# cvlab-kaist/SOLA

Measured on AMD Instinct MI355X. Metric: track-selection forward+loss samples/sec at (T=32,N=64,d=256), higher is better.
Workload: dtype f32 via split-f16 (hi+lo f16 operand pairs, 3 f16 MFMAs per product, f32 accumulate); 1 GPU; SOLA track selection forward+BCE+alignment loss+selection, T=32 N=64 d=256 L=16, mevis/default model (32.98M params, random init), 256 samples/step/GPU, conv weights re-standardised every step; batch_per_gpu=256, tracks=64, frames=32, text_len=16

## Files before the change

include/sola_hip.h:

```cpp
#ifndef SOLA_HIP_H
#define SOLA_HIP_H

#include <stddef.h>
#include <stdint.h>

#ifdef __cplusplus
extern "C" {
#endif

typedef enum SolaStatus {
    SOLA_OK = 0,
    SOLA_ERR_ARG = -1,
    SOLA_ERR_HIP = -2,
    SOLA_ERR_WEIGHT = -3,
    SOLA_ERR_WORKSPACE = -4,
    SOLA_ERR_STATE = -5
} SolaStatus;

typedef struct SolaConfig {
    int32_t object_token_dim;
    int32_t lang_token_dim;
    int32_t n_layers;
    int32_t max_temporal_length;
    int32_t n_negative;
    int32_t n_groups;
    int32_t n_groups_module;
    int32_t num_heads;
} SolaConfig;

typedef struct SolaCtx SolaCtx;

const char* sola_last_error(void);
const char* sola_version(void);

int sola_ctx_create(const SolaConfig* cfg, int device, SolaCtx** out);
int sola_ctx_destroy(SolaCtx* ctx);

int sola_num_weights(const SolaCtx* ctx);
int sola_weight_info(const SolaCtx* ctx, int index, const char** name, int64_t* numel);

int sola_set_weight(SolaCtx* ctx, const char* name, const void* dev_ptr, int64_t numel);

int sola_weights_changed(SolaCtx* ctx);
int sola_set_ws_policy(SolaCtx* ctx, int recompute_every_forward);

int sola_set_precision(SolaCtx* ctx, int precision);
int sola_set_split_guard(SolaCtx* ctx, int enable);

int sola_set_x16_arena(SolaCtx* ctx, void* dev_ptr, size_t bytes);
int sola_x16_arena_info(const SolaCtx* ctx, size_t* need_bytes, size_t* capacity_bytes, size_t* used_bytes);
int sola_split_fallback_count(const SolaCtx* ctx, int64_t* count, int32_t* last_guard);
int sola_cast_sp16(const float* dev_in, int ld_in, float* dev_out, int ld_out, int64_t rows, int K, float scale, void* stream);
int sola_cast_sp16_auto(const float* dev_in, int ld_in, float* dev_out, int ld_out, int64_t rows, int K, float* dev_scal, void* stream);
int sola_gemm_nt_split(const float* dev_a_sp, int lda, const float* dev_w_sp, const float* dev_bias, const float* dev_r,
                       int ldr, int r_is_split, float* dev_c, int ldc, int c_is_split, int M, int N, int K, float out_scale,
                       void* stream);
int sola_gemm_nt_split_scaled(const float* dev_a_sp, int lda, const float* dev_w_sp, const float* dev_bias, const float* dev_r,
                              int ldr, int r_is_split, float* dev_c, int ldc, int c_is_split, int M, int N, int K,
                              float out_scale, const float* dev_out_scale, void* stream);

int sola_cast_f16(const float* dev_in, int ld_in, void* dev_out, int ld_out, int64_t rows, int K, float scale, float* dev_scal, void* stream);
int sola_gemm_nt_f16(const void* dev_a_h, int lda, const void* dev_w_h, const float* dev_bias, const void* dev_r_h, int ldr,
                     void* dev_c, int ldc, int c_is_f16, int M, int N, int K, float out_scale, void* stream);
int sola_attention_f16(const void* dev_q, int ldq, const void* dev_k, int ldk, const void* dev_v, int ldv, void* dev_o, int ldo,
                       int G, int H, int head_dim, int Sq, int Sk, int inner, int64_t q_outer, int64_t q_inner, int64_t q_row_stride,
                       int64_t k_outer, int64_t k_inner, int64_t k_row_stride, float scale, void* stream);

int sola_gemm_nt_bf16(const void* dev_a, int lda, const void* dev_w, const float* dev_bias, const void* dev_r, int ldr, int r_is_bf16,
                      void* dev_c, int ldc, int c_is_bf16, int M, int N, int K, void* stream);
int sola_attention_bf16(const void* dev_q, int ldq, const void* dev_k, int ldk, const void* dev_v, int ldv, float* dev_o, void* dev_o_bf16, int ldo,
                        int G, int H, int head_dim, int Sq, int Sk, int inner, int64_t q_outer, int64_t q_inner, int64_t q_row_stride,
                        int64_t k_outer, int64_t k_inner, int64_t k_row_stride, float scale, float* dev_lse, void* stream);
int sola_attention_backward_bf16(const void* dev_q, int ldq, const void* dev_k, int ldk, const void* dev_v, int ldv, const void* dev_o, int o_is_bf16,
                                 const void* dev_dout, int dout_is_bf16, int ldo, const float* dev_lse, void* dev_dq_bf16, void* dev_dk_bf16, void* dev_dv_bf16,
                                 int ld_dq, int ld_dk, int ld_dv, float* dev_dq_scratch, float* dev_dvec, int G, int H, int head_dim, int Sq, int Sk,
                                 int inner, int64_t q_outer, int64_t q_inner, int64_t q_row_stride, int64_t k_outer, int64_t k_inner,
                                 int64_t k_row_stride, float scale, int64_t q_rows, float* dev_scratch, size_t scratch_floats, void* stream);

size_t sola_workspace_bytes(const SolaCtx* ctx, int B, int N, int T, int L);
int sola_forward(SolaCtx* ctx,
                 const float* dev_object_tokens,
                 const float* dev_lang_tokens,
                 int B, int N, int T, int L,
                 float* dev_score_map,
                 float* dev_score_tokens,
                 void* dev_workspace, size_t workspace_bytes, void* stream);

typedef struct SolaRaggedBatch {
    int32_t n_videos;
    const int32_t* video_tracks;
    const int32_t* video_frames;
    int32_t n_samples;
    const int32_t* sample_video;
    const int32_t* sample_text_len;
} SolaRaggedBatch;
size_t sola_ragged_workspace_bytes(const SolaCtx* ctx, const SolaRaggedBatch* batch);
int sola_forward_ragged(SolaCtx* ctx, const float* dev_object_tokens, const float* dev_lang_tokens, const SolaRaggedBatch* batch,
                        float* dev_score_map, float* dev_score_tokens, void* dev_workspace, size_t workspace_bytes, void* stream);
int sola_loss_ragged(const float* dev_score_map, const float* dev_score_tokens, const float* dev_labels,
                     const float* dev_pos_tokens, const float* dev_neg_tokens, int64_t neg_batch_stride, int n_samples,
                     const int32_t* dev_track_offsets, int max_tracks, int64_t total_tracks, int D, int n_neg,
                     float positive_weight, float temperature, float alignment_weight, float* dev_loss3,
                     int32_t* dev_neg_argmax, void* dev_scratch, size_t scratch_bytes, void* stream);

int sola_workspace_tap(const SolaCtx* ctx, const char* name, size_t* byte_offset, int64_t* rows, int64_t* cols);

int sola_loss(const float* dev_score_map, const float* dev_score_tokens,
              const float* dev_labels,
              const float* dev_pos_tokens,
              const float* dev_neg_tokens, int64_t neg_batch_stride,
              int B, int N, int D, int n_neg,
              float positive_weight, float temperature, float alignment_weight,
              float* dev_loss3, int32_t* dev_neg_argmax,
              void* dev_scratch, size_t scratch_bytes, void* stream);

int sola_select(const float* dev_score_map, int64_t n, float threshold, float* dev_prob, float* dev_pred, void* stream);

int sola_ws_standardize(const float* dev_w, int cout, int cin, int k, float* dev_out, void* stream);
int sola_gemm_nt(const float* dev_a, int lda, const float* dev_w, const float* dev_bias, const float* dev_r, int ldr,
                 float* dev_c, int ldc, int M, int N, int K, void* stream);
int sola_gemm_nn(const float* dev_a, int lda, const float* dev_w0, const float* dev_w1, const float* dev_w2, int w_rows, const float* dev_r,
                 int ldr, float* dev_c, int ldc, int M, int N, int K, void* stream);
int sola_conv1d_cl(const float* dev_x, const float* dev_wstd, const float* dev_bias, float* dev_y,
                   int R, int T_in, int cin, int cout, int k, int stride, int pad, void* stream);
int sola_group_norm(const float* dev_x, float* dev_y, float* dev_y2, const float* dev_pe,
                    const float* dev_gamma, const float* dev_beta,
                    int n_inst, int inner, int64_t outer_stride, int64_t inner_stride, int64_t tok_stride,
                    int ntok, int C, int groups, float eps, float leaky_slope, int apply_leaky, void* stream);
int sola_attention(const float* dev_q, int ldq, const float* dev_k, int ldk, const float* dev_v, int ldv,
                   float* dev_o, int ldo, int G, int H, int head_dim, int Sq, int Sk, int inner,
                   int64_t q_outer, int64_t q_inner, int64_t q_row_stride,
                   int64_t k_outer, int64_t k_inner, int64_t k_row_stride, float scale,
                   float* dev_lse , void* stream);
int sola_pos_encoding(const float* dev_gauss, int D, int t_len, int max_temporal_length, float* dev_pe, void* stream);

int sola_set_dropout(SolaCtx* ctx, float p_encoder, float p_attention, uint64_t seed);
int sola_set_stage_dropout(float p, uint64_t seed);
size_t sola_train_workspace_bytes(const SolaCtx* ctx, int B, int N, int T, int L);
size_t sola_backward_workspace_bytes(const SolaCtx* ctx, int B, int N, int T, int L);
int sola_set_grad(SolaCtx* ctx, const char* name, void* dev_ptr, int64_t numel);
int sola_forward_train(SolaCtx* ctx, const float* dev_object_tokens, const float* dev_lang_tokens,
                       int B, int N, int T, int L, float* dev_score_map, float* dev_score_tokens,
                       void* dev_workspace, size_t workspace_bytes, void* stream);
int sola_backward(SolaCtx* ctx, const float* dev_d_score_map, const float* dev_d_score_tokens,
                  const void* dev_forward_workspace, void* dev_scratch, size_t scratch_bytes, void* stream);
int sola_train_step_bind(SolaCtx* ctx, const char* const* names, const int32_t* group, int n, int n_groups);
size_t sola_train_step_workspace_bytes(const SolaCtx* ctx, int B, int N);
int sola_train_step(SolaCtx* ctx, const float* dev_object_tokens, const float* dev_lang_tokens, int B, int N, int T, int L,
                    const float* dev_labels, const float* dev_pos_tokens, float positive_weight, float temperature, float alignment_weight,
                    float max_grad_norm, float* dev_score_map, float* dev_score_tokens, float* dev_loss3, double* dev_grad_sq,
                    void* dev_train_workspace, size_t train_workspace_bytes, void* dev_backward_scratch, size_t backward_scratch_bytes,
                    void* dev_step_workspace, size_t step_workspace_bytes, void* stream);
int sola_adamw_bind(SolaCtx* ctx, const char* const* names, void* const* dev_exp_avg, void* const* dev_exp_avg_sq, void* const* dev_step, int n);
int sola_adamw_step(SolaCtx* ctx, double lr, double beta1, double beta2, double eps, double weight_decay, int64_t step, const double* dev_total_sq,
                    float max_grad_norm, int write_back_grads, void* stream);
size_t sola_train_ragged_workspace_bytes(const SolaCtx* ctx, const SolaRaggedBatch* batch);
size_t sola_backward_ragged_workspace_bytes(const SolaCtx* ctx, const SolaRaggedBatch* batch);
int sola_forward_train_ragged(SolaCtx* ctx, const float* dev_object_tokens, const float* dev_lang_tokens, const SolaRaggedBatch* batch,
                              float* dev_score_map, float* dev_score_tokens, void* dev_workspace, size_t workspace_bytes, void* stream);
int sola_backward_ragged(SolaCtx* ctx, const float* dev_d_score_map, const float* dev_d_score_tokens,
                         const void* dev_forward_workspace, void* dev_scratch, size_t scratch_bytes, void* stream);
int sola_loss_backward_ragged(const float* dev_score_map, const float* dev_score_tokens, const float* dev_labels,
                              const float* dev_pos_tokens, const float* dev_neg_tokens, int64_t neg_batch_stride, int n_samples,
                              const int32_t* dev_track_offsets, int max_tracks, int64_t total_tracks, int D, int n_neg,
                              float positive_weight, float temperature, float alignment_weight, const float* dev_g3,
                              float* dev_d_score_map, float* dev_d_score_tokens, float* dev_d_neg, void* dev_scratch,
                              size_t scratch_bytes, void* stream);
int sola_grad_bucket_count(const SolaCtx* ctx);
int sola_grad_bucket_of(const SolaCtx* ctx, const char* name);
int sola_backward_wait_bucket(SolaCtx* ctx, int bucket, void* stream);
int sola_loss_backward(const float* dev_score_map, const float* dev_score_tokens, const float* dev_labels,
                       const float* dev_pos_tokens, const float* dev_neg_tokens, int64_t neg_batch_stride,
                       int B, int N, int D, int n_neg, float positive_weight, float temperature, float alignment_weight,
                       const float* dev_g3, float* dev_d_score_map, float* dev_d_score_tokens, float* dev_d_neg,
                       void* dev_scratch, size_t scratch_bytes, void* stream);
size_t sola_grad_sqnorms_scratch_bytes(int n, const int64_t* numel);
int sola_grad_sqnorms(const float* const* dev_grads, const int64_t* numel, const int32_t* group, int n, int n_groups,
                      double* dev_out, void* dev_scratch, size_t scratch_bytes, void* stream);
int sola_grad_clip(float* const* dev_grads, const int64_t* numel, int n, const double* dev_total_sq, float max_norm,
                   void* stream);
int sola_ws_backward(const float* dev_w, const float* dev_dwstd, int cout, int cin, int k, float* dev_dw, void* stream);
int sola_attention_split(const float* dev_q_sp, int ldq, const float* dev_k_sp, int ldk, const float* dev_v_sp, int ldv,
                         float* dev_o, int ldo, int o_is_split, int G, int H, int head_dim, int Sq, int Sk, int inner,
                         int64_t q_outer, int64_t q_inner, int64_t q_row_stride,
                         int64_t k_outer, int64_t k_inner, int64_t k_row_stride, float scale, float* dev_lse, void* stream);
size_t sola_gemm_tn_scratch_bytes(int M, int N, int K);
int sola_gemm_tn(const float* dev_a, int lda, const float* dev_b, int ldb, float* dev_c, float* dev_bias_grad,
                 int M, int N, int K, void* dev_scratch, size_t scratch_bytes, void* stream);
size_t sola_gemm_tn_split_scratch_bytes(int M, int N, int K);
int sola_gemm_tn_split(const float* dev_a, int lda, const float* dev_b, int ldb, float* dev_c, int M, int N, int K,
                       void* dev_scratch, size_t scratch_bytes, void* stream);
int sola_gemm_tn_f16(const float* dev_a, int lda, const float* dev_b, int ldb, float* dev_c, int M, int N, int K, int fmt,
                     void* dev_scratch, size_t scratch_bytes, void* stream);
int sola_conv1d_cl_wgrad_f16(const float* dev_x, const float* dev_dy, float* dev_dwstd, int R, int T_in, int cin, int cout, int k,
                             int stride, int pad, int fmt, void* dev_scratch, size_t scratch_bytes, void* stream);
int sola_conv1d_cl_backward(const float* dev_x, const float* dev_wstd, const float* dev_dy, float* dev_dx,
                            float* dev_dwstd, float* dev_dbias, int R, int T_in, int cin, int cout, int k, int stride,
                            int pad, void* dev_scratch, size_t scratch_bytes, void* stream);
size_t sola_conv1d_cl_backward_split_scratch_bytes(int R, int T_in, int cin, int cout, int k, int stride, int pad);
int sola_conv1d_cl_backward_split(const float* dev_x, const float* dev_wstd, const float* dev_dy, float* dev_dx,
                                  float* dev_dwstd, float* dev_dbias, int R, int T_in, int cin, int cout, int k, int stride,
                                  int pad, void* dev_scratch, size_t scratch_bytes, void* stream);
int sola_group_norm_backward(const float* dev_x, const float* dev_dy, const float* dev_dy2, const float* dev_gamma,
                             const float* dev_beta, float* dev_dx, float* dev_dgamma, float* dev_dbeta,
                             int n_inst, int inner, int64_t outer_stride, int64_t inner_stride, int64_t tok_stride,
                             int ntok, int C, int groups, float eps, float leaky_slope, int apply_leaky,
                             void* dev_scratch, size_t scratch_bytes, void* stream);
int sola_attention_backward(const float* dev_q, int ldq, const float* dev_k, int ldk, const float* dev_v, int ldv,
                            const float* dev_o, const float* dev_dout, int ldo, const float* dev_lse,
                            float* dev_dq, float* dev_dk, float* dev_dv, float* dev_dvec ,
                            int G, int H, int head_dim, int Sq, int Sk, int inner,
                            int64_t q_outer, int64_t q_inner, int64_t q_row_stride,
                            int64_t k_outer, int64_t k_inner, int64_t k_row_stride, float scale, void* stream);
size_t sola_attention_backward_scratch_floats(int64_t q_rows, int G, int H, int Sk);
int sola_attention_backward_ws(const float* dev_q, int ldq, const float* dev_k, int ldk, const float* dev_v, int ldv,
                               const float* dev_o, const float* dev_dout, int ldo, const float* dev_lse,
                               float* dev_dq, float* dev_dk, float* dev_dv, float* dev_dvec, int G, int H, int head_dim, int Sq, int Sk,
                               int inner, int64_t q_outer, int64_t q_inner, int64_t q_row_stride, int64_t k_outer, int64_t k_inner,
                               int64_t k_row_stride, float scale, int64_t q_rows, float* dev_scratch, size_t scratch_floats, void* stream);

int64_t sola_mask_words(int H, int W);
int sola_mask_pack(const void* dev_masks, int elem_type, int n, int h, int w, int H, int W,
                   uint32_t* dev_bits, int64_t* dev_area, void* stream);
int sola_mask_pair_counts(const uint32_t* dev_a_bits, const int64_t* dev_a_area, int P, int T,
                          const uint32_t* dev_b_bits, const int64_t* dev_b_area, int R,
                          const int32_t* dev_a_frame, int64_t words,
                          int64_t* dev_inter, int64_t* dev_union, void* stream);
size_t sola_mask_iou_scratch_bytes(int P, int R, int H, int W);
int sola_mask_iou_matrix(const void* dev_a, const void* dev_b, int elem_type, int P, int R, int H, int W, int h, int w,
                         int64_t* dev_inter, int64_t* dev_union, void* dev_scratch, size_t scratch_bytes, void* stream);

int sola_mask_bilinear_pack(const void* dev_masks, int elem_type, int n, int h, int w, int H, int W,
                            uint32_t* dev_bits, int64_t* dev_area, void* stream);
int sola_mask_unpack(const uint32_t* dev_bits, int n, int H, int W, void* dev_out, int elem_type, void* stream);
int sola_rle_fill_or(const uint32_t* dev_cum, const int64_t* dev_off, int n_frames, int K, int h, int w,
                     uint8_t* dev_out, uint32_t* dev_bits, int64_t* dev_area, void* stream);

int64_t sola_rle_string_to_cum(const char* str, int64_t len, uint32_t* host_cum, int64_t cap, int64_t limit);

int64_t sola_jf_plane_words(int h, int w);
int sola_rle_pack_cm(const uint32_t* dev_cum, const int64_t* dev_off, int64_t n_planes, int h, int w, int64_t words_stride,
                     uint32_t* dev_bits, void* stream);
int sola_mask_select_counts(const uint32_t* dev_bits, int64_t words_stride, int n_masks, int T, const int32_t* dev_pred_off,
                            const int32_t* dev_pred_idx, const int32_t* dev_gt_off, const int32_t* dev_gt_idx, int E,
                            int64_t* dev_counts, void* stream);
int64_t sola_rle_strings_to_cum_batch(const char* chars, const int64_t* str_off, int64_t n, uint32_t* host_cum, int64_t cap,
                                      int64_t limit, int64_t* run_off);

int sola_mask_select_boundary_counts(const uint32_t* dev_bits, int64_t words_stride, int n_masks, int T, int h, int w, int radius,
                                     const int32_t* dev_pred_off, const int32_t* dev_pred_idx, const int32_t* dev_gt_off,
                                     const int32_t* dev_gt_idx, int E, int64_t* dev_counts, void* workspace, size_t workspace_bytes,
                                     void* stream);
size_t sola_boundary_counts_workspace_bytes(int h, int w, int radius, int E, int T);

size_t sola_rle_encode_scratch_bytes(int n, int h, int w);
int sola_rle_encode_runs(const void* dev_masks, int elem_type, int n, int h, int w, int64_t* dev_run_off,
                         void* dev_scratch, size_t scratch_bytes, void* stream);
int sola_rle_encode_cum(const void* dev_masks, int elem_type, int n, int h, int w, const int64_t* dev_run_off,
// ... 40 lines not shown
```

sola_amd/_lib.py:

```python
from __future__ import annotations

import contextlib
import ctypes as C
import os

_HERE = os.path.dirname(os.path.abspath(__file__))
LIB_PATH = os.environ.get("SOLA_HIP_LIB") or os.path.join(_HERE, "lib", "libsola_hip.so")


class SolaLibraryError(RuntimeError):
    pass


class SolaError(RuntimeError):
    """A libsola_hip call returned a negative status."""


class SolaConfig(C.Structure):
    _fields_ = [
        ("object_token_dim", C.c_int32),
        ("lang_token_dim", C.c_int32),
        ("n_layers", C.c_int32),
        ("max_temporal_length", C.c_int32),
        ("n_negative", C.c_int32),
        ("n_groups", C.c_int32),
        ("n_groups_module", C.c_int32),
        ("num_heads", C.c_int32),
    ]


class SolaRaggedBatch(C.Structure):
    _fields_ = [
        ("n_videos", C.c_int32),
        ("video_tracks", C.POINTER(C.c_int32)),
        ("video_frames", C.POINTER(C.c_int32)),
        ("n_samples", C.c_int32),
        ("sample_video", C.POINTER(C.c_int32)),
        ("sample_text_len", C.POINTER(C.c_int32)),
    ]


_vp, _i, _i64, _f, _sz = C.c_void_p, C.c_int, C.c_int64, C.c_float, C.c_size_t

SIGNATURES = {
    "sola_last_error": (C.c_char_p, []),
    "sola_version": (C.c_char_p, []),
    "sola_ctx_create": (_i, [C.POINTER(SolaConfig), _i, C.POINTER(_vp)]),
    "sola_ctx_destroy": (_i, [_vp]),
    "sola_num_weights": (_i, [_vp]),
    "sola_weight_info": (_i, [_vp, _i, C.POINTER(C.c_char_p), C.POINTER(_i64)]),
    "sola_set_weight": (_i, [_vp, C.c_char_p, _vp, _i64]),
    "sola_weights_changed": (_i, [_vp]),
    "sola_set_ws_policy": (_i, [_vp, _i]),
    "sola_set_precision": (_i, [_vp, _i]),
    "sola_set_split_guard": (_i, [_vp, _i]),
    "sola_split_fallback_count": (_i, [_vp, C.POINTER(_i64), C.POINTER(C.c_int32)]),
    "sola_cast_sp16": (_i, [_vp, _i, _vp, _i, _i64, _i, _f, _vp]),
    "sola_gemm_nt_split": (_i, [_vp, _i, _vp, _vp, _vp, _i, _i, _vp, _i, _i, _i, _i, _i, _f, _vp]),
    "sola_cast_sp16_auto": (_i, [_vp, _i, _vp, _i, _i64, _i, _vp, _vp]),
    "sola_gemm_nt_split_scaled": (_i, [_vp, _i, _vp, _vp, _vp, _i, _i, _vp, _i, _i, _i, _i, _i, _f, _vp, _vp]),
    "sola_cast_f16": (_i, [_vp, _i, _vp, _i, _i64, _i, _f, _vp, _vp]),
    "sola_gemm_nt_f16": (_i, [_vp, _i, _vp, _vp, _vp, _i, _vp, _i, _i, _i, _i, _i, _f, _vp]),
    "sola_gemm_nn": (_i, [_vp, _i, _vp, _vp, _vp, _i, _vp, _i, _vp, _i, _i, _i, _i, _vp]),
    "sola_gemm_nt_bf16": (_i, [_vp, _i, _vp, _vp, _vp, _i, _i, _vp, _i, _i, _i, _i, _i, _vp]),
    "sola_attention_bf16": (_i, [_vp, _i, _vp, _i, _vp, _i, _vp, _vp, _i, _i, _i, _i, _i, _i, _i, _i64, _i64, _i64, _i64, _i64, _i64, _f, _vp, _vp]),
    "sola_attention_backward_bf16": (_i, [_vp, _i, _vp, _i, _vp, _i, _vp, _i, _vp, _i, _i, _vp, _vp, _vp, _vp, _i, _i, _i, _vp, _vp, _i, _i, _i, _i, _i, _i,
                                          _i64, _i64, _i64, _i64, _i64, _i64, _f, _i64, _vp, _sz, _vp]),
    "sola_attention_f16": (_i, [_vp, _i, _vp, _i, _vp, _i, _vp, _i, _i, _i, _i, _i, _i, _i, _i64, _i64, _i64, _i64, _i64, _i64, _f, _vp]),
    "sola_workspace_bytes": (_sz, [_vp, _i, _i, _i, _i]),
    "sola_forward": (_i, [_vp, _vp, _vp, _i, _i, _i, _i, _vp, _vp, _vp, _sz, _vp]),
    "sola_ragged_workspace_bytes": (_sz, [_vp, C.POINTER(SolaRaggedBatch)]),
    "sola_forward_ragged": (_i, [_vp, _vp, _vp, C.POINTER(SolaRaggedBatch), _vp, _vp, _vp, _sz, _vp]),
    "sola_loss_ragged": (_i, [_vp, _vp, _vp, _vp, _vp, _i64, _i, _vp, _i, _i64, _i, _i, _f, _f, _f, _vp, _vp, _vp, _sz, _vp]),
    "sola_train_ragged_workspace_bytes": (_sz, [_vp, C.POINTER(SolaRaggedBatch)]),
    "sola_backward_ragged_workspace_bytes": (_sz, [_vp, C.POINTER(SolaRaggedBatch)]),
    "sola_forward_train_ragged": (_i, [_vp, _vp, _vp, C.POINTER(SolaRaggedBatch), _vp, _vp, _vp, _sz, _vp]),
    "sola_backward_ragged": (_i, [_vp, _vp, _vp, _vp, _vp, _sz, _vp]),
    "sola_loss_backward_ragged": (_i, [_vp, _vp, _vp, _vp, _vp, _i64, _i, _vp, _i, _i64, _i, _i, _f, _f, _f, _vp, _vp, _vp, _vp, _vp, _sz, _vp]),
    "sola_workspace_tap": (_i, [_vp, C.c_char_p, C.POINTER(_sz), C.POINTER(_i64), C.POINTER(_i64)]),
    "sola_loss": (_i, [_vp, _vp, _vp, _vp, _vp, _i64, _i, _i, _i, _i, _f, _f, _f, _vp, _vp, _vp, _sz, _vp]),
    "sola_select": (_i, [_vp, _i64, _f, _vp, _vp, _vp]),
    "sola_ws_standardize": (_i, [_vp, _i, _i, _i, _vp, _vp]),
    "sola_gemm_nt": (_i, [_vp, _i, _vp, _vp, _vp, _i, _vp, _i, _i, _i, _i, _vp]),
    "sola_conv1d_cl": (_i, [_vp, _vp, _vp, _vp, _i, _i, _i, _i, _i, _i, _i, _vp]),
    "sola_group_norm": (_i, [_vp, _vp, _vp, _vp, _vp, _vp, _i, _i, _i64, _i64, _i64, _i, _i, _i, _f, _f, _i, _vp]),
    "sola_attention": (_i, [_vp, _i, _vp, _i, _vp, _i, _vp, _i, _i, _i, _i, _i, _i, _i, _i64, _i64, _i64, _i64, _i64, _i64, _f, _vp, _vp]),
    "sola_attention_split": (_i, [_vp, _i, _vp, _i, _vp, _i, _vp, _i, _i, _i, _i, _i, _i, _i, _i, _i64, _i64, _i64, _i64, _i64, _i64, _f, _vp, _vp]),
    "sola_set_dropout": (_i, [_vp, _f, _f, C.c_uint64]),
    "sola_set_stage_dropout": (_i, [_f, C.c_uint64]),
    "sola_train_workspace_bytes": (_sz, [_vp, _i, _i, _i, _i]),
    "sola_backward_workspace_bytes": (_sz, [_vp, _i, _i, _i, _i]),
    "sola_set_grad": (_i, [_vp, C.c_char_p, _vp, _i64]),
    "sola_forward_train": (_i, [_vp, _vp, _vp, _i, _i, _i, _i, _vp, _vp, _vp, _sz, _vp]),
    "sola_backward": (_i, [_vp, _vp, _vp, _vp, _vp, _sz, _vp]),
    "sola_grad_bucket_count": (_i, [_vp]),
    "sola_grad_bucket_of": (_i, [_vp, C.c_char_p]),
    "sola_backward_wait_bucket": (_i, [_vp, _i, _vp]),
    "sola_loss_backward": (_i, [_vp, _vp, _vp, _vp, _vp, _i64, _i, _i, _i, _i, _f, _f, _f, _vp, _vp, _vp, _vp, _vp, _sz, _vp]),
    "sola_ws_backward": (_i, [_vp, _vp, _i, _i, _i, _vp, _vp]),
    "sola_gemm_tn_scratch_bytes": (_sz, [_i, _i, _i]),
    "sola_gemm_tn_split_scratch_bytes": (_sz, [_i, _i, _i]),
    "sola_gemm_tn_split": (_i, [_vp, _i, _vp, _i, _vp, _i, _i, _i, _vp, _sz, _vp]),
    "sola_gemm_tn_f16": (_i, [_vp, _i, _vp, _i, _vp, _i, _i, _i, _i, _vp, _sz, _vp]),
    "sola_conv1d_cl_wgrad_f16": (_i, [_vp, _vp, _vp, _i, _i, _i, _i, _i, _i, _i, _i, _vp, _sz, _vp]),
    "sola_gemm_tn": (_i, [_vp, _i, _vp, _i, _vp, _vp, _i, _i, _i, _vp, _sz, _vp]),
    "sola_conv1d_cl_backward": (_i, [_vp, _vp, _vp, _vp, _vp, _vp, _i, _i, _i, _i, _i, _i, _i, _vp, _sz, _vp]),
    "sola_conv1d_cl_backward_split_scratch_bytes": (_sz, [_i, _i, _i, _i, _i, _i, _i]),
    "sola_conv1d_cl_backward_split": (_i, [_vp, _vp, _vp, _vp, _vp, _vp, _i, _i, _i, _i, _i, _i, _i, _vp, _sz, _vp]),
    "sola_group_norm_backward": (_i, [_vp, _vp, _vp, _vp, _vp, _vp, _vp, _vp, _i, _i, _i64, _i64, _i64, _i, _i, _i, _f, _f, _i, _vp, _sz, _vp]),
    "sola_attention_backward": (_i, [_vp, _i, _vp, _i, _vp, _i, _vp, _vp, _i, _vp, _vp, _vp, _vp, _vp, _i, _i, _i, _i, _i, _i,
                                     _i64, _i64, _i64, _i64, _i64, _i64, _f, _vp]),
    "sola_attention_backward_scratch_floats": (_sz, [_i64, _i, _i, _i]),
    "sola_attention_backward_ws": (_i, [_vp, _i, _vp, _i, _vp, _i, _vp, _vp, _i, _vp, _vp, _vp, _vp, _vp, _i, _i, _i, _i, _i, _i,
                                        _i64, _i64, _i64, _i64, _i64, _i64, _f, _i64, _vp, _sz, _vp]),
    "sola_pos_encoding": (_i, [_vp, _i, _i, _i, _vp, _vp]),
    "sola_mask_words": (_i64, [_i, _i]),
    "sola_mask_pack": (_i, [_vp, _i, _i, _i, _i, _i, _i, _vp, _vp, _vp]),
    "sola_mask_pair_counts": (_i, [_vp, _vp, _i, _i, _vp, _vp, _i, _vp, _i64, _vp, _vp, _vp]),
    "sola_mask_bilinear_pack": (_i, [_vp, _i, _i, _i, _i, _i, _i, _vp, _vp, _vp]),
    "sola_mask_unpack": (_i, [_vp, _i, _i, _i, _vp, _i, _vp]),
    "sola_rle_fill_or": (_i, [_vp, _vp, _i, _i, _i, _i, _vp, _vp, _vp, _vp]),
    "sola_rle_string_to_cum": (_i64, [C.c_char_p, _i64, _vp, _i64, _i64]),
    "sola_jf_plane_words": (_i64, [_i, _i]),
    "sola_rle_pack_cm": (_i, [_vp, _vp, _i64, _i, _i, _i64, _vp, _vp]),
    "sola_mask_select_counts": (_i, [_vp, _i64, _i, _i, _vp, _vp, _vp, _vp, _i, _vp, _vp]),
    "sola_mask_select_boundary_counts": (_i, [_vp, _i64, _i, _i, _i, _i, _i, _vp, _vp, _vp, _vp, _i, _vp, _vp, _sz, _vp]),
    "sola_boundary_counts_workspace_bytes": (_sz, [_i, _i, _i, _i, _i]),
    "sola_rle_strings_to_cum_batch": (_i64, [_vp, _vp, _i64, _vp, _i64, _i64, _vp]),
    "sola_rle_encode_scratch_bytes": (_sz, [_i, _i, _i]),
    "sola_rle_encode_runs": (_i, [_vp, _i, _i, _i, _i, _vp, _vp, _sz, _vp]),
    "sola_rle_encode_cum": (_i, [_vp, _i, _i, _i, _i, _vp, _vp, _vp, _vp, _sz, _vp]),
    "sola_rle_encode_chars": (_i, [_vp, _vp, _vp, _i, _vp, _vp]),
    "sola_png_deflate_scratch_bytes": (_sz, [_i, _i, _i]),
    "sola_png_deflate_sizes": (_i, [_vp, _i, _i, _i, _i, _vp, _vp, _vp, _sz, _vp]),
    "sola_png_deflate_write": (_i, [_vp, _i, _i, _i, _i, _vp, _vp, _vp, _vp, _sz, _vp]),
    "sola_mask_iou_scratch_bytes": (_sz, [_i, _i, _i, _i]),
    "sola_mask_iou_matrix": (_i, [_vp, _vp, _i, _i, _i, _i, _i, _i, _i, _vp, _vp, _vp, _sz, _vp]),
    "sola_grad_sqnorms_scratch_bytes": (_sz, [_i, _vp]),
    "sola_grad_sqnorms": (_i, [_vp, _vp, _vp, _i, _i, _vp, _vp, _sz, _vp]),
    "sola_grad_clip": (_i, [_vp, _vp, _i, _vp, _f, _vp]),
    "sola_set_x16_arena": (_i, [_vp, _vp, _sz]),
    "sola_x16_arena_info": (_i, [_vp, C.POINTER(_sz), C.POINTER(_sz), C.POINTER(_sz)]),
    "sola_tune": (_i, [C.c_char_p, _i]),
    "sola_tune_query": (_i, [C.c_char_p, C.POINTER(_i), C.POINTER(_i)]),
    "sola_tune_key": (C.c_char_p, [_i]),
    "sola_has_experiments": (_i, []),
    "sola_selftest": (_i, [_vp]),
    "sola_adamw_bind": (_i, [_vp, C.POINTER(C.c_char_p), C.POINTER(_vp), C.POINTER(_vp), C.POINTER(_vp), _i]),
    "sola_adamw_step": (_i, [_vp, C.c_double, C.c_double, C.c_double, C.c_double, C.c_double, _i64, _vp, _f, _i, _vp]),
    "sola_train_step_bind": (_i, [_vp, C.POINTER(C.c_char_p), C.POINTER(C.c_int32), _i, _i]),
    "sola_train_step_workspace_bytes": (_sz, [_vp, _i, _i]),
    "sola_train_step": (_i, [_vp, _vp, _vp, _i, _i, _i, _i, _vp, _vp, _f, _f, _f, _f, _vp, _vp, _vp, _vp, _vp, _sz, _vp, _sz, _vp, _sz, _vp]),
    "sola_gemm_trace_read": (C.c_longlong, [_vp, C.c_longlong]),
    "sola_profile_enable": (_i, [_i]),
    "sola_profile_read": (_i, [C.POINTER(_i64), C.POINTER(C.c_double), C.POINTER(C.c_double), C.POINTER(C.c_double), _i]),
}

PROF_CATEGORIES = ["gemm128", "attn", "group_norm", "ws_standardize", "head_loss", "misc", "iou_pack", "iou_pair", "gemm64", "gemm_tn", "attn_bwd", "gemm_split",
                   "gemm_split256", "gemm_split256_gn"]

_lib = None


def lib():
    global _lib
    if _lib is not None:
        return _lib
    import torch

    if not os.path.exists(LIB_PATH):
        raise SolaLibraryError(
            f"{LIB_PATH} not found. Build it with `python -c 'import __graft_entry__ as g; g.build()'` "
            "(or `make -C sola_amd/csrc`). sola_amd has no CPU or PyTorch fallback.")
    try:
        h = C.CDLL(LIB_PATH)
    except OSError as e:
        raise SolaLibraryError(f"failed to load {LIB_PATH}: {e}") from e
    for name, (res, args) in SIGNATURES.items():
        try:
            fn = getattr(h, name)
        except AttributeError as e:
            raise SolaLibraryError(f"{LIB_PATH} does not export {name}") from e
        fn.restype = res
        fn.argtypes = args
    for kv in filter(None, os.environ.get("SOLA_TUNE", "").split(",")):
        k, v = kv.split("=")
        if h.sola_tune(k.strip().encode(), int(v)) != 0:
            raise SolaLibraryError(f"SOLA_TUNE: unknown key {k!r}")
    _lib = h
    return h


def has_experiments():
    return bool(lib().sola_has_experiments())


def tune_query(key):
    value, default = _i(), _i()
    check(lib().sola_tune_query(key.encode(), C.byref(value), C.byref(default)), f"sola_tune_query {key!r}")
    return value.value, default.value


def tune_default(key):
    return tune_query(key)[1]


@contextlib.contextmanager
def tuned(**keys):
    before = [(k, tune_query(k)[0]) for k in keys]
    try:
        for k, v in keys.items():
            check(lib().sola_tune(k.encode(), int(v)), f"sola_tune {k!r}")
        yield
    finally:
        for k, old in reversed(before):
            check(lib().sola_tune(k.encode(), old), f"sola_tune {k!r}")


def check(status, what=""):
    if status != 0:
        msg = lib().sola_last_error()
        raise SolaError(f"{what} failed with status {status}: {msg.decode() if msg else ''}")


def ptr(t):
    return None if t is None else C.c_void_p(t.data_ptr())


def current_stream(device=None):
    import torch

    return C.c_void_p(torch.cuda.current_stream(device).cuda_stream)
# ... 25 lines not shown
```

sola_amd/csrc/api.hip:

```cpp
#include <math.h>
#include <stdarg.h>
#include <string.h>

#include <algorithm>
#include <exception>
#include <mutex>

#include "ragged.h"
#include "tune.h"

static thread_local char g_err[1024] = "";
void sola_set_error(const char* fmt, ...) {
    va_list ap;
    va_start(ap, fmt);
    vsnprintf(g_err, sizeof(g_err), fmt, ap);
    va_end(ap);
}
extern "C" const char* sola_last_error(void) { return g_err; }
extern "C" const char* sola_version(void) { return "sola_hip 0.6 (gfx950; f32, range-guarded split-f16 and f16-operand MFMA forward and backward, ragged batches, mask IoU + masklet rows)"; }

namespace {
struct ProfRec {
    int cat;
    hipEvent_t e0, e1;
// ... 203 lines not shown
    if (w->grad != static_cast<float*>(dev_ptr)) c->adam_n = 0;
    w->grad = static_cast<float*>(dev_ptr);
    return SOLA_OK;
}

extern "C" int sola_weights_changed(SolaCtx* c) {
    SOLA_ARG(c, "weights_changed: null ctx");
    c->ws_dirty = true;
    c->lin16_dirty = true;
    return SOLA_OK;
}

extern "C" int sola_set_dropout(SolaCtx* c, float p_encoder, float p_attention, uint64_t seed) {
    SOLA_ARG(c && p_encoder >= 0.f && p_encoder < 1.f && p_attention >= 0.f && p_attention < 1.f, "set_dropout: bad argument");
    c->p_drop_encoder = p_encoder;
    c->p_drop_attention = p_attention;
    c->drop_seed = seed;
    return SOLA_OK;
}

static thread_local DropoutCfg g_stage_drop = {0u, 0u, 0xFFFFFFFFu, 1.f, 0};
extern "C" int sola_set_stage_dropout(float p, uint64_t seed) {
    SOLA_ARG(p >= 0.f && p < 1.f, "set_stage_dropout: p=%f", (double)p);
    g_stage_drop = make_dropout(p, seed, 0);
    return SOLA_OK;
}

__global__ void selftest_wave_kernel(const float* __restrict__ in, int* __restrict__ bad) {
    const int i = blockIdx.x * blockDim.x + threadIdx.x;
    const float x = in[i];
    float v = x, m = x;
    int wrong = 0;
    float w = x;
#pragma unroll
    for (int o = 32, s = 0; o > 0; o >>= 1, ++s) {
        v += __shfl_xor(v, o, 64);
        m = fmaxf(m, __shfl_xor(m, o, 64));
        w = s == 0 ? sum_xor32(w) : s == 1 ? sum_xor16(w) : s == 2 ? sum_xor8(w) : s == 3 ? sum_xor4(w) : s == 4 ? sum_xor2(w) : sum_xor1(w);
        wrong |= __float_as_uint(w) != __float_as_uint(v) ? 1 << s : 0;
    }
    wrong |= __float_as_uint(wave_sum(x)) != __float_as_uint(v) ? 64 : 0;
    wrong |= __float_as_uint(wave_max(x)) != __float_as_uint(m) ? 128 : 0;
    if (wrong) atomicOr(bad, wrong);
}
extern "C" int sola_selftest(void* stream_) {
    hipStream_t s = as_stream(stream_);
    constexpr int n = 64 * 1024;
    std::vector<float> h(n);
    unsigned r = 12345u;
    for (int i = 0; i < n; ++i) {
        r = r * 1664525u + 1013904223u;
        h[i] = ((int)(r >> 8) % 20001 - 10000) / 37.0f * ((i % 7) ? 1.f : 1e-3f);
    }
    float* d_in = nullptr;
    int* d_bad = nullptr;
    SOLA_HIP(hipMalloc(&d_in, n * sizeof(float)));
    if (hipMalloc(&d_bad, sizeof(int)) != hipSuccess) { (void)hipFree(d_in); sola_set_error("selftest: hipMalloc"); return SOLA_ERR_HIP; }
    int bad = 0, rc = SOLA_OK;
    if (hipMemcpyAsync(d_in, h.data(), n * sizeof(float), hipMemcpyHostToDevice, s) != hipSuccess || hipMemsetAsync(d_bad, 0, sizeof(int), s) != hipSuccess) rc = SOLA_ERR_HIP;
    if (rc == SOLA_OK) {
        hipLaunchKernelGGL(selftest_wave_kernel, dim3(n / 256), dim3(256), 0, s, d_in, d_bad);
        if (hipGetLastError() != hipSuccess || hipMemcpyAsync(&bad, d_bad, sizeof(int), hipMemcpyDeviceToHost, s) != hipSuccess || hipStreamSynchronize(s) != hipSuccess) rc = SOLA_ERR_HIP;
    }
    (void)hipFree(d_in);
    (void)hipFree(d_bad);
    if (rc != SOLA_OK) { sola_set_error("selftest: HIP error"); return rc; }
    if (bad) {
        sola_set_error("selftest: the vector-ALU wave reductions differ from the __shfl_xor butterfly (mask 0x%x: bits 0-5 = steps 32..1, 64 = wave_sum, 128 = wave_max)", bad);
        return SOLA_ERR_STATE;
    }
    return SOLA_OK;
}

extern "C" int sola_has_experiments(void) {
#ifdef SOLA_EXPERIMENTS
    return 1;
#else
    return 0;
#endif
}

static int g_stage_split_math = 0;
static void sola_set_stage_split_math(int v) { g_stage_split_math = v != 0; }
#define TUNE_EXTERN(key) extern int g_##key;
#define TUNE_NONE(key, setter, report)
SOLA_TUNE_KEYS(TUNE_EXTERN, TUNE_NONE)
#ifdef SOLA_EXPERIMENTS
SOLA_TUNE_EXPERIMENT_KEYS(TUNE_EXTERN, TUNE_NONE)
#endif
namespace {
struct TuneKey {
    const char* key;
    void (*set)(int);
    int (*report)();
    int initial;
};
#define TUNE_PLAIN(key) {#key, [](int v) { g_##key = v; }, []() -> int { return g_##key; }, g_##key},
#define TUNE_SPECIAL(key, setter, report) {#key, setter, []() -> int { return report; }, report},
const TuneKey g_tune_keys[] = {
    SOLA_TUNE_KEYS(TUNE_PLAIN, TUNE_SPECIAL)
#ifdef SOLA_EXPERIMENTS
    SOLA_TUNE_EXPERIMENT_KEYS(TUNE_PLAIN, TUNE_SPECIAL)
#endif
};
constexpr int kTuneKeys = sizeof(g_tune_keys) / sizeof(g_tune_keys[0]);

const TuneKey* tune_find(const char* key) {
    for (const TuneKey& k : g_tune_keys)
        if (!strcmp(key, k.key)) return &k;
    sola_set_error("tune: unknown key '%s'%s", key, sola_has_experiments() ? "" : " (experiment keys exist in EXPERIMENTS=1 builds only)");
    return nullptr;
}
}

extern "C" int sola_tune(const char* key, int value) {
    SOLA_ARG(key, "tune: null key");
    const TuneKey* k = tune_find(key);
    if (!k) return SOLA_ERR_ARG;
    k->set(value);
    return SOLA_OK;
}

extern "C" int sola_tune_query(const char* key, int* value, int* default_value) {
    SOLA_ARG(key, "tune: null key");
    const TuneKey* k = tune_find(key);
    if (!k) return SOLA_ERR_ARG;
    if (value) *value = k->report();
    if (default_value) *default_value = k->initial;
    return SOLA_OK;
}

extern "C" const char* sola_tune_key(int index) { return index >= 0 && index < kTuneKeys ? g_tune_keys[index].key : nullptr; }

extern "C" int sola_set_ws_policy(SolaCtx* c, int every) {
    SOLA_ARG(c, "set_ws_policy: null ctx");
    c->ws_every_forward = every != 0;
    return SOLA_OK;
}

extern "C" size_t sola_workspace_bytes(const SolaCtx* c, int B, int N, int T, int L) {
    if (!c || B <= 0 || N <= 0 || T <= 0 || L < 0) return 0;
    return make_plan(c, B, N, T, L, false).total;
}

extern "C" size_t sola_train_workspace_bytes(const SolaCtx* c, int B, int N, int T, int L) {
    if (!c || B <= 0 || N <= 0 || T <= 0 || L < 0) return 0;
    return make_plan(c, B, N, T, L, true).total;
}

extern "C" int sola_workspace_tap(const SolaCtx* c, const char* name, size_t* off, int64_t* rows, int64_t* cols) {
    SOLA_ARG(c && name, "workspace_tap: null argument");
    auto it = c->last.bufs.find(name);
    SOLA_ARG(it != c->last.bufs.end(), "workspace_tap: no buffer named '%s' (run sola_forward first)", name);
    if (off) *off = it->second.off;
    if (rows) *rows = it->second.rows;
    if (cols) *cols = it->second.cols;
    return SOLA_OK;
}

extern "C" int sola_set_precision(SolaCtx* c, int precision) {
    SOLA_ARG(c && precision >= 0 && precision <= 3, "set_precision: 0 (f32), 1 (split-f16), 2 (f16 storage / f16 GEMM operands) or 3 (bf16 GEMM operands, training)");
    if (precision >= 1 && !c->lin16_buf) {
        const size_t D = c->cfg.lang_token_dim;
        size_t ws_total = 0;
        for (int i = 0; i < 6; ++i) ws_total += (size_t)c->conv[i].cout * c->conv[i].cin * c->conv[i].k;
        SOLA_HIP(hipSetDevice(c->device));
        SOLA_HIP(hipMalloc(&c->ws16_buf, ws_total * sizeof(float)));
        SOLA_HIP(hipMalloc(&c->lin16_buf, (size_t)c->cfg.n_layers * 12 * D * D * sizeof(float)));
        const size_t n_pairs = 2 + (size_t)c->cfg.n_layers * 12;
        SOLA_HIP(hipMalloc(&c->scal_buf, (2 * n_pairs + 2 + 4) * sizeof(float)));
        SOLA_HIP(hipMemset(c->scal_buf, 0, (2 * n_pairs + 2 + 4) * sizeof(float)));
        c->guard = reinterpret_cast<int*>(c->scal_buf + 2 * n_pairs);
        SOLA_HIP(hipHostMalloc(reinterpret_cast<void**>(&c->guard_host), 2 * sizeof(int), hipHostMallocDefault));
        c->guard_host[0] = c->guard_host[1] = 0;
    }
    c->precision = precision;
    c->ws_dirty = true;
    c->lin16_dirty = true;
    return SOLA_OK;
}

extern "C" int sola_cast_sp16(const float* in, int ld_in, float* out, int ld_out, int64_t rows, int K, float scale, void* stream_) {
    return launch_cast_sp16(in, ld_in, out, ld_out, rows, K, scale, as_stream(stream_));
}

extern "C" int sola_gemm_nt_split(const float* a_sp, int lda, const float* w_sp, const float* bias, const float* r, int ldr,
                                  int r_sp16, float* cmat, int ldc, int c_sp16, int M, int N, int K, float out_scale, void* stream_) {
    SOLA_ARG(a_sp && w_sp && cmat, "gemm_nt_split: null argument");
    GemmDesc gd{};
    gd.nprob = 1;
    gd.p[0] = GemmProblem{a_sp, w_sp, bias, r, cmat};
    gd.M = M; gd.N = N; gd.K = K; gd.lda = lda; gd.ldr = ldr; gd.ldc = ldc;
    gd.arith = 1; gd.out_scale = out_scale; gd.r_sp16 = r_sp16; gd.c_sp16 = c_sp16;
    return launch_gemm(gd, as_stream(stream_));
}

int launch_attention_f16(const AttnDesc& d, hipStream_t s);
extern "C" int sola_cast_f16(const float* in, int ld_in, void* out, int ld_out, int64_t rows, int K, float scale, float* dev_scal, void* stream_) {
    return launch_cast_f16(in, ld_in, out, ld_out, rows, K, scale, dev_scal, as_stream(stream_));
}
extern "C" int sola_gemm_nt_f16(const void* a_h, int lda, const void* w_h, const float* bias, const void* r_h, int ldr, void* cmat, int ldc,
                                int c_is_f16, int M, int N, int K, float out_scale, void* stream_) {
    SOLA_ARG(a_h && w_h && cmat, "gemm_nt_f16: null argument");
    GemmDesc gd{};
    gd.nprob = 1;
    gd.p[0] = GemmProblem{static_cast<const float*>(a_h), static_cast<const float*>(w_h), bias, static_cast<const float*>(r_h), static_cast<float*>(cmat)};
    gd.M = M; gd.N = N; gd.K = K; gd.lda = lda; gd.ldr = ldr; gd.ldc = ldc;
    gd.arith = 2; gd.out_scale = out_scale; gd.r_f16 = r_h ? 1 : 0; gd.c_f16 = c_is_f16;
    return launch_gemm(gd, as_stream(stream_));
}
extern "C" int sola_attention_f16(const void* q, int ldq, const void* k, int ldk, const void* v, int ldv, void* o, int ldo, int G, int H,
                                  int head_dim, int Sq, int Sk, int inner, int64_t q_outer, int64_t q_inner, int64_t q_rs,
                                  int64_t k_outer, int64_t k_inner, int64_t k_rs, float scale, void* stream_) {
    SOLA_ARG(q && k && v && o, "attention_f16: null argument");
    AttnDesc d{static_cast<const float*>(q), static_cast<const float*>(k), static_cast<const float*>(v), static_cast<float*>(o), ldq, ldk, ldv, ldo,
               G, H, head_dim, Sq, Sk, inner, q_outer, q_inner, q_rs, k_outer, k_inner, k_rs, scale, nullptr};
    return launch_attention_f16(d, as_stream(stream_));
}

extern "C" int sola_gemm_nt_bf16(const void* a_b, int lda, const void* w_b, const float* bias, const void* r, int ldr, int r_is_bf16, void* cmat, int ldc,
                                 int c_is_bf16, int M, int N, int K, void* stream_) {
    SOLA_ARG(a_b && w_b && cmat, "gemm_nt_bf16: null argument");
    GemmDesc gd{};
    gd.nprob = 1;
    gd.p[0] = GemmProblem{static_cast<const float*>(a_b), static_cast<const float*>(w_b), bias, static_cast<const float*>(r), static_cast<float*>(cmat)};
    gd.M = M; gd.N = N; gd.K = K; gd.lda = lda; gd.ldr = ldr; gd.ldc = ldc;
    gd.arith = 2; gd.bf16 = 1; gd.out_scale = 1.f; gd.r_f16 = (r && r_is_bf16) ? 1 : 0; gd.c_f16 = c_is_bf16;
    return launch_gemm(gd, as_stream(stream_));
}
extern "C" int sola_attention_bf16(const void* q, int ldq, const void* k, int ldk, const void* v, int ldv, float* o, void* o_bf16, int ldo, int G, int H,
                                   int head_dim, int Sq, int Sk, int inner, int64_t q_outer, int64_t q_inner, int64_t q_rs,
                                   int64_t k_outer, int64_t k_inner, int64_t k_rs, float scale, float* lse, void* stream_) {
    SOLA_ARG(q && k && v && (o || o_bf16), "attention_bf16: null argument");
    AttnDesc d{static_cast<const float*>(q), static_cast<const float*>(k), static_cast<const float*>(v), o, ldq, ldk, ldv, ldo,
               G, H, head_dim, Sq, Sk, inner, q_outer, q_inner, q_rs, k_outer, k_inner, k_rs, scale, lse};
    d.drop = g_stage_drop;
    d.in_bf16 = 1;
    bool done = false;
    if (o_bf16) { d.o_cast = o_bf16; d.o_cast_fmt = 3; d.o_cast_done = &done; }
    SOLA_TRY(launch_attention(d, as_stream(stream_)));
    SOLA_ARG(!o_bf16 || done, "attention_bf16: this shape does not write the bf16 output");
    return SOLA_OK;
}
extern "C" int sola_attention_backward_bf16(const void* q, int ldq, const void* k, int ldk, const void* v, int ldv, const void* o, int o_bf16, const void* dout, int dout_bf16, int ldo,
                                            const float* lse, void* dq16, void* dk16, void* dv16, int ld_dq, int ld_dk, int ld_dv, float* dq_scratch,
                                            float* dvec, int G, int H, int head_dim, int Sq, int Sk, int inner, int64_t q_outer, int64_t q_inner,
                                            int64_t q_rs, int64_t k_outer, int64_t k_inner, int64_t k_rs, float scale, int64_t q_rows, float* scratch,
                                            size_t scratch_floats, void* stream_) {
    SOLA_ARG(q && k && v && o && dout && lse && dq16 && dk16 && dv16 && dq_scratch && dvec, "attention_backward_bf16: null argument");
    AttnBwdDesc d{static_cast<const float*>(q), static_cast<const float*>(k), static_cast<const float*>(v), static_cast<const float*>(o), static_cast<const float*>(dout), lse, dq_scratch, nullptr, nullptr, dvec,
                  ldq, ldk, ldv, ldo, ld_dq, ld_dk, ld_dv, G, H, head_dim, Sq, Sk, inner, q_outer, q_inner, q_rs, k_outer, k_inner, k_rs, scale};
    d.drop = g_stage_drop;
    d.part = scratch; d.part_floats = scratch_floats; d.part_rows = q_rows;
    d.io_bf16 = 1; d.dq16 = dq16; d.dk16 = dk16; d.dv16 = dv16;
    d.dout_bf16 = dout_bf16 ? 1 : 0;
    d.o_bf16 = o_bf16 ? 1 : 0;
    return launch_attention_bwd(d, as_stream(stream_));
}

extern "C" int sola_cast_sp16_auto(const float* in, int ld_in, float* out, int ld_out, int64_t rows, int K, float* scal, void* stream_) {
    return launch_cast_sp16_auto(in, ld_in, out, ld_out, rows, K, scal, as_stream(stream_));
}

extern "C" int sola_gemm_nt_split_scaled(const float* a_sp, int lda, const float* w_sp, const float* bias, const float* r, int ldr,
                                         int r_sp16, float* cmat, int ldc, int c_sp16, int M, int N, int K, float out_scale,
                                         const float* out_scale_dev, void* stream_) {
    SOLA_ARG(a_sp && w_sp && cmat, "gemm_nt_split_scaled: null argument");
    GemmDesc gd{};
    gd.nprob = 1;
    gd.p[0] = GemmProblem{a_sp, w_sp, bias, r, cmat};
    gd.M = M; gd.N = N; gd.K = K; gd.lda = lda; gd.ldr = ldr; gd.ldc = ldc;
    gd.arith = 1; gd.out_scale = out_scale; gd.out_scale_dev = out_scale_dev; gd.r_sp16 = r_sp16; gd.c_sp16 = c_sp16;
    return launch_gemm(gd, as_stream(stream_));
}

int sola_split_guard_tripped(SolaCtx* c, hipStream_t s, bool* tripped) {
    *tripped = false;
    if (!c->split_guard || !c->guard) return SOLA_OK;
    hipStreamCaptureStatus cap = hipStreamCaptureStatusNone;
    if (hipStreamIsCapturing(s, &cap) == hipSuccess && cap != hipStreamCaptureStatusNone) return SOLA_OK;
    SOLA_HIP(hipMemcpyAsync(c->guard_host, c->guard, 2 * sizeof(int), hipMemcpyDeviceToHost, s));
    SOLA_HIP(hipStreamSynchronize(s));
    *tripped = (c->guard_host[0] | c->guard_host[1]) != 0;
    if (!c->guard_host[1]) c->weight_range_bad = false;
    if (c->guard_host[1] && !c->weight_range_bad) {
        c->weight_range_bad = true;
        fprintf(stderr, "sola_hip: GroupNorm weights outside the range of the split-f16 activations (rms of (gamma, beta) not in "
                        "[2^-6, 2^9]): precision 1 calls run on the exact-f32 kernels until the weights change\n");
    }
    return SOLA_OK;
}
static bool split_known_out_of_range(const SolaCtx* c) { return c->precision == 1 && c->split_guard && c->weight_range_bad && !c->lin16_dirty; }

int g_infer_f32_rows = 4096;
struct PrecScope {
    SolaCtx* c;
    int saved;
    PrecScope(SolaCtx* ctx, int p) : c(ctx), saved(ctx->precision) { c->precision = p; }
    ~PrecScope() { c->precision = saved; }
    PrecScope(const PrecScope&) = delete;
    PrecScope& operator=(const PrecScope&) = delete;
};
static bool few_rows_f32(const SolaCtx* c, long long rows0) { return c->precision == 1 && g_infer_f32_rows > 0 && rows0 <= g_infer_f32_rows; }

extern "C" int sola_forward(SolaCtx* c, const float* obj, const float* lang, int B, int N, int T, int L, float* score_map,
                            float* score_tokens, void* workspace, size_t ws_bytes, void* stream_) {
    hipStream_t s = as_stream(stream_);
    SOLA_ARG(!c || c->precision != 3, "forward: precision 3 (bf16 GEMM operands) is a TRAINING mode; inference runs precision 0, 1 or 2");
    if (c && B > 0 && N > 0 && T > 0 && few_rows_f32(c, (long long)B * N * T)) {
        PrecScope f32(c, 0);
// ... 666 lines not shown
```

sola_amd/csrc/ctx.h:

```cpp
#pragma once
#include <string>
#include <unordered_map>
#include <vector>

#include "kernels.h"

struct ConvGeom {
    int cin, cout, k, stride, pad;
};
struct Weight {
    std::string name;
    int64_t numel;
    const float* ptr;
    float* grad;
};
struct Buf {
    size_t off;
    int64_t rows, cols;
};
struct Plan {
    int B = 0, N = 0, T = 0, L = 0, W = 0, Tp = 0, M = 0;
    int Tl[6] = {0};
    bool train = false;
    bool rag = false;
    std::unordered_map<std::string, Buf> bufs;
    size_t total = 0;
    size_t add(const std::string& name, int64_t rows, int64_t cols) {
        const size_t off = total;
        bufs[name] = Buf{off, rows, cols};
        total += (((size_t)rows * (size_t)cols * sizeof(float)) + 255) & ~(size_t)255;
        return off;
    }
};

struct RagTables {
    const int4* u_lvl[7] = {nullptr};
    const int2* rowmap[5] = {nullptr};
    const int4* imap[5] = {nullptr};
    const int4* u_vt = nullptr;
    const int4* u_st = nullptr;
    const int4* u_strk = nullptr;
    const int4* u_smp = nullptr;
    const int4* u_lang = nullptr;
    const int4* u_langk = nullptr;
    const int4* u_gather = nullptr;
    const int32_t* trk_off = nullptr;
    int V = 0, S = 0, NT = 0, sumNS = 0, sumTpV = 0, sumTpS = 0;
    int maxN = 0, maxT[7] = {0}, maxW = 0, maxRowsSample = 0;
    long long rows[7] = {0}, Mv = 0, Ms = 0, LW = 0, Lin = 0;
    bool identity = false;
};

struct SolaRagStage;
void sola_rag_stage_free(SolaRagStage* st);

struct SolaCtx {
    SolaConfig cfg;
    int device;
    ConvGeom conv[6];
    std::vector<Weight> weights;
    std::unordered_map<std::string, int> index;
    float* ws_buf = nullptr;
    size_t ws_off[6];
    bool ws_dirty = true;
    int ws16_fmt = 0;
    bool ws_every_forward = true;
    Plan last;
    const float* last_obj = nullptr;
    RagTables last_rag;
    const void* last_ws = nullptr;
    std::vector<char> qkv16;
    std::vector<char> res16;
    std::vector<char> attn_o16;
    std::vector<char> gn2_stats;
    int precision = 0;
    bool lin16_dirty = true;
    float* ws16_buf = nullptr;
    float* lin16_buf = nullptr;
    struct X16Entry { const float* src; const void* p16; int cols; int fmt; };
    std::vector<X16Entry> x16;
    char* x16_arena = nullptr;
    size_t x16_cap = 0, x16_used = 0, x16_need = 0;
    void* x16_alloc(size_t bytes) {
        bytes = (bytes + 255) & ~(size_t)255;
        x16_need += bytes;
        if (x16_used + bytes > x16_cap) return nullptr;
        void* r = x16_arena + x16_used;
        x16_used += bytes;
        return r;
    }
    const void* x16_find(const float* src, int cols, int fmt) const {
        for (const X16Entry& e : x16)
            if (e.src == src && e.cols == cols && e.fmt == fmt) return e.p16;
        return nullptr;
    }
    float* scal_buf = nullptr;
    int* guard = nullptr;
    int* guard_host = nullptr;
    bool split_guard = true;
    long long split_fallbacks = 0;
    bool weight_range_bad = false;
    SolaRagStage* rag_stage = nullptr;
    std::vector<hipEvent_t> bucket_ev;
    hipStream_t side_stream = nullptr;
    hipEvent_t ev_fork = nullptr, ev_side[4] = {nullptr, nullptr, nullptr, nullptr};
    bool bucket_recorded = false;
    int n_buckets() const { return cfg.n_layers + 1; }
    float* scal_pair(int i) const { return scal_buf + 2 * i; }
    float* scal_extra(int i) const { return scal_buf + 2 * (2 + (size_t)cfg.n_layers * 12) + 2 + i; }
    const float* lin_inv_scale(int layer, int attn, int proj) const { return scal_buf + 2 * (2 + (layer * 3 + attn) * 4 + proj) + 1; }
    struct StepBinding {
        std::vector<int> widx;
        std::vector<int32_t> group;
        std::vector<long long> numel;
        int n_groups = 0;
        size_t sq_scratch = 0;
    } step;
    void* adam_tab = nullptr;
    int adam_n = 0, adam_cap = 0, adam_blocks = 0;
    bool adam_has_steps = false;
    int* adam_ticket = nullptr;
    double adam_bytes = 0.0;
    float p_drop_encoder = 0.f, p_drop_attention = 0.f;
    unsigned long long drop_seed = 0;
    DropoutCfg enc_drop(int conv_idx) const { return make_dropout(p_drop_encoder, drop_seed, 1u + (unsigned)conv_idx); }
    DropoutCfg attn_drop(int layer, int a) const { return make_dropout(p_drop_attention, drop_seed, 100u + 3u * (unsigned)layer + (unsigned)a); }
};

static const int kConvIdx[6] = {0, 4, 8, 12, 16, 20};
static const int kNormIdx[5] = {1, 5, 9, 13, 17};
static const char* const kAttnShort[3] = {"obj", "mot", "o2l"};
static const char* const kAttnLong[3] = {"obj_attn", "motion_attn", "object2lang_attn"};
constexpr float kLinScale = 64.f;
int sola_refresh_lin16(SolaCtx* c, hipStream_t s);
int sola_refresh_conv_weights(SolaCtx* c, int fmt, bool force, hipStream_t s);
int sola_check_forward_args(const SolaCtx* c, const char* who, size_t need, const void* workspace, size_t ws_bytes);

inline const float* ctx_weight(const SolaCtx* c, const std::string& name) {
    auto it = c->index.find(name);
    return it == c->index.end() ? nullptr : c->weights[it->second].ptr;
}
inline float* ctx_grad(const SolaCtx* c, const std::string& name) {
    auto it = c->index.find(name);
    return it == c->index.end() ? nullptr : c->weights[it->second].grad;
}

inline std::string abuf(bool train, int layer, const char* attn, const char* what) {
    if (!train) return what;
    return "l" + std::to_string(layer) + "_" + attn + "_" + what;
}

struct RagShape;
Plan make_plan(const SolaCtx* c, int B, int N, int T, int L, bool train);
Plan make_plan_ragged(const SolaCtx* c, const RagShape& r, bool train);
int sola_forward_train_impl(SolaCtx* c, const float* obj, const float* lang, int B, int N, int T, int L, float* score_map,
                            float* score_tokens, void* workspace, size_t ws_bytes, hipStream_t s, const RagShape* rs = nullptr);
int sola_forward_infer_impl(SolaCtx* c, const float* obj, const float* lang, int B, int N, int T, int L, float* score_map,
                            float* score_tokens, void* workspace, size_t ws_bytes, hipStream_t s);
size_t sola_backward_scratch_bytes(const SolaCtx* c, const Plan& p);
size_t sola_ragged_workspace_bytes_impl(const SolaCtx* c, const SolaRaggedBatch* b, int precision);
int sola_forward_ragged_impl(SolaCtx* c, const float* obj, const float* lang, const SolaRaggedBatch* batch, float* score_map,
                             float* score_tokens, void* workspace, size_t ws_bytes, hipStream_t s);
```

sola_amd/csrc/forward.hip:

```cpp
#include <math.h>
#include <string.h>

#include <algorithm>

#include "ragged.h"

int g_train_gn_cast = 1;
extern int g_train_dw_f16;
int g_train_attn_cast = 1;
int g_train_bf16_store = 3;
int g_train_gn_stats = 1;
int g_train_x16_keep = 1;
int g_train_split_min_rows = 1024;

namespace {
struct PlanSizes {
    int64_t rows0;
    int64_t rows[6];
    int64_t M, BW;
    int64_t S;
    int64_t gn_slots;
    size_t tables;
};
void plan_fill(Plan& p, const SolaCtx* c, const PlanSizes& z, bool train) {
    const int D = c->cfg.lang_token_dim, H = c->cfg.num_heads;
    if (z.tables) p.add("tables", (int64_t)((z.tables + 3) / 4), 1);
    for (int i = 0; i < 6; ++i) {
        p.add("conv" + std::to_string(i), z.rows[i], c->conv[i].cout);
        if (i < 5) p.add("act" + std::to_string(i), z.rows[i], c->conv[i].cout);
    }
    if (z.M <= 8192) p.add("splitk", 8192, 4096);
    p.add("pe", p.Tp, D);
    p.add("gn_slots", z.gn_slots, 1);
    p.add("lang", z.BW, D);
    p.add("lbar", z.S, D);
    if (!train && c->precision >= 1) {
        p.add("obj_sp", z.rows0, c->cfg.object_token_dim);
        p.add("conv5_sp", z.M, D);
        p.add("lang_sp", z.BW, D);
    }
    if (train && c->precision >= 1 && z.M >= g_train_split_min_rows) {
        int64_t amax = std::max<int64_t>(z.rows0 * c->cfg.object_token_dim, std::max<int64_t>(z.M * D, z.BW * D));
        for (int i = 0; i < 5; ++i) amax = std::max<int64_t>(amax, z.rows[i] * c->conv[i].cout);
        p.add("sp_a", amax, 1);
        p.add("sp_b", z.M, D);
    }
    const int n_sets = train ? c->cfg.n_layers : 1;
    for (int l = 0; l < n_sets; ++l)
        for (int a = 0; a < (train ? 3 : 1); ++a) {
            p.add(abuf(train, l, kAttnShort[a], "q"), z.M, D);
            if (!train || a < 2) {
                p.add(abuf(train, l, kAttnShort[a], "k"), z.M, D);
                p.add(abuf(train, l, kAttnShort[a], "v"), z.M, D);
            }
            p.add(abuf(train, l, kAttnShort[a], "attn"), z.M, D);
            p.add(abuf(train, l, kAttnShort[a], "res"), z.M, D);
            if (train) p.add(abuf(train, l, kAttnShort[a], "lse"), z.M, H);
            if (!train || a == 2) {
                p.add(abuf(train, l, kAttnShort[a], "lk"), z.BW, D);
                p.add(abuf(train, l, kAttnShort[a], "lv"), z.BW, D);
            }
        }
    for (int l = 0; l < c->cfg.n_layers; ++l) {
        if (train) p.add("l" + std::to_string(l) + "_gn2st", z.S * c->cfg.n_groups_module, 2);
        p.add("l" + std::to_string(l) + "_obj", z.M, D);
        p.add("l" + std::to_string(l) + "_xpe", z.M, D);
        p.add("l" + std::to_string(l) + "_motion", z.M, D);
        p.add("l" + std::to_string(l) + "_o2l", z.M, D);
    }
}
}

Plan make_plan(const SolaCtx* c, int B, int N, int T, int L, bool train) {
    Plan p;
    p.B = B; p.N = N; p.T = T; p.L = L; p.train = train;
    p.W = L + c->cfg.n_negative;
    int t = T;
    for (int i = 0; i < 6; ++i) {
        t = (t + 2 * c->conv[i].pad - c->conv[i].k) / c->conv[i].stride + 1;
        p.Tl[i] = t;
    }
    p.Tp = p.Tl[5];
    p.M = B * N * p.Tp;
    const int64_t R = (int64_t)B * N;
    PlanSizes z{};
    z.rows0 = R * T;
    for (int i = 0; i < 6; ++i) z.rows[i] = R * p.Tl[i];
    z.M = p.M; z.BW = (int64_t)B * p.W; z.S = B;
    z.gn_slots = std::max<int64_t>(R * T, (int64_t)p.M) / 4 + 1024;
    plan_fill(p, c, z, train);
    return p;
}

Plan make_plan_ragged(const SolaCtx* c, const RagShape& r, bool train) {
    Plan p;
    p.rag = true;
    p.B = r.S; p.N = r.maxN; p.T = r.maxT[0]; p.L = r.maxW - c->cfg.n_negative; p.train = train;
    p.W = r.maxW;
    for (int i = 0; i < 6; ++i) p.Tl[i] = r.maxT[i + 1];
    p.Tp = r.maxT[6];
    p.M = (int)r.Ms;
    PlanSizes z{};
    z.rows0 = r.rows[0];
    for (int i = 0; i < 6; ++i) z.rows[i] = r.rows[i + 1];
    z.M = r.Ms; z.BW = r.LW; z.S = r.S;
    z.gn_slots = (int64_t)(rag_gn_slots_bytes(r) / 4 + 64);
    z.tables = rag_tables_bytes(r, train);
    plan_fill(p, c, z, train);
    return p;
}

int sola_forward_train_impl(SolaCtx* c, const float* obj, const float* lang, int B, int N, int T, int L, float* score_map,
                            float* score_tokens, void* workspace, size_t ws_bytes, hipStream_t s, const RagShape* rs) {
    SOLA_ARG(c && obj && lang && score_map && score_tokens && workspace, "forward: null argument");
    if (rs) SOLA_ARG(rs->identity, "forward: a ragged training batch has one sample per video (sample_video[i] == i)");
    else SOLA_ARG(B > 0 && N > 0 && T > 0 && L >= 1, "forward: bad sizes B=%d N=%d T=%d L=%d", B, N, T, L);
    Plan p = rs ? make_plan_ragged(c, *rs, true) : make_plan(c, B, N, T, L, true);
    SOLA_TRY(sola_check_forward_args(c, "forward", p.total, workspace, ws_bytes));
    char* base = static_cast<char*>(workspace);
    auto buf = [&](const std::string& name) { return reinterpret_cast<float*>(base + p.bufs.at(name).off); };
    float* const splitk_ws = p.bufs.count("splitk") ? buf("splitk") : nullptr;
    const size_t splitk_bytes = splitk_ws ? (size_t)p.bufs.at("splitk").rows * p.bufs.at("splitk").cols * sizeof(float) : 0;
    auto W = [&](const std::string& name) { return ctx_weight(c, name); };
    const int D = c->cfg.lang_token_dim, H = c->cfg.num_heads, DH = D / H;
    const int Tp = p.Tp, M = p.M, Wn = p.W;
    if (rs) { B = rs->S; N = rs->maxN; T = rs->maxT[0]; }
    const int R = rs ? rs->NT : B * N;
    RagTables rt;
    if (rs) SOLA_TRY(rag_build_tables(c, *rs, base + p.bufs.at("tables").off, true, &rt, s));
    auto level_rows = [&](int lvl) -> long long { return rs ? rs->rows[lvl] : (long long)R * (lvl == 0 ? T : p.Tl[lvl - 1]); };
    const long long text_rows = rs ? rs->LW : (long long)B * Wn;
    const bool pure = c->precision >= 2;
    const int bf = c->precision == 3 ? 1 : 0;
    const bool split = c->precision >= 1 && D % (pure ? 64 : 32) == 0 && c->cfg.object_token_dim % (pure ? 64 : 32) == 0 && p.M >= g_train_split_min_rows;
    const int lowp_arith = pure ? 2 : 1;
    auto cast_auto = [&](const float* in, int ld, float* out, long long rows, int K, float* scal) -> int {
        return pure ? launch_cast_f16(in, ld, out, K, rows, K, 0.f, scal, s, 13, nullptr, bf) : launch_cast_sp16_auto(in, ld, out, K, rows, K, scal, s);
    };
    auto cast_fixed = [&](const float* in, int ld, float* out, long long rows, int K, float scale, void* side16 = nullptr) -> int {
        return pure ? launch_cast_f16(in, ld, out, K, rows, K, scale, nullptr, s, 13, nullptr, bf) : launch_cast_sp16(in, ld, out, K, rows, K, scale, s, side16);
    };

    SOLA_TRY(sola_refresh_conv_weights(c, split ? (pure ? 2 + bf : 1) : 0, true, s));
    auto lin_idx = [&](const std::string& attn, int proj) -> int {
        const int l = attn[attn.find('.') + 1] - '0';
        int a3 = 0;
        for (int a = 0; a < 3; ++a)
            if (attn.size() >= strlen(kAttnLong[a]) && attn.compare(attn.size() - strlen(kAttnLong[a]), std::string::npos, kAttnLong[a]) == 0) a3 = a;
        return (l * 3 + a3) * 4 + proj;
    };
    auto lin16 = [&](const std::string& attn, int proj) -> const float* {
        return pure ? reinterpret_cast<const float*>(reinterpret_cast<const _Float16*>(c->lin16_buf) + (size_t)lin_idx(attn, proj) * D * D)
                    : c->lin16_buf + (size_t)lin_idx(attn, proj) * D * D;
    };
    auto lin_inv = [&](const std::string& attn, int proj) -> const float* { return c->scal_buf + 2 * (2 + lin_idx(attn, proj)) + 1; };
    if (split) SOLA_TRY(sola_refresh_lin16(c, s));
    float* const sp_a = split ? buf("sp_a") : nullptr;
    float* const sp_b = split ? buf("sp_b") : nullptr;
    const bool keep16 = split && pure && g_train_x16_keep != 0;
    const bool side16_on = split && !pure && g_train_x16_keep != 0 && g_train_dw_f16 != 0;
    c->x16.clear();
    c->x16_used = 0;
    c->x16_need = 0;
    auto side16 = [&](const float* src, long long rows, int cols) -> void* {
        if (!side16_on) return nullptr;
        void* q = c->x16_alloc((size_t)rows * cols * 2);
        if (q) c->x16.push_back(SolaCtx::X16Entry{src, q, cols, 1});
        return q;
    };
    auto slot16 = [&](int which, const float* src, long long rows, int cols) -> float* {
        if (keep16)
            if (void* q = c->x16_alloc((size_t)rows * cols * 2)) {
                c->x16.push_back(SolaCtx::X16Entry{src, q, cols, 1 + bf});
                return static_cast<float*>(q);
            }
        return which ? sp_b : sp_a;
    };

    const int gn_fmt = (split && pure && g_train_gn_cast) ? 2 + bf : 0;
    const float* pc_src[2] = {nullptr, nullptr};
    float* pc_dst[2] = {nullptr, nullptr};
    const float* x = obj;
    int t_in = T;
    for (int i = 0; i < 6; ++i) {
        const ConvGeom& g = c->conv[i];
        const std::string cp = "short_motion_encoder." + std::to_string(kConvIdx[i]);
        GemmDesc gd{};
        gd.nprob = 1;
        gd.p[0] = GemmProblem{x, c->ws_buf + c->ws_off[i], W(cp + ".bias"), nullptr, buf("conv" + std::to_string(i))};
        gd.M = (int)level_rows(i + 1); gd.N = g.cout; gd.K = g.k * g.cin;
        gd.lda = g.cin; gd.ldr = 0; gd.ldc = g.cout;
        gd.conv = g.k > 1 ? 1 : 0;
// ... 112 lines not shown
    void* ac_side = nullptr;
    bool ac_done = false;
    int o16_site = -1;
    c->attn_o16.assign((size_t)c->cfg.n_layers * 3, 0);
    auto attention = [&](AttnDesc& ad) -> int {
        ac_src = nullptr; ac_done = false;
        if (split && (pure ? g_train_attn_cast != 0 : g_train_attn_cast == 2) && ad.ldo == D) {
            ac_src = ad.o;
            ac_dst = slot16(0, ad.o, M, D);
            ac_side = side16(ad.o, M, D);
            ad.o_cast = ac_dst; ad.o_side = ac_side; ad.o_cast_fmt = pure ? 2 + bf : 1; ad.o_cast_done = &ac_done;
            if (o16_site >= 0 && ad.in_bf16 && g_train_bf16_store >= 3 && ac_dst != sp_a && ac_dst != sp_b && ad.o_cast_fmt == 3 &&
                attention_bf16_mfma_supported(ad) && attention_bwd_dout_bf16_enabled()) {
                ad.o = nullptr;
                c->attn_o16[(size_t)o16_site] = 1;
            }
        }
        o16_site = -1;
        return launch_attention(ad, s);
    };
    auto out_proj = [&](const std::string& attn, const float* ao, const float* resid, float* res, const void* r16 = nullptr) -> int {
        GemmDesc gd{};
        gd.nprob = 1;
        gd.p[0] = GemmProblem{ao, W(attn + ".out_proj.weight"), W(attn + ".out_proj.bias"), resid, res};
        gd.M = M; gd.N = D; gd.K = D; gd.lda = D; gd.ldr = D; gd.ldc = D;
        gd.splitk_ws = splitk_ws; gd.splitk_bytes = splitk_bytes;
        if (split && r16) { gd.p[0].R = static_cast<const float*>(r16); gd.r_f16 = 1; gd.c_f16 = 1; }
        if (split) {
            float* dst;
            if (ac_src == ao) {
                dst = ac_dst;
                if (!ac_done) SOLA_TRY(cast_fixed(ao, D, dst, M, D, 1.f, ac_side));
            } else {
                dst = slot16(0, ao, M, D);
                SOLA_TRY(cast_fixed(ao, D, dst, M, D, 1.f, side16(ao, M, D)));
            }
            ac_src = nullptr;
            gd.p[0].A = dst; gd.p[0].W = lin16(attn, 3); gd.p[0].scale_dev = lin_inv(attn, 3);
            gd.arith = lowp_arith; gd.out_scale = 1.f; gd.bf16 = bf;
        }
        return launch_gemm(gd, s);
    };
    int gn_layer = 0;
    auto gn = [&](const std::string& lp, int idx, const float* res, float* y, float* y2, int n_inst, int inner,
                  long long outer, long long inner_stride, long long tok_stride, int ntok, const int4* units = nullptr,
                  const float* next_src0 = nullptr, const float* next_src1 = nullptr, bool res_bf16 = false) -> int {
        GroupNormDesc nd{};
        nd.in_f16 = res_bf16 ? 2 : 0;
        if (gn_fmt) {
            const float* nxt[2] = {next_src0, next_src1};
            const long long y_rows = std::max<long long>(M, text_rows);
            for (int e = 0; e < 2; ++e) {
                if (!nxt[e]) continue;
                if (nxt[e] == y) { float* dst = slot16(e, y, y_rows, D); nd.y_cast = dst; pc_src[e] = y; pc_dst[e] = dst; }
                else if (nxt[e] == y2) { float* dst = slot16(e, y2, y_rows, D); nd.y2_cast = dst; pc_src[e] = y2; pc_dst[e] = dst; }
            }
            nd.cast_fmt = gn_fmt;
        }
            nd.slice_ws = buf("gn_slots"); nd.slice_ws_bytes = (size_t)p.bufs.at("gn_slots").rows * p.bufs.at("gn_slots").cols * sizeof(float);
        nd.x = res; nd.y = y; nd.y2 = y2; nd.pe = y2 ? buf("pe") : nullptr;
        nd.gamma = W(lp + "norm." + std::to_string(idx) + ".weight");
        nd.beta = W(lp + "norm." + std::to_string(idx) + ".bias");
        nd.n_inst = n_inst; nd.inner = inner; nd.outer_stride = outer; nd.inner_stride = inner_stride;
        nd.tok_stride = tok_stride; nd.ntok = ntok; nd.C = D; nd.groups = c->cfg.n_groups_module;
        nd.eps = 1e-5f; nd.slope = 0.f; nd.leaky = 0;
        nd.units = units;
        if (idx == 2 && g_train_gn_stats) {
            const int l = gn_layer;
            int wrote = 0;
            nd.stats_out = buf("l" + std::to_string(l) + "_gn2st");
            nd.stats_written = &wrote;
            SOLA_TRY(launch_group_norm(nd, s));
            if ((size_t)l < c->gn2_stats.size()) c->gn2_stats[l] = (char)wrote;
            return SOLA_OK;
        }
        return launch_group_norm(nd, s);
    };
    c->gn2_stats.assign((size_t)c->cfg.n_layers, 0);
    c->res16.assign((size_t)c->cfg.n_layers * 3, 0);
    auto resid16 = [&](const float* resid) -> const void* {
        if (!(split && pure && bf && g_train_bf16_store >= 2 && keep16 && D % 8 == 0)) return nullptr;
        return c->x16_find(resid, D, 1 + bf);
    };
    const float* xin = buf("conv5");
    for (int l = 0; l < c->cfg.n_layers; ++l) {
        const std::string lp = "object_lang_align_layers." + std::to_string(l) + ".";
        gn_layer = l;
        const std::string ls = "l" + std::to_string(l);
        auto ab = [&](int a, const char* what) { return buf(abuf(true, l, kAttnShort[a], what)); };
        float* x_obj = buf(ls + "_obj");
        float* x_pe = buf(ls + "_xpe");
        float* x_mot = buf(ls + "_motion");
        float* x_o2l = buf(ls + "_o2l");
        {
            AttnDesc ad{ab(0, "q"), ab(0, "k"), ab(0, "v"), ab(0, "attn"), D, D, D, D, B * Tp, H, DH, N, N, Tp,
                        (long long)N * Tp, 1, Tp, (long long)N * Tp, 1, Tp, scale, ab(0, "lse")};
            if (rs) { ad.G = rt.sumTpS; ad.inner = 1; ad.q_units = rt.u_st; }
            ad.drop = c->attn_drop(l, 0);
            const bool s16 = site16(ad, false);
            SOLA_TRY(linear3(xin, xin, xin, lp + "obj_attn", 3, M, ab(0, "q"), ab(0, "k"), ab(0, "v"), 0, nullptr, s16));
            ad.in_bf16 = s16 ? 1 : 0;
            c->qkv16[(size_t)l * 3 + 0] = s16;
            o16_site = l * 3 + 0;
            SOLA_TRY(attention(ad));
        }
        const void* r16_0 = resid16(xin);
        c->res16[(size_t)l * 3 + 0] = r16_0 != nullptr;
        SOLA_TRY(out_proj(lp + "obj_attn", ab(0, "attn"), xin, ab(0, "res"), r16_0));
        if (rs) SOLA_TRY(gn(lp, 0, ab(0, "res"), x_obj, x_pe, rt.sumTpS, 1, 0, 0, 1, N, rt.u_st, x_pe, x_obj, r16_0 != nullptr));
        else SOLA_TRY(gn(lp, 0, ab(0, "res"), x_obj, x_pe, B * Tp, Tp, (long long)N * Tp, 1, Tp, N, nullptr, x_pe, x_obj, r16_0 != nullptr));
        {
            AttnDesc ad{ab(1, "q"), ab(1, "k"), ab(1, "v"), ab(1, "attn"), D, D, D, D, B * N, H, DH, Tp, Tp, 1,
                        (long long)Tp, 0, 1, (long long)Tp, 0, 1, scale, ab(1, "lse")};
            if (rs) { ad.G = rt.sumNS; ad.q_units = rt.u_strk; }
            ad.drop = c->attn_drop(l, 1);
            const bool s16 = site16(ad, false);
            SOLA_TRY(linear3(x_pe, x_pe, x_obj, lp + "motion_attn", 3, M, ab(1, "q"), ab(1, "k"), ab(1, "v"), 0, nullptr, s16));
            ad.in_bf16 = s16 ? 1 : 0;
            c->qkv16[(size_t)l * 3 + 1] = s16;
            o16_site = l * 3 + 1;
            SOLA_TRY(attention(ad));
        }
        const void* r16_1 = resid16(x_obj);
        c->res16[(size_t)l * 3 + 1] = r16_1 != nullptr;
        SOLA_TRY(out_proj(lp + "motion_attn", ab(1, "attn"), x_obj, ab(1, "res"), r16_1));
        if (rs) SOLA_TRY(gn(lp, 1, ab(1, "res"), x_mot, nullptr, rt.sumNS, 1, 0, 0, 1, Tp, rt.u_strk, x_mot, nullptr, r16_1 != nullptr));
        else SOLA_TRY(gn(lp, 1, ab(1, "res"), x_mot, nullptr, B * N, 1, Tp, 0, 1, Tp, nullptr, x_mot, nullptr, r16_1 != nullptr));
        {
            AttnDesc ad{ab(2, "q"), ab(2, "lk"), ab(2, "lv"), ab(2, "attn"), D, D, D, D, B, H, DH, N * Tp, Wn, 1,
                        (long long)N * Tp, 0, 1, (long long)Wn, 0, 1, scale, ab(2, "lse")};
            if (rs) { ad.Sq = rt.maxRowsSample; ad.q_units = rt.u_smp; ad.k_units = rt.u_langk; }
            ad.drop = c->attn_drop(l, 2);
            const bool s16 = site16(ad, true);
            SOLA_TRY(linear3(x_mot, nullptr, nullptr, lp + "object2lang_attn", 1, M, ab(2, "q"), nullptr, nullptr, 0, nullptr, s16));
            SOLA_TRY(linear3(buf("lang"), buf("lang"), nullptr, lp + "object2lang_attn", 2, (int)text_rows, ab(2, "lk"), ab(2, "lv"), nullptr, 1,
                             split ? c->scal_pair(1) : nullptr, s16));
            ad.in_bf16 = s16 ? 1 : 0;
            c->qkv16[(size_t)l * 3 + 2] = s16;
            o16_site = l * 3 + 2;
            SOLA_TRY(attention(ad));
        }
        const void* r16_2 = resid16(x_mot);
        c->res16[(size_t)l * 3 + 2] = r16_2 != nullptr;
        SOLA_TRY(out_proj(lp + "object2lang_attn", ab(2, "attn"), x_mot, ab(2, "res"), r16_2));
        const float* nxt_in = l + 1 < c->cfg.n_layers ? x_o2l : nullptr;
        if (rs) SOLA_TRY(gn(lp, 2, ab(2, "res"), x_o2l, nullptr, B, 1, 0, 0, 1, rt.maxRowsSample, rt.u_smp, nxt_in, nullptr, r16_2 != nullptr));
        else SOLA_TRY(gn(lp, 2, ab(2, "res"), x_o2l, nullptr, B, 1, (long long)N * Tp, 0, 1, N * Tp, nullptr, nxt_in, nullptr, r16_2 != nullptr));
        xin = x_o2l;
    }

    HeadDesc hd{xin, buf("lbar"), score_map, score_tokens, B, N, Tp, D};
    if (rs) { hd.B = 1; hd.N = rt.sumNS; hd.units = rt.u_strk; }
    SOLA_TRY(launch_score_head(hd, s));
    c->last = p;
    c->last_rag = rt;
    c->last_ws = workspace;
    c->last_obj = obj;
    return SOLA_OK;
}
```

sola_amd/csrc/forward_infer.hip:

```cpp
#include <math.h>

#include <algorithm>

#include "ctx.h"

int sola_refresh_lin16(SolaCtx* c, hipStream_t s) {
    if (!c->lin16_dirty) return SOLA_OK;
    SOLA_ARG(c->lin16_buf && c->scal_buf, "split-f16 weights requested before sola_set_precision(ctx, 1)");
    static const char* pn[4] = {"q_proj", "k_proj", "v_proj", "out_proj"};
    const int D = c->cfg.lang_token_dim;
    std::vector<const float*> in;
    std::vector<float*> out;
    for (int l = 0; l < c->cfg.n_layers; ++l)
        for (int a = 0; a < 3; ++a)
            for (int j = 0; j < 4; ++j) {
                const std::string nm = "object_lang_align_layers." + std::to_string(l) + "." + kAttnLong[a] + "." + pn[j] + ".weight";
                const float* w = ctx_weight(c, nm);
                if (!w) {
                    sola_set_error("forward: weight '%s' has not been set", nm.c_str());
                    return SOLA_ERR_WEIGHT;
                }
                in.push_back(w);
                out.push_back(c->lin16_buf + ((size_t)(l * 3 + a) * 4 + j) * D * D);
            }
    if (c->precision >= 2) {
        std::vector<void*> outh;
        for (size_t i = 0; i < out.size(); ++i) outh.push_back(reinterpret_cast<_Float16*>(c->lin16_buf) + i * (size_t)D * D);
        SOLA_TRY(launch_cast_f16_auto_multi(in.data(), outh.data(), (int)in.size(), D, D, c->scal_pair(2), s, c->precision == 3 ? 1 : 0));
    } else {
        SOLA_TRY(launch_cast_sp16_auto_multi(in.data(), out.data(), (int)in.size(), D, D, c->scal_pair(2), s));
    }
    std::vector<NormPair> norms;
    for (int i = 0; i < 5; ++i) {
        const std::string np = "short_motion_encoder." + std::to_string(kNormIdx[i]);
        norms.push_back(NormPair{ctx_weight(c, np + ".weight"), ctx_weight(c, np + ".bias"), c->conv[i].cout});
    }
    for (int l = 0; l < c->cfg.n_layers; ++l)
        for (int j = 0; j < 3; ++j) {
            const std::string np = "object_lang_align_layers." + std::to_string(l) + ".norm." + std::to_string(j);
            norms.push_back(NormPair{ctx_weight(c, np + ".weight"), ctx_weight(c, np + ".bias"), D});
        }
    for (const NormPair& n : norms)
        if (!n.gamma || !n.beta) {
            sola_set_error("forward: a GroupNorm weight has not been set");
            return SOLA_ERR_WEIGHT;
        }
    SOLA_HIP(hipMemsetAsync(c->guard + 1, 0, sizeof(int), s));
    for (size_t i0 = 0; i0 < norms.size(); i0 += 32)
        SOLA_TRY(launch_norm_range_check(norms.data() + i0, (int)std::min<size_t>(32, norms.size() - i0), c->guard + 1, s));
    c->lin16_dirty = false;
    return SOLA_OK;
}

int sola_refresh_conv_weights(SolaCtx* c, int fmt, bool force, hipStream_t s) {
    if (!force && !c->ws_dirty && !c->ws_every_forward && (fmt == 0 || c->ws16_fmt == fmt)) return SOLA_OK;
    WsLayer layers[6];
    for (int i = 0; i < 6; ++i) {
        const std::string nm = "short_motion_encoder." + std::to_string(kConvIdx[i]) + ".weight";
        layers[i] = WsLayer{ctx_weight(c, nm), c->ws_buf + c->ws_off[i], c->conv[i].cout, c->conv[i].cin, c->conv[i].k};
    }
    SOLA_TRY(launch_ws_standardize(layers, 6, s));
    c->ws16_fmt = 0;
    for (int i = 0; i < 6 && fmt != 0; ++i) {
        const int kc = c->conv[i].k * c->conv[i].cin;
        const float* w = c->ws_buf + c->ws_off[i];
        if (fmt == 1) SOLA_TRY(launch_cast_sp16(w, kc, c->ws16_buf + c->ws_off[i], kc, c->conv[i].cout, kc, 1.f, s));
        else SOLA_TRY(launch_cast_f16(w, kc, reinterpret_cast<_Float16*>(c->ws16_buf) + c->ws_off[i], kc, c->conv[i].cout, kc, 1.f, nullptr, s, 13,
                                      nullptr, fmt == 3 ? 1 : 0));
    }
    c->ws_dirty = false;
    c->ws16_fmt = fmt;
    return SOLA_OK;
}

int sola_check_forward_args(const SolaCtx* c, const char* who, size_t need, const void* workspace, size_t ws_bytes) {
    for (const Weight& w : c->weights)
        if (!w.ptr) {
            sola_set_error("%s: weight '%s' has not been set", who, w.name.c_str());
            return SOLA_ERR_WEIGHT;
        }
    if (ws_bytes < need) {
        sola_set_error("%s: workspace %zu bytes < required %zu", who, ws_bytes, need);
        return SOLA_ERR_WORKSPACE;
    }
    SOLA_ARG((reinterpret_cast<uintptr_t>(workspace) & 255) == 0, "%s: workspace must be 256-byte aligned", who);
    return SOLA_OK;
}

int g_attn_split_min_keys = 96;

int g_lang_shared_neg = 1;

int launch_attention_f16(const AttnDesc& d, hipStream_t s);

int sola_forward_infer_impl(SolaCtx* c, const float* obj, const float* lang, int B, int N, int T, int L, float* score_map,
                            float* score_tokens, void* workspace, size_t ws_bytes, hipStream_t s) {
    SOLA_ARG(c && obj && lang && score_map && score_tokens && workspace, "forward: null argument");
    SOLA_ARG(B > 0 && N > 0 && T > 0 && L >= 1, "forward: bad sizes B=%d N=%d T=%d L=%d", B, N, T, L);
    const bool sp = c->precision == 1;
    const bool h16 = c->precision == 2;
    if (sp)
        SOLA_ARG(c->cfg.object_token_dim % 8 == 0 && (c->cfg.lang_token_dim / c->cfg.n_groups_module) % 8 == 0 &&
                     (2 * c->cfg.object_token_dim / c->cfg.n_groups) % 8 == 0 && (c->cfg.lang_token_dim / c->cfg.n_groups) % 8 == 0,
                 "split-f16 mode needs channel counts per GroupNorm group that are multiples of 8");
    if (h16)
        SOLA_ARG(c->cfg.object_token_dim % 64 == 0 && c->cfg.lang_token_dim % 64 == 0,
                 "16-bit storage mode needs object_token_dim and lang_token_dim to be multiples of 64");
    Plan p = make_plan(c, B, N, T, L, false);
    SOLA_TRY(sola_check_forward_args(c, "forward", p.total, workspace, ws_bytes));
    char* base = static_cast<char*>(workspace);
    auto buf = [&](const std::string& name) { return reinterpret_cast<float*>(base + p.bufs.at(name).off); };
    float* const splitk_ws = (!h16 && p.bufs.count("splitk")) ? buf("splitk") : nullptr;
    const size_t splitk_bytes = splitk_ws ? (size_t)p.bufs.at("splitk").rows * p.bufs.at("splitk").cols * sizeof(float) : 0;
    auto W = [&](const std::string& name) { return ctx_weight(c, name); };
    const int D = c->cfg.lang_token_dim, H = c->cfg.num_heads, DH = D / H, d_in = c->cfg.object_token_dim;
    const int Tp = p.Tp, M = p.M, Wn = p.W;
    const int R = B * N;
    int* const guard = (sp || h16) ? c->guard : nullptr;
    auto ws_w = [&](int i) -> const float* {
        if (h16) return reinterpret_cast<const float*>(reinterpret_cast<const _Float16*>(c->ws16_buf) + c->ws_off[i]);
        return sp ? c->ws16_buf + c->ws_off[i] : c->ws_buf + c->ws_off[i];
    };
    auto lin_w = [&](const std::string& an, const char* proj_name, int layer, int attn, int proj) -> const float* {
        const size_t idx = (size_t)(layer * 3 + attn) * 4 + proj;
        if (sp) return c->lin16_buf + idx * D * D;
        if (h16) return reinterpret_cast<const float*>(reinterpret_cast<const _Float16*>(c->lin16_buf) + idx * D * D);
        return W(an + "." + proj_name + ".weight");
    };
    auto lin_inv = [&](int layer, int attn, int proj) -> const float* { return (sp || h16) ? c->lin_inv_scale(layer, attn, proj) : nullptr; };

    SOLA_TRY(sola_refresh_conv_weights(c, sp ? 1 : (h16 ? 2 : 0), false, s));
    if (sp || h16) {
        SOLA_TRY(sola_refresh_lin16(c, s));
        SOLA_HIP(hipMemsetAsync(c->guard, 0, sizeof(int), s));
    } else {
        c->x16.clear();
        c->x16_used = 0;
        c->x16_need = 0;
    }

    const float* x = obj;
    if (sp) SOLA_TRY(launch_cast_sp16_auto(obj, d_in, buf("obj_sp"), d_in, (long long)R * T, d_in, c->scal_pair(0), s));
    if (h16) SOLA_TRY(launch_cast_f16(obj, d_in, buf("obj_sp"), d_in, (long long)R * T, d_in, 256.f, c->scal_pair(0), s, 6, c->scal_extra(0)));
    if (sp || h16) x = buf("obj_sp");
    const bool conv5_16 = h16 || (sp && c->conv[5].cout % 8 == 0);
    int t_in = T;
    for (int i = 0; i < 6; ++i) {
        const ConvGeom& g = c->conv[i];
        const std::string cp = "short_motion_encoder." + std::to_string(kConvIdx[i]);
        const bool to16 = i == 5 && conv5_16;
        GemmDesc gd{};
        gd.nprob = 1;
        gd.p[0] = GemmProblem{x, ws_w(i), W(cp + ".bias"), nullptr, to16 ? buf("conv5_sp") : buf("conv" + std::to_string(i))};
        gd.M = R * p.Tl[i]; gd.N = g.cout; gd.K = g.k * g.cin;
        gd.lda = g.cin; gd.ldr = 0; gd.ldc = g.cout;
        gd.conv = g.k > 1 ? 1 : 0;
        gd.T_in = t_in; gd.T_out = p.Tl[i]; gd.stride = g.stride; gd.pad = g.pad; gd.Cin = g.cin;
        if (sp) {
            gd.arith = 1; gd.out_scale = 1.f; gd.c_sp16 = to16 ? 1 : 0; gd.guard = guard;
            if (i == 0) gd.out_scale_dev = c->scal_pair(0) + 1;
        }
        if (h16) {
            gd.arith = 2; gd.out_scale = 1.f; gd.c_f16 = 1; gd.guard = guard;
            if (i == 0) gd.bias_scale_dev = c->scal_extra(0);
        }
        gd.splitk_ws = splitk_ws; gd.splitk_bytes = splitk_bytes;
        bool fused_norm = false;
        if (sp && i < 5) {
            GemmDesc probe = gd;
            probe.c_sp16 = 1;
            if (gemm_gn_fusable(probe, g.cout / c->cfg.n_groups, p.Tl[i])) {
                const std::string np = "short_motion_encoder." + std::to_string(kNormIdx[i]);
                gd.c_sp16 = 1;
                gd.p[0].C = buf("act" + std::to_string(i));
                gd.gn_gamma = W(np + ".weight"); gd.gn_beta = W(np + ".bias");
                gd.gn_tokens = p.Tl[i]; gd.gn_eps = 1e-5f; gd.gn_slope = 0.01f;
                fused_norm = true;
            }
        }
        SOLA_TRY(launch_gemm(gd, s));
        if (i < 5 && !fused_norm) {
            const std::string np = "short_motion_encoder." + std::to_string(kNormIdx[i]);
            GroupNormDesc nd{};
            nd.slice_ws = buf("gn_slots"); nd.slice_ws_bytes = (size_t)p.bufs.at("gn_slots").rows * p.bufs.at("gn_slots").cols * sizeof(float);
            nd.x = buf("conv" + std::to_string(i)); nd.y = buf("act" + std::to_string(i));
            nd.gamma = W(np + ".weight"); nd.beta = W(np + ".bias");
            nd.n_inst = R; nd.inner = 1; nd.outer_stride = p.Tl[i]; nd.inner_stride = 0; nd.tok_stride = 1;
            nd.ntok = p.Tl[i]; nd.C = g.cout; nd.groups = c->cfg.n_groups; nd.eps = 1e-5f; nd.slope = 0.01f; nd.leaky = 1;
            nd.out_sp16 = sp ? 1 : 0; nd.guard = guard;
            if (h16) {
                nd.in_f16 = 1; nd.out_f16 = 1;
                if (i == 0) nd.in_scale_dev = c->scal_pair(0) + 1;
            }
            SOLA_TRY(launch_group_norm(nd, s));
        }
        if (i < 5) x = buf("act" + std::to_string(i));
        t_in = p.Tl[i];
    }
    if (sp && !conv5_16) SOLA_TRY(launch_cast_sp16(buf("conv5"), D, buf("conv5_sp"), D, M, D, 1.f, s));

    SOLA_TRY(launch_pos_encoding(W("positional_encoding_gaussian_matrix"), D, Tp, c->cfg.max_temporal_length, buf("pe"), s));
    bool shared_neg = false;
    if (sp && g_lang_shared_neg && c->cfg.n_negative > 0 && Wn <= g_attn_split_min_keys && (long long)B * L + c->cfg.n_negative >= 1024) {
        AttnDesc probe{};
        probe.G = B; probe.H = H; probe.DH = DH; probe.Sq = N * Tp; probe.Sk = Wn; probe.inner = 1; probe.k_private = L;
        shared_neg = attention_shared_keys_supported(probe);
    }
    const long long lang_rows = shared_neg ? (long long)B * L + c->cfg.n_negative : (long long)B * Wn;
    if (shared_neg) SOLA_TRY(launch_lang_concat_shared(lang, W("negative_token.weight"), buf("lang"), buf("lbar"), B, L, c->cfg.n_negative, D, s));
    else SOLA_TRY(launch_lang_concat(lang, W("negative_token.weight"), buf("lang"), buf("lbar"), B, L, c->cfg.n_negative, D, s));
    if (sp) SOLA_TRY(launch_cast_sp16_auto(buf("lang"), D, buf("lang_sp"), D, lang_rows, D, c->scal_pair(1), s));
    if (h16) SOLA_TRY(launch_cast_f16(buf("lang"), D, buf("lang_sp"), D, lang_rows, D, 1.f, c->scal_pair(1), s, 6));
    const float* const lang_in = (sp || h16) ? buf("lang_sp") : buf("lang");

    const float scale = 1.0f / sqrtf((float)DH);
    auto linear3 = [&](const float* a0, const float* a1, const float* a2, int layer, int attn, int nprob, int rows, float* o0,
                       float* o1, float* o2, int first_proj, int out_sp16, const float* a_inv_scale = nullptr) -> int {
        static const char* pn[3] = {"q_proj", "k_proj", "v_proj"};
        const std::string an = "object_lang_align_layers." + std::to_string(layer) + "." + kAttnLong[attn];
        const float* as[3] = {a0, a1, a2};
        float* os[3] = {o0, o1, o2};
        GemmDesc gd{};
        gd.nprob = nprob;
        for (int j = 0; j < nprob; ++j)
            gd.p[j] = GemmProblem{as[j], lin_w(an, pn[first_proj + j], layer, attn, first_proj + j), W(an + "." + pn[first_proj + j] + ".bias"),
                                  nullptr, os[j], lin_inv(layer, attn, first_proj + j)};
        gd.M = rows; gd.N = D; gd.K = D; gd.lda = D; gd.ldr = 0; gd.ldc = D;
        if (sp) { gd.arith = 1; gd.out_scale = 1.f; gd.out_scale_dev = a_inv_scale; gd.c_sp16 = out_sp16; gd.guard = guard; }
        if (h16) { gd.arith = 2; gd.out_scale = 1.f; gd.out_scale_dev = a_inv_scale; gd.c_f16 = 1; gd.guard = guard; }
        gd.splitk_ws = splitk_ws; gd.splitk_bytes = splitk_bytes;
        return launch_gemm(gd, s);
    };
    auto out_proj = [&](int layer, int attn, const float* resid, int resid_sp16) -> int {
        const std::string an = "object_lang_align_layers." + std::to_string(layer) + "." + kAttnLong[attn];
        GemmDesc gd{};
        gd.nprob = 1;
        gd.p[0] = GemmProblem{buf("attn"), lin_w(an, "out_proj", layer, attn, 3), W(an + ".out_proj.bias"), resid, buf("res"), lin_inv(layer, attn, 3)};
        gd.M = M; gd.N = D; gd.K = D; gd.lda = D; gd.ldr = D; gd.ldc = D;
        if (sp) { gd.arith = 1; gd.out_scale = 1.f; gd.r_sp16 = resid_sp16; }
        if (h16) { gd.arith = 2; gd.out_scale = 1.f; gd.r_f16 = 1; gd.c_f16 = 1; gd.guard = guard; }
        gd.splitk_ws = splitk_ws; gd.splitk_bytes = splitk_bytes;
        return launch_gemm(gd, s);
    };
    auto gn = [&](const std::string& lp, int idx, float* y, float* y2, int out16, int n_inst, int inner, long long outer,
                  long long inner_stride, long long tok_stride, int ntok) -> int {
        GroupNormDesc nd{};
        nd.slice_ws = buf("gn_slots"); nd.slice_ws_bytes = (size_t)p.bufs.at("gn_slots").rows * p.bufs.at("gn_slots").cols * sizeof(float);
        nd.x = buf("res"); nd.y = y; nd.y2 = y2; nd.pe = y2 ? buf("pe") : nullptr;
        nd.gamma = W(lp + "norm." + std::to_string(idx) + ".weight");
        nd.beta = W(lp + "norm." + std::to_string(idx) + ".bias");
        nd.n_inst = n_inst; nd.inner = inner; nd.outer_stride = outer; nd.inner_stride = inner_stride;
        nd.tok_stride = tok_stride; nd.ntok = ntok; nd.C = D; nd.groups = c->cfg.n_groups_module;
        nd.eps = 1e-5f; nd.slope = 0.f; nd.leaky = 0; nd.guard = guard;
        if (sp) nd.out_sp16 = out16;
        if (h16) { nd.in_f16 = 1; nd.out_f16 = out16; }
        return launch_group_norm(nd, s);
    };
    auto attention = [&](const float* q, const float* k, const float* v, int G, int Sq, int Sk, int inner, long long qo,
                         long long qi, long long qr, long long ko, long long ki, long long kr, int in_sp16, int k_private = 0,
                         long long k_shared_row = 0) -> int {
        AttnDesc ad{q, k, v, buf("attn"), D, D, D, D, G, H, DH, Sq, Sk, inner, qo, qi, qr, ko, ki, kr, scale, nullptr};
        ad.k_private = k_private;
        ad.k_shared_row = k_shared_row;
        ad.o_sp16 = sp ? 1 : 0;
        ad.in_sp16 = in_sp16;
        ad.guard = guard;
        ad.split_math = sp ? 1 : 0;
        return h16 ? launch_attention_f16(ad, s) : launch_attention(ad, s);
    };
    const int obj_sp = (sp && N > g_attn_split_min_keys && N > 16 && DH % 16 == 0) ? 1 : 0;
    const int mot_sp = (sp && Tp > g_attn_split_min_keys && Tp > 16 && DH % 16 == 0) ? 1 : 0;
    const int o2l_sp = (sp && Wn > g_attn_split_min_keys && DH % 16 == 0) ? 1 : 0;

    const float* xin = (sp || h16) ? buf("conv5_sp") : buf("conv5");
    const float* xres = conv5_16 ? buf("conv5_sp") : buf("conv5");
    int xres_sp = conv5_16 ? 1 : 0;
    for (int l = 0; l < c->cfg.n_layers; ++l) {
        const std::string lp = "object_lang_align_layers." + std::to_string(l) + ".";
        const std::string ls = "l" + std::to_string(l);
        const bool last = l + 1 == c->cfg.n_layers;
        float *q = buf("q"), *k = buf("k"), *v = buf("v");
        float* x_obj = buf(ls + "_obj");
        float* x_pe = buf(ls + "_xpe");
        float* x_mot = buf(ls + "_motion");
        float* x_o2l = buf(ls + "_o2l");
        SOLA_TRY(linear3(xin, xin, xin, l, 0, 3, M, q, k, v, 0, obj_sp));
        SOLA_TRY(attention(q, k, v, B * Tp, N, N, Tp, (long long)N * Tp, 1, Tp, (long long)N * Tp, 1, Tp, obj_sp));
        SOLA_TRY(out_proj(l, 0, xres, xres_sp));
        SOLA_TRY(gn(lp, 0, x_obj, x_pe, 1, B * Tp, Tp, (long long)N * Tp, 1, Tp, N));
        SOLA_TRY(linear3(x_pe, x_pe, x_obj, l, 1, 3, M, q, k, v, 0, mot_sp));
        SOLA_TRY(attention(q, k, v, B * N, Tp, Tp, 1, (long long)Tp, 0, 1, (long long)Tp, 0, 1, mot_sp));
        SOLA_TRY(out_proj(l, 1, x_obj, 1));
        SOLA_TRY(gn(lp, 1, x_mot, nullptr, 1, B * N, 1, Tp, 0, 1, Tp));
        SOLA_TRY(linear3(x_mot, nullptr, nullptr, l, 2, 1, M, q, nullptr, nullptr, 0, o2l_sp));
        SOLA_TRY(linear3(lang_in, lang_in, nullptr, l, 2, 2, (int)lang_rows, buf("lk"), buf("lv"), nullptr, 1, o2l_sp, c->scal_pair(1) + 1));
        if (shared_neg) SOLA_TRY(attention(q, buf("lk"), buf("lv"), B, N * Tp, Wn, 1, (long long)N * Tp, 0, 1, (long long)L, 0, 1, o2l_sp, L, (long long)B * L));
        else SOLA_TRY(attention(q, buf("lk"), buf("lv"), B, N * Tp, Wn, 1, (long long)N * Tp, 0, 1, (long long)Wn, 0, 1, o2l_sp));
        SOLA_TRY(out_proj(l, 2, x_mot, 1));
        SOLA_TRY(gn(lp, 2, x_o2l, nullptr, last ? 0 : 1, B, 1, (long long)N * Tp, 0, 1, N * Tp));
        xin = x_o2l;
        xres = x_o2l;
        xres_sp = 1;
    }

    HeadDesc hd{xin, buf("lbar"), score_map, score_tokens, B, N, Tp, D};
    SOLA_TRY(launch_score_head(hd, s));
    c->last = p;
    c->last_obj = nullptr;
    return SOLA_OK;
}
```

sola_amd/csrc/head.hip:

```cpp
#include "kernels.h"

namespace {

struct HeadArgs {
    const float* x;
    const float* lbar;
    float* score_map;
    float* score_tokens;
    int N, Tp, D;
    const int4* units;
};

__global__ __launch_bounds__(256) void score_head_kernel(const HeadArgs a) {
    extern __shared__ float sh[];
    float* logits = sh;
    float* red = sh + ((a.Tp + 3) & ~3);
    const int bn = blockIdx.x;
    int b = bn / a.N, Tp = a.Tp;
    long long row0 = (long long)bn * a.Tp;
    if (a.units) {
        const int4 u = a.units[bn];
        row0 = u.x; Tp = u.z; b = u.w;
    }
    const int d4n = a.D >> 2;
    const float4* xb = reinterpret_cast<const float4*>(a.x + row0 * a.D);
    const float4* lb = reinterpret_cast<const float4*>(a.lbar + (long long)b * a.D);
    const int lane = threadIdx.x & 63, wave = threadIdx.x >> 6;
    for (int t = wave; t < Tp; t += 4) {
        float s = 0.f;
        for (int i = lane; i < d4n; i += 64) {
            const float4 xv = xb[(long long)t * d4n + i], lv = lb[i];
            s += (xv.x * lv.x + xv.y * lv.y) + (xv.z * lv.z + xv.w * lv.w);
        }
        s = wave_sum(s);
        if (lane == 0) logits[t] = s;
    }
    __syncthreads();
    float mx = -INFINITY;
    for (int t = 0; t < Tp; ++t) mx = fmaxf(mx, logits[t]);
    float den = 0.f;
    for (int t = 0; t < Tp; ++t) den += expf(logits[t] - mx);
    __syncthreads();
    for (int t = threadIdx.x; t < Tp; t += 256) logits[t] = expf(logits[t] - mx) / den;
    __syncthreads();
    float part = 0.f;
    float4* out = reinterpret_cast<float4*>(a.score_tokens + (long long)bn * a.D);
    for (int i = threadIdx.x; i < d4n; i += 256) {
        float4 acc = make_float4(0.f, 0.f, 0.f, 0.f);
        for (int t = 0; t < Tp; ++t) {
            const float w = logits[t];
            const float4 xv = xb[(long long)t * d4n + i];
            acc.x += xv.x * w; acc.y += xv.y * w; acc.z += xv.z * w; acc.w += xv.w * w;
        }
        out[i] = acc;
        const float4 lv = lb[i];
        part += (acc.x * lv.x + acc.y * lv.y) + (acc.z * lv.z + acc.w * lv.w);
    }
    const float score = block_sum_256(part, red);
    if (threadIdx.x == 0) a.score_map[bn] = score;
}

struct LossArgs {
    const float *score_map, *score_tokens, *labels, *pos, *neg;
    long long neg_batch_stride;
    int N, D, n_neg;
    float pos_w, temp_scale;
    float* terms;
    int32_t* neg_argmax;
    const int32_t* trk_off;
};
__device__ __forceinline__ void sample_tracks(const LossArgs& a, int b, long long& first, int& count) {
    if (a.trk_off) { first = a.trk_off[b]; count = a.trk_off[b + 1] - a.trk_off[b]; }
    else { first = (long long)b * a.N; count = a.N; }
}

__device__ __forceinline__ float bce_logits(float x, float y) {
    return fmaxf(x, 0.f) - x * y + log1pf(expf(-fabsf(x)));
}

__global__ __launch_bounds__(256) void loss_terms_kernel(const LossArgs a) {
    extern __shared__ float sh[];
    float* negl = sh;
    float* red = sh + ((a.n_neg + 3) & ~3);
    const int bn = blockIdx.x;
    const int b = bn / a.N;
    const int d4n = a.D >> 2;
    const float4* tok = reinterpret_cast<const float4*>(a.score_tokens + (long long)bn * a.D);
    const float4* pos = reinterpret_cast<const float4*>(a.pos + (long long)b * a.D);
    const float* negb = a.neg + (long long)b * a.neg_batch_stride;
    const int lane = threadIdx.x & 63, wave = threadIdx.x >> 6;
    float p = 0.f;
    for (int i = threadIdx.x; i < d4n; i += 256) {
        const float4 tv = tok[i], pv = pos[i];
        p += (tv.x * pv.x + tv.y * pv.y) + (tv.z * pv.z + tv.w * pv.w);
    }
    const float pos_logit = block_sum_256(p, red) * a.temp_scale;
    for (int m = wave; m < a.n_neg; m += 4) {
        const float4* nv = reinterpret_cast<const float4*>(negb + (long long)m * a.D);
        float s = 0.f;
        for (int i = lane; i < d4n; i += 64) {
            const float4 tv = tok[i], v = nv[i];
            s += (tv.x * v.x + tv.y * v.y) + (tv.z * v.z + tv.w * v.w);
        }
        s = wave_sum(s);
        if (lane == 0) negl[m] = s * a.temp_scale;
    }
    __syncthreads();
    if (threadIdx.x == 0) {
        const float y = a.labels[bn];
        const float x = a.score_map[bn];
        const float w = y > 0.f ? a.pos_w : 1.f;
        int arg = 0;
        float best = negl[0];
        for (int m = 1; m < a.n_neg; ++m)
            if (negl[m] > best) { best = negl[m]; arg = m; }
        float neg_sum = 0.f;
        for (int m = 0; m < a.n_neg; ++m) neg_sum += bce_logits(negl[m], m == arg ? (1.f - y) : 0.f);
        a.terms[(long long)bn * 3 + 0] = w * bce_logits(x, y);
        a.terms[(long long)bn * 3 + 1] = bce_logits(pos_logit, y);
        a.terms[(long long)bn * 3 + 2] = neg_sum;
        if (a.neg_argmax) a.neg_argmax[bn] = arg;
    }
}

constexpr int LOSS_RPB = 8;
__global__ __launch_bounds__(256) void loss_terms_rows_kernel(const LossArgs a) {
    extern __shared__ float sh[];
    const int d4n = a.D >> 2;
    float4* tok = reinterpret_cast<float4*>(sh);
    float* logit = sh + (size_t)LOSS_RPB * a.D;
    const int b = blockIdx.y, n0 = blockIdx.x * LOSS_RPB;
    long long first;
    int count;
    sample_tracks(a, b, first, count);
    if (n0 >= count) return;
    const int rows = min(LOSS_RPB, count - n0);
    const int lane = threadIdx.x & 63, wave = threadIdx.x >> 6;
    for (int i = threadIdx.x; i < LOSS_RPB * d4n; i += 256) {
        const int r = i / d4n, c = i - r * d4n;
        tok[i] = r < rows ? reinterpret_cast<const float4*>(a.score_tokens + (first + n0 + r) * a.D)[c]
                          : make_float4(0.f, 0.f, 0.f, 0.f);
    }
    __syncthreads();
    const float* negb = a.neg + (long long)b * a.neg_batch_stride;
    const int stride = a.n_neg + 1;
    for (int m = wave; m <= a.n_neg; m += 4) {
        const float4* vec = reinterpret_cast<const float4*>(m < a.n_neg ? negb + (long long)m * a.D : a.pos + (long long)b * a.D);
        float s[LOSS_RPB];
#pragma unroll
        for (int r = 0; r < LOSS_RPB; ++r) s[r] = 0.f;
        for (int i = lane; i < d4n; i += 64) {
            const float4 v = vec[i];
#pragma unroll
            for (int r = 0; r < LOSS_RPB; ++r) {
                const float4 tv = tok[r * d4n + i];
                s[r] += (tv.x * v.x + tv.y * v.y) + (tv.z * v.z + tv.w * v.w);
            }
        }
#pragma unroll
        for (int r = 0; r < LOSS_RPB; ++r) {
            const float t = wave_sum(s[r]);
            if (lane == 0) logit[r * stride + m] = t * a.temp_scale;
        }
    }
    __syncthreads();
    if (threadIdx.x < rows) {
        const int r = threadIdx.x;
        const long long bn = first + n0 + r;
        const float* negl = logit + r * stride;
        const float y = a.labels[bn];
        const float x = a.score_map[bn];
        const float w = y > 0.f ? a.pos_w : 1.f;
        int arg = 0;
        float best = negl[0];
        for (int m = 1; m < a.n_neg; ++m)
            if (negl[m] > best) { best = negl[m]; arg = m; }
        float neg_sum = 0.f;
        for (int m = 0; m < a.n_neg; ++m) neg_sum += bce_logits(negl[m], m == arg ? (1.f - y) : 0.f);
        a.terms[bn * 3 + 0] = w * bce_logits(x, y);
        a.terms[bn * 3 + 1] = bce_logits(negl[a.n_neg], y);
        a.terms[bn * 3 + 2] = neg_sum;
        if (a.neg_argmax) a.neg_argmax[bn] = arg;
    }
}

template <int NI>
__global__ __launch_bounds__(256) void loss_terms_regs_kernel(const LossArgs a) {
    extern __shared__ float sh[];
    float* logit = sh;
    const int d4n = a.D >> 2;
    const int b = blockIdx.y, n0 = blockIdx.x * LOSS_RPB;
    long long first;
    int count;
    sample_tracks(a, b, first, count);
    if (n0 >= count) return;
    const int rows = min(LOSS_RPB, count - n0);
    const int lane = threadIdx.x & 63, wave = threadIdx.x >> 6;
    float4 tk[LOSS_RPB][NI];
#pragma unroll
    for (int r = 0; r < LOSS_RPB; ++r)
#pragma unroll
        for (int i = 0; i < NI; ++i)
            tk[r][i] = r < rows ? reinterpret_cast<const float4*>(a.score_tokens + (first + n0 + r) * a.D)[lane + 64 * i]
                                : make_float4(0.f, 0.f, 0.f, 0.f);
    const float* negb = a.neg + (long long)b * a.neg_batch_stride;
    const int stride = a.n_neg + 1;
    auto vec_of = [&](int m) { return reinterpret_cast<const float4*>(m < a.n_neg ? negb + (long long)m * a.D : a.pos + (long long)b * a.D); };
    float4 vcur[NI], vnext[NI];
    if (wave <= a.n_neg) {
#pragma unroll
        for (int i = 0; i < NI; ++i) vcur[i] = vec_of(wave)[lane + 64 * i];
    }
    for (int m = wave; m <= a.n_neg; m += 4) {
        if (m + 4 <= a.n_neg) {
#pragma unroll
            for (int i = 0; i < NI; ++i) vnext[i] = vec_of(m + 4)[lane + 64 * i];
        }
        float s[LOSS_RPB];
#pragma unroll
        for (int r = 0; r < LOSS_RPB; ++r) s[r] = 0.f;
#pragma unroll
        for (int i = 0; i < NI; ++i) {
            const float4 v = vcur[i];
#pragma unroll
            for (int r = 0; r < LOSS_RPB; ++r) {
                const float4 tv = tk[r][i];
                s[r] += (tv.x * v.x + tv.y * v.y) + (tv.z * v.z + tv.w * v.w);
            }
        }
#pragma unroll
        for (int i = 0; i < NI; ++i) vcur[i] = vnext[i];
#pragma unroll
        for (int r = 0; r < LOSS_RPB; ++r) {
            const float t = wave_sum(s[r]);
            if (lane == 0) logit[r * stride + m] = t * a.temp_scale;
        }
    }
    (void)d4n;
    __syncthreads();
    if (threadIdx.x < rows) {
        const int r = threadIdx.x;
        const long long bn = first + n0 + r;
        const float* negl = logit + r * stride;
        const float y = a.labels[bn];
        const float x = a.score_map[bn];
        const float w = y > 0.f ? a.pos_w : 1.f;
        int arg = 0;
        float best = negl[0];
        for (int m = 1; m < a.n_neg; ++m)
            if (negl[m] > best) { best = negl[m]; arg = m; }
        float neg_sum = 0.f;
        for (int m = 0; m < a.n_neg; ++m) neg_sum += bce_logits(negl[m], m == arg ? (1.f - y) : 0.f);
        a.terms[bn * 3 + 0] = w * bce_logits(x, y);
        a.terms[bn * 3 + 1] = bce_logits(negl[a.n_neg], y);
        a.terms[bn * 3 + 2] = neg_sum;
        if (a.neg_argmax) a.neg_argmax[bn] = arg;
    }
}

__global__ __launch_bounds__(256) void loss_reduce_kernel(const float* terms, int n, int n_neg, float pos_w,
                                                          float align_w, float* loss3) {
    __shared__ float red[4];
    float s0 = 0.f, s1 = 0.f, s2 = 0.f;
    for (int i = threadIdx.x; i < n; i += 256) {
        s0 += terms[(long long)i * 3 + 0];
        s1 += terms[(long long)i * 3 + 1];
        s2 += terms[(long long)i * 3 + 2];
    }
    s0 = block_sum_256(s0, red);
    s1 = block_sum_256(s1, red);
    s2 = block_sum_256(s2, red);
    if (threadIdx.x == 0) {
        const float bce = s0 / (float)n;
        const float align = pos_w * (s1 / (float)n) + s2 / ((float)n * (float)n_neg);
        loss3[0] = bce + align_w * align;
        loss3[1] = bce;
        loss3[2] = align;
    }
}

__global__ __launch_bounds__(256) void loss_reduce_ragged_kernel(const float* terms, const int32_t* trk_off, int n_neg, float pos_w,
                                                                 float align_w, float* loss3) {
    __shared__ float red[4];
    const int b = blockIdx.x;
    const int first = trk_off[b], n = trk_off[b + 1] - first;
    float s0 = 0.f, s1 = 0.f, s2 = 0.f;
    for (int i = threadIdx.x; i < n; i += 256) {
        s0 += terms[(long long)(first + i) * 3 + 0];
        s1 += terms[(long long)(first + i) * 3 + 1];
        s2 += terms[(long long)(first + i) * 3 + 2];
    }
    s0 = block_sum_256(s0, red);
    s1 = block_sum_256(s1, red);
    s2 = block_sum_256(s2, red);
    if (threadIdx.x == 0) {
        const float bce = s0 / (float)n;
        const float align = pos_w * (s1 / (float)n) + s2 / ((float)n * (float)n_neg);
        loss3[b * 3 + 0] = bce + align_w * align;
        loss3[b * 3 + 1] = bce;
        loss3[b * 3 + 2] = align;
    }
}

__global__ void select_kernel(const float* score, long long n, float thr, float* prob, float* pred) {
    const long long i = (long long)blockIdx.x * blockDim.x + threadIdx.x;
    if (i >= n) return;
    const float p = 1.f / (1.f + expf(-score[i]));
    if (prob) prob[i] = p;
    if (pred) pred[i] = p > thr ? 1.f : 0.f;
}

}

int launch_score_head(const HeadDesc& d, hipStream_t s) {
    SOLA_ARG(d.D % 4 == 0 && d.B > 0 && d.N > 0 && d.Tp > 0, "score_head: bad sizes");
    HeadArgs a{d.x, d.lbar, d.score_map, d.score_tokens, d.N, d.Tp, d.D, d.units};
    const size_t lds = (((size_t)d.Tp + 3) & ~(size_t)3) * 4 + 16;
    SOLA_ARG(lds <= 60000, "score_head: T'=%d too long", d.Tp);
    const double elems = (double)d.B * d.N * d.Tp * d.D;
    SolaProfScope prof(SOLA_PROF_HEAD, s, 4.0 * elems, 4.0 * elems + 4.0 * d.B * d.N * d.D);
    hipLaunchKernelGGL(score_head_kernel, dim3(d.B * d.N), dim3(256), lds, s, a);
    SOLA_LAUNCH_CHECK();
    return SOLA_OK;
}

int launch_loss(const LossDesc& d, hipStream_t s) {
    SOLA_ARG(d.D % 4 == 0 && d.B > 0 && d.N > 0 && d.n_neg > 0 && d.n_neg < 8192, "loss: bad sizes");
    LossArgs a{d.score_map, d.score_tokens, d.labels, d.pos, d.neg, d.neg_batch_stride, d.N, d.D, d.n_neg,
               d.pos_w, d.temp_scale, d.terms, d.neg_argmax, d.trk_off};
    const size_t lds = (((size_t)d.n_neg + 3) & ~(size_t)3) * 4 + 16;
    {
        SolaProfScope prof(SOLA_PROF_HEAD, s, 2.0 * d.B * d.N * (double)d.D * (d.n_neg + 1),
                           4.0 * d.B * d.N * (double)d.D);
        const size_t lds_rows = ((size_t)LOSS_RPB * d.D + (size_t)LOSS_RPB * (d.n_neg + 1)) * 4;
        const size_t lds_logits = (size_t)LOSS_RPB * (d.n_neg + 1) * 4;
        if (d.D == 1024 && lds_logits <= 64 * 1024)
            hipLaunchKernelGGL(loss_terms_regs_kernel<4>, dim3((d.N + LOSS_RPB - 1) / LOSS_RPB, d.B), dim3(256), lds_logits, s, a);
        else if (d.D == 512 && lds_logits <= 64 * 1024)
            hipLaunchKernelGGL(loss_terms_regs_kernel<2>, dim3((d.N + LOSS_RPB - 1) / LOSS_RPB, d.B), dim3(256), lds_logits, s, a);
        else if (lds_rows <= 64 * 1024)
            hipLaunchKernelGGL(loss_terms_rows_kernel, dim3((d.N + LOSS_RPB - 1) / LOSS_RPB, d.B), dim3(256), lds_rows, s, a);
        else {
            SOLA_ARG(!d.trk_off, "loss: ragged batches need D and n_neg that fit the row kernels' LDS");
            hipLaunchKernelGGL(loss_terms_kernel, dim3(d.B * d.N), dim3(256), lds, s, a);
        }
        SOLA_LAUNCH_CHECK();
    }
    {
        SolaProfScope prof(SOLA_PROF_HEAD, s, 0, 12.0 * d.B * d.N);
        if (d.trk_off)
            hipLaunchKernelGGL(loss_reduce_ragged_kernel, dim3(d.B), dim3(256), 0, s, d.terms, d.trk_off, d.n_neg, d.pos_w, d.align_w, d.loss3);
        else
            hipLaunchKernelGGL(loss_reduce_kernel, dim3(1), dim3(256), 0, s, d.terms, d.B * d.N, d.n_neg, d.pos_w, d.align_w, d.loss3);
        SOLA_LAUNCH_CHECK();
    }
    return SOLA_OK;
}

int launch_select(const float* score, long long n, float thr, float* prob, float* pred, hipStream_t s) {
    SOLA_ARG(n > 0, "select: n=%lld", n);
    SolaProfScope prof(SOLA_PROF_HEAD, s, 0, 12.0 * n);
    hipLaunchKernelGGL(select_kernel, dim3((unsigned)((n + 255) / 256)), dim3(256), 0, s, score, n, thr, prob, pred);
    SOLA_LAUNCH_CHECK();
    return SOLA_OK;
}
```

sola_amd/csrc/kernels.h:

```cpp
#pragma once
#include "common.h"

struct GemmProblem {
    const float* A;
    const float* W;
    const float* bias;
    const float* R;
    float* C;
    const float* scale_dev;
};
struct GemmDesc {
    GemmProblem p[3];
    int nprob;
    int M, N, K;
    int lda, ldr, ldc;
    int conv;
    int T_in, T_out, stride, pad, Cin;
    const int2* rowmap;
    int arith;
    float out_scale;
    int ksplit;
    const float* out_scale_dev;
    int r_sp16;
    int c_sp16;
// ... 82 lines not shown
int launch_splitk_reduce_bf16(const void* part, int ksplit, int nprob, float* const* C, int M, int N, int ldc, const float* out_scale_dev,
                              const float* scale_dev, hipStream_t s);
bool gemm_tn_tr_supported(int M, int N, int K, long long lda, long long ldb);
void gemm_tn_tr_geometry(int M, int N, int K, int nprob, int max_ranges, int& ksplit, int& kper);
int launch_gemm_tn_tr(const GemmTnTrDesc& d, hipStream_t s);
int launch_splitk_reduce(const float* part, int ksplit, int nprob, float* const* C, int M, int N, int ldc, const float* out_scale_dev,
                         const float* scale_dev, hipStream_t s);

int launch_transpose(const float* in, float* out, int rows, int cols, int ldi, int ldo, int col_off, hipStream_t s);
int launch_transpose_cast(const float* in, void* out, int rows, int cols, int ldi, int ldo, int col_off, float scale, int fmt, hipStream_t s);
size_t colsum_scratch_bytes(int segments, int seg_rows, int cols);
int launch_colsum(const float* in, float* out, int segments, int seg_rows, int cols, int ld, float scale, int accumulate,
                  float* scratch, size_t scratch_bytes, hipStream_t s);
int launch_colsum_pair(const float* in0, const float* in1, float* out0, float* out1, int seg_rows, int cols, int ld, float* scratch,
                       size_t scratch_bytes, hipStream_t s);
struct ColsumPairGroupDesc {
    const float* in0[16];
    const float* in1[16];
    float* out0[16];
    float* out1[16];
    int rows[16], cols[16];
    int n;
};
int launch_colsum_pair_group(const ColsumPairGroupDesc& d, hipStream_t s);
struct ColsumJobsDesc {
    const float* in[48];
    float* out[48];
    int rows[48], cols[48], ld[48];
    int n;
};
int launch_colsum_jobs(const ColsumJobsDesc& d, hipStream_t s);

struct AttnDesc {
    const float *q, *k, *v;
    float* o;
    int ldq, ldk, ldv, ldo;
    int G, H, DH, Sq, Sk, inner;
    long long q_outer, q_inner, q_rs;
    long long k_outer, k_inner, k_rs;
    float scale;
    float* lse;
    DropoutCfg drop;
    int o_sp16;
    int in_sp16;
    int in_bf16 = 0;
    int* guard;
    const int4 *q_units, *k_units;
    int split_math;
    int k_private = 0;
    long long k_shared_row = 0;
    void* o_cast = nullptr;
    void* o_side = nullptr;
    int o_cast_fmt = 0;
    bool* o_cast_done = nullptr;
};
int launch_attention(const AttnDesc& d, hipStream_t s);
bool attention_in_bf16_supported(const AttnDesc& d);
bool attention_bf16_mfma_supported(const AttnDesc& d);
bool attention_shared_keys_supported(const AttnDesc& d);

struct AttnBwdDesc {
    const float *q, *k, *v, *o, *dout, *lse;
    float *dq, *dk, *dv, *dvec;
    int ldq, ldk, ldv, ldo;
    int ld_dq, ld_dk, ld_dv;
    int G, H, DH, Sq, Sk, inner;
    long long q_outer, q_inner, q_rs;
    long long k_outer, k_inner, k_rs;
    float scale;
    DropoutCfg drop;
    const int4 *q_units, *k_units;
    float* part = nullptr;
    size_t part_floats = 0;
    long long part_rows = 0;
    int io_bf16 = 0;
    void *dq16 = nullptr, *dk16 = nullptr, *dv16 = nullptr;
    int dout_bf16 = 0;
    int o_bf16 = 0;
};
bool attention_bwd_dout_bf16_enabled();
int launch_attention_bwd(const AttnBwdDesc& d, hipStream_t s);
bool attention_bwd_bf16_supported(const AttnBwdDesc& d);
size_t attention_bwd_part_floats(long long q_rows, int G, int H, int Sk);

struct GroupNormBwdDesc {
    const float* x;
    const float* dy;
    const float* dy2;
    const float *gamma, *beta;
    float* dx;
    float* dgamma_part;
    float* dbeta_part;
    int n_inst, inner;
    long long outer_stride, inner_stride, tok_stride;
    int ntok, C, groups;
    float eps, slope;
    int leaky;
    DropoutCfg drop;
    const int4* units;
    void* dx16 = nullptr;
    int x_bf16 = 0;
    const void* stats_in = nullptr;
    int dy2_bf16 = 0;
};
int launch_group_norm_bwd(const GroupNormBwdDesc& d, hipStream_t s);
bool group_norm_bwd_dy2_bf16_supported(int ntok, int C, int groups);
struct WsBwdLayer {
    const float* w;
    const float* dwstd;
    float* dw;
    int cout, cin, k;
};
int launch_ws_backward(const WsBwdLayer* layers, int n_layers, hipStream_t s);
struct HeadBwdDesc {
    const float *x, *lbar, *d_score, *d_tok;
    float* dx;
    float* dlbar_part;
    int B, N, Tp, D;
    const int4* units;
};
int launch_score_head_bwd(const HeadBwdDesc& d, hipStream_t s);
struct LossBwdDesc {
    const float *score_map, *score_tokens, *labels, *pos, *neg;
    long long neg_batch_stride;
    int B, N, D, n_neg;
    float pos_w, temp_scale, align_w;
    const float* g3;
    float* d_score;
    float* d_tok;
    float* coef;
    float* d_neg;
    const int32_t* trk_off;
    long long total_tracks;
};
int launch_loss_bwd(const LossBwdDesc& d, hipStream_t s);
int launch_neg_token_grad(const float* d_lang, const float* dlbar, const float* d_neg_align, float* d_negw, int B, int L,
                          int n_neg, int D, hipStream_t s, const int4* units = nullptr);
int launch_segsum_rows(const float* in, float* out, const int32_t* off, int segments, int cols, hipStream_t s);

size_t mt_sqnorm_scratch_bytes(int n, const long long* numel);
int launch_mt_sqnorm(const float* const* ptrs, const long long* numel, const int* group, int n, int n_groups, double* out,
                     void* scratch, size_t scratch_bytes, hipStream_t s);
int launch_mt_clip(float* const* ptrs, const long long* numel, int n, const double* total_sq, float max_norm, hipStream_t s);
size_t mt_adam_entry_bytes();
void mt_adam_entry_fill(void* host_entry, float* p, float* g, float* m, float* v, float* step, long long numel, int first_block);
int mt_adam_blocks(long long numel);
int launch_mt_clip_adamw(const void* tab_dev, int n, int blocks, double bytes, const double* total_sq, float max_norm, double lr, double beta1, double beta2,
                         double eps, double weight_decay, float step, int write_back, int* ticket, hipStream_t s);

struct WsLayer {
    const float* w;
    float* out;
    int cout, cin, k;
};
int launch_ws_standardize(const WsLayer* layers, int n_layers, hipStream_t s);

struct GroupNormDesc {
    const float* x;
    float* y;
    float* y2;
    const float* pe;
    const float *gamma, *beta;
    int n_inst, inner;
    long long outer_stride, inner_stride, tok_stride;
    int ntok, C, groups;
    float eps, slope;
    int leaky;
    DropoutCfg drop;
    int out_sp16;
    int* guard;
    const int4* units;
    int in_f16, out_f16;
    const float* in_scale_dev;
    void* slice_ws;
    size_t slice_ws_bytes;
    void* y_cast = nullptr;
    void* y2_cast = nullptr;
    int cast_fmt = 0;
    void* stats_out = nullptr;
    int* stats_written = nullptr;
};
int launch_group_norm(const GroupNormDesc& d, hipStream_t s);
int launch_cast_sp16(const float* in, int ld_in, float* out, int ld_out, long long rows, int K, float scale, hipStream_t s, void* side16 = nullptr);
int launch_amax_accumulate(const float* in, int ld_in, long long rows, int K, float* scal, hipStream_t s);
int launch_amax_colsum(const float* in, int ld_in, long long rows, int K, float* scal, float* part, hipStream_t s);
int launch_cast_bf16_colsum(const float* in, int ld_in, void* out, int ld_out, long long rows, int K, float* scal, float* part, hipStream_t s);
int launch_colsum_slabs_bf16(const void* in, int ld_in, long long rows, int K, float* scal, float* part, hipStream_t s);
int launch_cast_sp16_scaled(const float* in, int ld_in, float* out, int ld_out, long long rows, int K, float* scal, hipStream_t s);
int launch_cast_sp16_auto(const float* in, int ld_in, float* out, int ld_out, long long rows, int K, float* scal, hipStream_t s);
int launch_cast_sp16_auto_multi(const float* const* in, float* const* out, int n, int rows, int K, float* scal, hipStream_t s);
int launch_cast_f16(const float* in, int ld_in, void* out, int ld_out, long long rows, int K, float scale, float* scal, hipStream_t s,
                    int target_exp = 13, float* scale_out = nullptr, int bf16 = 0);
int launch_cast_f16_auto_multi(const float* const* in, void* const* out, int n, int rows, int K, float* scal, hipStream_t s, int bf16 = 0);
int launch_cast_f16_scaled(const float* in, int ld_in, void* out, int ld_out, long long rows, int K, float* scal, hipStream_t s, int bf16 = 0);
int launch_cast_f16_t(const float* in, int ld_in, void* out, long long ld_out, int rows, int cols, float* scal, hipStream_t s, int bf16 = 0);
struct NormPair { const float *gamma, *beta; int C; };
int launch_norm_range_check(const NormPair* norms, int n, int* guard, hipStream_t s);
int launch_pos_encoding(const float* gauss, int D, int t_len, int max_len, float* pe, hipStream_t s);
int launch_lang_concat(const float* lang, const float* neg, float* out, float* lbar, int B, int L, int n_neg, int D,
                       hipStream_t s);
int launch_lang_concat_shared(const float* lang, const float* neg, float* out, float* lbar, int B, int L, int n_neg, int D, hipStream_t s);
int launch_lang_concat_ragged(const float* lang, const float* neg, float* out, float* lbar, int B, const int4* units, int n_neg,
                              int D, hipStream_t s);
int launch_gather_rows(const float* src, float* dst, const int4* list, int n, int row_floats, long long total_rows, hipStream_t s);

struct HeadDesc {
    const float* x;
    const float* lbar;
    float* score_map;
    float* score_tokens;
    int B, N, Tp, D;
    const int4* units;
};
int launch_score_head(const HeadDesc& d, hipStream_t s);
struct LossDesc {
    const float *score_map, *score_tokens, *labels, *pos, *neg;
    long long neg_batch_stride;
    int B, N, D, n_neg;
    float pos_w, temp_scale, align_w;
    float* terms;
    float* loss3;
    int32_t* neg_argmax;
    const int32_t* trk_off;
};
int launch_loss(const LossDesc& d, hipStream_t s);
int launch_select(const float* score, long long n, float thr, float* prob, float* pred, hipStream_t s);

bool launch_mask_pack_pair(const void* a_masks, int P, uint32_t* a_bits, long long* a_area, const void* b_masks, int R, uint32_t* b_bits,
                           long long* b_area, size_t area_span_bytes, int H, int W, hipStream_t s, int* status);
int launch_mask_pack(const void* masks, int elem_type, int n, int h, int w, int H, int W, uint32_t* bits,
                     long long* area, hipStream_t s);
int launch_mask_pair(const uint32_t* a_bits, const long long* a_area, int P, int T, const uint32_t* b_bits,
                     const long long* b_area, int R, const int32_t* a_frame, long long words, long long* inter,
                     long long* uni, hipStream_t s);

int launch_mask_bilinear_pack(const void* masks, int elem_type, int n, int h, int w, int H, int W, uint32_t* bits,
                              long long* area, hipStream_t s);
int launch_mask_unpack(const uint32_t* bits, int n, int H, int W, void* out, int elem_type, hipStream_t s);
int launch_rle_fill_or(const uint32_t* cum, const long long* off, int n_frames, int K, int h, int w, uint8_t* out,
                       uint32_t* bits, long long* area, hipStream_t s);

size_t rle_encode_scratch_bytes(int n, int h, int w);
int launch_rle_encode_runs(const void* masks, int elem_type, int n, int h, int w, long long* run_off, void* scratch,
                           size_t scratch_bytes, hipStream_t s);
int launch_rle_encode_cum(const void* masks, int elem_type, int n, int h, int w, const long long* run_off, uint32_t* cum,
                          long long* char_off, void* scratch, size_t scratch_bytes, hipStream_t s);
int launch_rle_encode_chars(const uint32_t* cum, const long long* run_off, const long long* char_off, int n, char* chars,
                            hipStream_t s);

size_t png_deflate_scratch_bytes(int n, int h, int w);
int launch_png_deflate_sizes(const void* masks, int elem_type, int n, int h, int w, long long* byte_off, uint32_t* adler,
                             void* scratch, size_t scratch_bytes, hipStream_t s);
int launch_png_deflate_write(const void* masks, int elem_type, int n, int h, int w, const long long* byte_off,
                             const uint32_t* adler, uint8_t* bytes, void* scratch, size_t scratch_bytes, hipStream_t s);
```

sola_amd/csrc/norm.hip:

```cpp
#include <algorithm>

#include <map>
#include <mutex>
#include <utility>

#include "kernels.h"

namespace {

constexpr int WS_MAX_LAYERS = 8;
constexpr int WS_MAX_PER_THREAD = 16;
struct WsArgs {
    WsLayer layer[WS_MAX_LAYERS];
    int first_block[WS_MAX_LAYERS + 1];
    int n_layers;
};

__global__ __launch_bounds__(256) void ws_standardize_kernel(const WsArgs a) {
    __shared__ float red[4];
    int li = 0;
    while (li + 1 < a.n_layers && (int)blockIdx.x >= a.first_block[li + 1]) ++li;
    const WsLayer L = a.layer[li];
    const int co = blockIdx.x - a.first_block[li];
    const int n = L.cin * L.k;
    const float* w = L.w + (long long)co * n;
    float v[WS_MAX_PER_THREAD];
    float s = 0.f;
#pragma unroll
    for (int i = 0; i < WS_MAX_PER_THREAD; ++i) {
        const int idx = threadIdx.x + 256 * i;
        v[i] = idx < n ? w[idx] : 0.f;
        s += v[i];
    }
    const float mean = block_sum_256(s, red) / (float)n;
    float q = 0.f;
#pragma unroll
    for (int i = 0; i < WS_MAX_PER_THREAD; ++i) {
        const int idx = threadIdx.x + 256 * i;
        const float c = idx < n ? v[i] - mean : 0.f;
        v[i] = c;
        q += c * c;
    }
    const float var = block_sum_256(q, red) / (float)(n - 1);
    const float denom = sqrtf(var) + 1e-5f;
    float* out = L.out + (long long)co * n;
#pragma unroll
    for (int i = 0; i < WS_MAX_PER_THREAD; ++i) {
        const int idx = threadIdx.x + 256 * i;
        if (idx < n) {
            const int ci = idx / L.k, kk = idx - ci * L.k;
            out[kk * L.cin + ci] = v[i] / denom;
        }
    }
}

struct GnArgs {
    const float* x;
    float* y;
    float* y2;
    const float* pe;
    const float *gamma, *beta;
    int inner;
    long long outer_stride, inner_stride, tok_stride;
    int ntok, C, cg, groups;
    float eps, slope;
    int leaky;
    DropoutCfg drop;
    int out_sp16;
    int* guard;
    const int4* units;
    int in_f16, out_f16;
    const float* in_scale_dev;
    void *y_cast, *y2_cast;
    int cast_fmt;
    float2* stats_out;
};

typedef _Float16 half4n __attribute__((ext_vector_type(4)));
__device__ __forceinline__ float4 gn_load(const GnArgs& a, long long off) {
    float4 v;
    if (a.in_f16 == 2) {
        const uint2 w = *reinterpret_cast<const uint2*>(reinterpret_cast<const unsigned short*>(a.x) + off);
        v = make_float4(__builtin_bit_cast(float, w.x << 16), __builtin_bit_cast(float, w.x & 0xffff0000u),
                        __builtin_bit_cast(float, w.y << 16), __builtin_bit_cast(float, w.y & 0xffff0000u));
    } else if (a.in_f16) {
        const half4n h = *reinterpret_cast<const half4n*>(reinterpret_cast<const _Float16*>(a.x) + off);
        v = make_float4((float)h[0], (float)h[1], (float)h[2], (float)h[3]);
    } else {
        v = *reinterpret_cast<const float4*>(a.x + off);
    }
    if (a.in_scale_dev) {
        const float sc = *a.in_scale_dev;
        v.x *= sc; v.y *= sc; v.z *= sc; v.w *= sc;
    }
    return v;
}

template <int R>
__device__ __forceinline__ void gn_load_slots(const GnArgs& a, float4 (&v)[R], long long row0, long long tok_stride, int ntok, int t_first, int tpp, int ch) {
    const float sc = a.in_scale_dev ? *a.in_scale_dev : 1.f;
    if (a.in_f16 == 2) {
        const unsigned short* x = reinterpret_cast<const unsigned short*>(a.x);
        uint2 h[R];
#pragma unroll
        for (int r = 0; r < R; ++r) {
            const int t = t_first + r * tpp;
            h[r] = *reinterpret_cast<const uint2*>(x + (row0 + (long long)(t < ntok ? t : 0) * tok_stride) * a.C + ch);
        }
#pragma unroll
        for (int r = 0; r < R; ++r) {
            const bool ok = t_first + r * tpp < ntok;
            v[r] = make_float4(ok ? __builtin_bit_cast(float, h[r].x << 16) * sc : 0.f, ok ? __builtin_bit_cast(float, h[r].x & 0xffff0000u) * sc : 0.f,
                               ok ? __builtin_bit_cast(float, h[r].y << 16) * sc : 0.f, ok ? __builtin_bit_cast(float, h[r].y & 0xffff0000u) * sc : 0.f);
        }
    } else if (a.in_f16) {
        const _Float16* x = reinterpret_cast<const _Float16*>(a.x);
        half4n h[R];
#pragma unroll
        for (int r = 0; r < R; ++r) {
            const int t = t_first + r * tpp;
            h[r] = *reinterpret_cast<const half4n*>(x + (row0 + (long long)(t < ntok ? t : 0) * tok_stride) * a.C + ch);
        }
#pragma unroll
        for (int r = 0; r < R; ++r) {
            const bool ok = t_first + r * tpp < ntok;
            v[r] = make_float4(ok ? (float)h[r][0] * sc : 0.f, ok ? (float)h[r][1] * sc : 0.f, ok ? (float)h[r][2] * sc : 0.f, ok ? (float)h[r][3] * sc : 0.f);
        }
    } else {
#pragma unroll
        for (int r = 0; r < R; ++r) {
            const int t = t_first + r * tpp;
            v[r] = *reinterpret_cast<const float4*>(a.x + (row0 + (long long)(t < ntok ? t : 0) * tok_stride) * a.C + ch);
        }
#pragma unroll
        for (int r = 0; r < R; ++r) {
            const bool ok = t_first + r * tpp < ntok;
            v[r] = make_float4(ok ? v[r].x * sc : 0.f, ok ? v[r].y * sc : 0.f, ok ? v[r].z * sc : 0.f, ok ? v[r].w * sc : 0.f);
        }
    }
}

struct GnUnit { long long row0, tok_stride; int ntok, pe_row; };
__device__ __forceinline__ GnUnit gn_unit(const GnArgs& a, int inst) {
    GnUnit u;
    if (a.units) {
        const int4 d = a.units[inst];
        u.row0 = d.x; u.tok_stride = d.y; u.ntok = d.z; u.pe_row = d.w;
    } else {
        u.row0 = (long long)(inst / a.inner) * a.outer_stride + (long long)(inst % a.inner) * a.inner_stride;
        u.tok_stride = a.tok_stride; u.ntok = a.ntok; u.pe_row = inst % a.inner;
    }
    return u;
}

typedef _Float16 half8 __attribute__((ext_vector_type(8)));

__device__ __forceinline__ void gn_apply_store(const GnArgs& a, long long off, const float4 v, float mean, float rstd, const float4 ga,
                                               const float4 be, const float4 pe, int c4) {
    float4 o;
    o.x = (v.x - mean) * rstd * ga.x + be.x;
    o.y = (v.y - mean) * rstd * ga.y + be.y;
    o.z = (v.z - mean) * rstd * ga.z + be.z;
    o.w = (v.w - mean) * rstd * ga.w + be.w;
    if (a.leaky) {
        o.x = o.x >= 0.f ? o.x : o.x * a.slope;
        o.y = o.y >= 0.f ? o.y : o.y * a.slope;
        o.z = o.z >= 0.f ? o.z : o.z * a.slope;
        o.w = o.w >= 0.f ? o.w : o.w * a.slope;
    }
    if (a.drop.enabled) {
        o.x = dropout_keep(a.drop, (unsigned long long)off) ? o.x * a.drop.scale : 0.f;
        o.y = dropout_keep(a.drop, (unsigned long long)off + 1) ? o.y * a.drop.scale : 0.f;
        o.z = dropout_keep(a.drop, (unsigned long long)off + 2) ? o.z * a.drop.scale : 0.f;
        o.w = dropout_keep(a.drop, (unsigned long long)off + 3) ? o.w * a.drop.scale : 0.f;
    }
    if (a.out_f16) {
        if (off < 0) return;
        half4n h;
        h[0] = (_Float16)o.x; h[1] = (_Float16)o.y; h[2] = (_Float16)o.z; h[3] = (_Float16)o.w;
        *reinterpret_cast<half4n*>(reinterpret_cast<_Float16*>(a.y) + off) = h;
        if (a.y2) {
            h[0] = (_Float16)(o.x + pe.x); h[1] = (_Float16)(o.y + pe.y); h[2] = (_Float16)(o.z + pe.z); h[3] = (_Float16)(o.w + pe.w);
            *reinterpret_cast<half4n*>(reinterpret_cast<_Float16*>(a.y2) + off) = h;
        }
        if (a.guard && !(fmaxf(fmaxf(fabsf(o.x), fabsf(o.y)), fmaxf(fabsf(o.z), fabsf(o.w))) < 65000.f)) atomicOr(a.guard, 1);
        return;
    }
    if (a.out_sp16) {
        const float4 o2 = make_float4(o.x + pe.x, o.y + pe.y, o.z + pe.z, o.w + pe.w);
        const float4 n = make_float4(__shfl_xor(o.x, 1, 64), __shfl_xor(o.y, 1, 64), __shfl_xor(o.z, 1, 64), __shfl_xor(o.w, 1, 64));
        const float4 n2 = make_float4(__shfl_xor(o2.x, 1, 64), __shfl_xor(o2.y, 1, 64), __shfl_xor(o2.z, 1, 64), __shfl_xor(o2.w, 1, 64));
        if ((c4 & 1) == 0 && off >= 0) {
            const float v8[8] = {o.x, o.y, o.z, o.w, n.x, n.y, n.z, n.w};
            half8 hi, lo;
#pragma unroll
            for (int j = 0; j < 8; ++j) { _Float16 h1, l1; split_f16(v8[j], h1, l1); hi[j] = h1; lo[j] = l1; }
            half8* dst = reinterpret_cast<half8*>(a.y + off);
            dst[0] = hi; dst[1] = lo;
            if (a.guard) {
                float m = 0.f;
#pragma unroll
                for (int j = 0; j < 8; ++j) m = fmaxf(m, fabsf(v8[j]));
                if (!(m < 65000.f)) atomicOr(a.guard, 1);
            }
            if (a.y2) {
                const float w8[8] = {o2.x, o2.y, o2.z, o2.w, n2.x, n2.y, n2.z, n2.w};
#pragma unroll
                for (int j = 0; j < 8; ++j) { _Float16 h1, l1; split_f16(w8[j], h1, l1); hi[j] = h1; lo[j] = l1; }
                half8* dst2 = reinterpret_cast<half8*>(a.y2 + off);
                dst2[0] = hi; dst2[1] = lo;
            }
        }
        return;
    }
    if (a.cast_fmt >= 2 && off >= 0) {
        const bool bf = a.cast_fmt == 3;
        auto cv = [&](float x) -> _Float16 { return bf ? __builtin_bit_cast(_Float16, (__bf16)x) : (_Float16)x; };
        half4n h;
        if (a.y_cast) {
            h[0] = cv(o.x); h[1] = cv(o.y); h[2] = cv(o.z); h[3] = cv(o.w);
            *reinterpret_cast<half4n*>(static_cast<_Float16*>(a.y_cast) + off) = h;
        }
        if (a.y2_cast) {
            h[0] = cv(o.x + pe.x); h[1] = cv(o.y + pe.y); h[2] = cv(o.z + pe.z); h[3] = cv(o.w + pe.w);
            *reinterpret_cast<half4n*>(static_cast<_Float16*>(a.y2_cast) + off) = h;
        }
    }
    if (off < 0) return;
    *reinterpret_cast<float4*>(a.y + off) = o;
    if (a.y2) *reinterpret_cast<float4*>(a.y2 + off) = make_float4(o.x + pe.x, o.y + pe.y, o.z + pe.z, o.w + pe.w);
}

__global__ __launch_bounds__(256) void group_norm_kernel(const GnArgs a) {
    __shared__ float red[4];
    const int inst = (int)(blockIdx.x / a.groups), g = (int)(blockIdx.x % a.groups);
    const int f4 = a.cg >> 2;
    const int lpt = f4;
    const int tpp = 256 / lpt;
    const int tl = threadIdx.x / lpt;
    const int c4 = threadIdx.x - tl * lpt;
    const GnUnit un = gn_unit(a, inst);
    const long long row0 = un.row0, tok_stride = un.tok_stride;
    const int ntok = un.ntok;
    const int ch = g * a.cg + c4 * 4;
    const bool active = tl < tpp;
    const float cnt = (float)ntok * (float)a.cg;

    float s = 0.f;
    if (active)
        for (int t = tl; t < ntok; t += tpp) {
            const float4 v = gn_load(a, (row0 + (long long)t * tok_stride) * a.C + ch);
            s += (v.x + v.y) + (v.z + v.w);
        }
    const float mean = block_sum_256(s, red) / cnt;
    float q = 0.f;
    if (active)
        for (int t = tl; t < ntok; t += tpp) {
            const float4 v = gn_load(a, (row0 + (long long)t * tok_stride) * a.C + ch);
            const float d0 = v.x - mean, d1 = v.y - mean, d2 = v.z - mean, d3 = v.w - mean;
            q += (d0 * d0 + d1 * d1) + (d2 * d2 + d3 * d3);
        }
    const float var = block_sum_256(q, red) / cnt;
    const float rstd = 1.0f / sqrtf(var + a.eps);
    if (!active) return;
    const float4 ga = *reinterpret_cast<const float4*>(a.gamma + ch);
    const float4 be = *reinterpret_cast<const float4*>(a.beta + ch);
    float4 pe = make_float4(0.f, 0.f, 0.f, 0.f);
    if (a.y2) pe = *reinterpret_cast<const float4*>(a.pe + (long long)un.pe_row * a.C + ch);
    for (int t = tl; t < ntok; t += tpp) {
        const long long off = (row0 + (long long)t * tok_stride) * a.C + ch;
        gn_apply_store(a, off, gn_load(a, off), mean, rstd, ga, be, pe, c4);
    }
}

template <int NTHR>
__device__ __forceinline__ float block_sum_n(float v, float* red) {
    if (NTHR == 256) return block_sum_256(v, red);
    v = wave_sum(v);
    __syncthreads();
    if ((threadIdx.x & 63) == 0) red[threadIdx.x >> 6] = v;
    __syncthreads();
    float t = 0.f;
#pragma unroll
    for (int i = 0; i < NTHR / 64; ++i) t += red[i];
    return t;
}

template <int R, bool WAVE, int NTHR = 256>
__global__ __launch_bounds__(NTHR) void group_norm_reg_kernel(const GnArgs a, long long n_units) {
    __shared__ float red[NTHR / 64];
    const int f4 = a.cg >> 2;
    const int nthr = WAVE ? 64 : NTHR;
    const int tid = WAVE ? (threadIdx.x & 63) : threadIdx.x;
    const long long unit = WAVE ? (long long)blockIdx.x * 4 + (threadIdx.x >> 6) : (long long)blockIdx.x;
    if (WAVE && unit >= n_units) return;
    const int inst = (int)(unit / a.groups), g = (int)(unit - (long long)inst * a.groups);
    const int tpp = nthr / f4;
    const int tl = tid / f4, c4 = tid - tl * f4;
    const GnUnit un = gn_unit(a, inst);
    const long long row0 = un.row0, tok_stride = un.tok_stride;
    const int ntok = un.ntok;
    const int ch = g * a.cg + c4 * 4;
    const float cnt = (float)ntok * (float)a.cg;
    const float4 ga = *reinterpret_cast<const float4*>(a.gamma + ch);
    const float4 be = *reinterpret_cast<const float4*>(a.beta + ch);
    float4 pe = make_float4(0.f, 0.f, 0.f, 0.f);
    if (a.y2) pe = *reinterpret_cast<const float4*>(a.pe + (long long)un.pe_row * a.C + ch);
    float4 v[R];
    gn_load_slots<R>(a, v, row0, tok_stride, ntok, tl, tpp, ch);
    float s = 0.f;
#pragma unroll
    for (int r = 0; r < R; ++r) s += (v[r].x + v[r].y) + (v[r].z + v[r].w);
    const float mean = (WAVE ? wave_sum(s) : block_sum_n<NTHR>(s, red)) / cnt;
    float q = 0.f;
#pragma unroll
    for (int r = 0; r < R; ++r) {
        if (tl + r * tpp < ntok) {
            const float d0 = v[r].x - mean, d1 = v[r].y - mean, d2 = v[r].z - mean, d3 = v[r].w - mean;
            q += (d0 * d0 + d1 * d1) + (d2 * d2 + d3 * d3);
        }
    }
    const float var = (WAVE ? wave_sum(q) : block_sum_n<NTHR>(q, red)) / cnt;
    const float rstd = 1.0f / sqrtf(var + a.eps);
#pragma unroll
    for (int r = 0; r < R; ++r) {
        const int t = tl + r * tpp;
        const long long off = t < ntok ? (row0 + (long long)t * tok_stride) * a.C + ch : -1;
        gn_apply_store(a, off, v[r], mean, rstd, ga, be, pe, c4);
    }
}

template <int R, bool WAVE, int NTHR = 256>
__global__ __launch_bounds__(NTHR) void group_norm_reg_h8_kernel(const GnArgs a, long long n_units) {
    __shared__ float red[NTHR / 64];
    const int f8 = a.cg >> 3;
    const int nthr = WAVE ? 64 : NTHR;
    const int tid = WAVE ? (threadIdx.x & 63) : threadIdx.x;
    const long long unit = WAVE ? (long long)blockIdx.x * 4 + (threadIdx.x >> 6) : (long long)blockIdx.x;
    if (WAVE && unit >= n_units) return;
    const int inst = (int)(unit / a.groups), g = (int)(unit - (long long)inst * a.groups);
    const int tpp = nthr / f8;
    const int tl = tid / f8, c8 = tid - tl * f8;
    const GnUnit un = gn_unit(a, inst);
    const long long row0 = un.row0, tok_stride = un.tok_stride;
    const int ntok = un.ntok;
    const int ch = g * a.cg + c8 * 8;
    const float cnt = (float)ntok * (float)a.cg;
    const float sc_in = a.in_scale_dev ? *a.in_scale_dev : 1.f;
    const _Float16* x16 = reinterpret_cast<const _Float16*>(a.x);
    float v[R][8];
    float s = 0.f;
#pragma unroll
    for (int r = 0; r < R; ++r) {
        const int t = tl + r * tpp;
        const bool ok = t < ntok;
        const half8 h = *reinterpret_cast<const half8*>(x16 + (row0 + (long long)(ok ? t : 0) * tok_stride) * a.C + ch);
#pragma unroll
        for (int e = 0; e < 8; ++e) v[r][e] = ok ? (float)h[e] * sc_in : 0.f;
        s += ((v[r][0] + v[r][1]) + (v[r][2] + v[r][3])) + ((v[r][4] + v[r][5]) + (v[r][6] + v[r][7]));
    }
    const float mean = (WAVE ? wave_sum(s) : block_sum_n<NTHR>(s, red)) / cnt;
    float q = 0.f;
#pragma unroll
    for (int r = 0; r < R; ++r)
        if (tl + r * tpp < ntok) {
#pragma unroll
            for (int e = 0; e < 8; ++e) {
                const float d = v[r][e] - mean;
                q += d * d;
            }
        }
    const float var = (WAVE ? wave_sum(q) : block_sum_n<NTHR>(q, red)) / cnt;
    const float rstd = 1.0f / sqrtf(var + a.eps);
    float ga[8], be[8], pe[8];
    {
        const float4 g0 = *reinterpret_cast<const float4*>(a.gamma + ch), g1 = *reinterpret_cast<const float4*>(a.gamma + ch + 4);
        const float4 b0 = *reinterpret_cast<const float4*>(a.beta + ch), b1 = *reinterpret_cast<const float4*>(a.beta + ch + 4);
        ga[0] = g0.x; ga[1] = g0.y; ga[2] = g0.z; ga[3] = g0.w; ga[4] = g1.x; ga[5] = g1.y; ga[6] = g1.z; ga[7] = g1.w;
        be[0] = b0.x; be[1] = b0.y; be[2] = b0.z; be[3] = b0.w; be[4] = b1.x; be[5] = b1.y; be[6] = b1.z; be[7] = b1.w;
#pragma unroll
        for (int e = 0; e < 8; ++e) pe[e] = 0.f;
        if (a.y2) {
            const float4 p0 = *reinterpret_cast<const float4*>(a.pe + (long long)un.pe_row * a.C + ch);
            const float4 p1 = *reinterpret_cast<const float4*>(a.pe + (long long)un.pe_row * a.C + ch + 4);
            pe[0] = p0.x; pe[1] = p0.y; pe[2] = p0.z; pe[3] = p0.w; pe[4] = p1.x; pe[5] = p1.y; pe[6] = p1.z; pe[7] = p1.w;
        }
    }
    float m = 0.f;
    _Float16* y16 = reinterpret_cast<_Float16*>(a.y);
    _Float16* y216 = reinterpret_cast<_Float16*>(a.y2);
#pragma unroll
    for (int r = 0; r < R; ++r) {
        const int t = tl + r * tpp;
        if (t < ntok) {
            const long long off = (row0 + (long long)t * tok_stride) * a.C + ch;
            half8 h, h2;
#pragma unroll
            for (int e = 0; e < 8; ++e) {
                float o = (v[r][e] - mean) * rstd * ga[e] + be[e];
                if (a.leaky) o = o >= 0.f ? o : o * a.slope;
                h[e] = (_Float16)o;
                h2[e] = (_Float16)(o + pe[e]);
                m = fmaxf(m, fabsf(o));
            }
            *reinterpret_cast<half8*>(y16 + off) = h;
            if (a.y2) *reinterpret_cast<half8*>(y216 + off) = h2;
        }
    }
    if (a.guard && !(m < 65000.f)) atomicOr(a.guard, 1);
}

constexpr int GNC_R = 32;
struct GncGeo { long long row0, tok_stride, unit; int ntok, pe_row, g, inst, t0, tl, c4, tpp, nslice, sl; };
__device__ __forceinline__ GncGeo gnc_geo(const GnArgs& a, int S) {
    GncGeo q;
    const long long rest = blockIdx.x / a.groups;
    q.g = (int)(blockIdx.x - rest * a.groups);
    q.inst = (int)(rest / S);
    const int sl = (int)(rest - (long long)q.inst * S);
    q.sl = sl;
    q.unit = (long long)q.inst * a.groups + q.g;
    const int f4 = a.cg >> 2;
    const GnUnit un = gn_unit(a, q.inst);
    q.row0 = un.row0; q.tok_stride = un.tok_stride; q.ntok = un.ntok; q.pe_row = un.pe_row;
    q.tpp = 256 / f4;
    q.tl = threadIdx.x / f4; q.c4 = threadIdx.x - q.tl * f4;
    const int ts = q.tpp * GNC_R;
    q.nslice = (q.ntok + ts - 1) / ts;
    q.t0 = sl < q.nslice ? sl * ts : -1;
    return q;
}
__global__ __launch_bounds__(256) void group_norm_slice_stats_kernel(const GnArgs a, int S, float2* __restrict__ slots) {
    __shared__ float red[4];
    const GncGeo q = gnc_geo(a, S);
    if (q.t0 < 0) return;
    const int ch = q.g * a.cg + q.c4 * 4;
    float4 v[GNC_R];
    gn_load_slots<GNC_R>(a, v, q.row0, q.tok_stride, q.ntok, q.t0 + q.tl, q.tpp, ch);
    float s = 0.f;
#pragma unroll
    for (int r = 0; r < GNC_R; ++r) s += (v[r].x + v[r].y) + (v[r].z + v[r].w);
    const int ntok_i = min(q.ntok - q.t0, q.tpp * GNC_R);
    const float mean = block_sum_256(s, red) / ((float)ntok_i * (float)a.cg);
    float m2 = 0.f;
#pragma unroll
    for (int r = 0; r < GNC_R; ++r)
        if (q.t0 + q.tl + r * q.tpp < q.ntok) {
            const float d0 = v[r].x - mean, d1 = v[r].y - mean, d2 = v[r].z - mean, d3 = v[r].w - mean;
            m2 += (d0 * d0 + d1 * d1) + (d2 * d2 + d3 * d3);
        }
    m2 = block_sum_256(m2, red);
    if (threadIdx.x == 0) slots[q.unit * S + q.sl] = make_float2(mean, m2);
}
__global__ __launch_bounds__(256) void group_norm_slice_apply_kernel(const GnArgs a, int S, const float2* __restrict__ slots) {
    const GncGeo q = gnc_geo(a, S);
    if (q.t0 < 0) return;
    const int ts = q.tpp * GNC_R;
    const long long unit = q.unit;
    float mean = 0.f;
    const float ntot = (float)q.ntok * (float)a.cg;
    float m2 = 0.f;
    if (q.nslice <= 64) {
        const int li = threadIdx.x & 63;
        const float2 mine = li < q.nslice ? slots[unit * S + li] : make_float2(0.f, 0.f);
        for (int i = 0; i < q.nslice; ++i) mean += __shfl(mine.x, i, 64) * ((float)min(q.ntok - i * ts, ts) * (float)a.cg / ntot);
        for (int i = 0; i < q.nslice; ++i) {
            const float d = __shfl(mine.x, i, 64) - mean;
            m2 += __shfl(mine.y, i, 64) + (float)min(q.ntok - i * ts, ts) * (float)a.cg * d * d;
        }
    } else {
        for (int i = 0; i < q.nslice; ++i) mean += slots[unit * S + i].x * ((float)min(q.ntok - i * ts, ts) * (float)a.cg / ntot);
        for (int i = 0; i < q.nslice; ++i) {
            const float2 sm = slots[unit * S + i];
            const float d = sm.x - mean;
            m2 += sm.y + (float)min(q.ntok - i * ts, ts) * (float)a.cg * d * d;
        }
    }
    const float rstd = 1.0f / sqrtf(m2 / ntot + a.eps);
    if (a.stats_out && q.sl == 0 && threadIdx.x == 0) a.stats_out[unit] = make_float2(mean, rstd);
    const int ch = q.g * a.cg + q.c4 * 4;
    const float4 ga = *reinterpret_cast<const float4*>(a.gamma + ch);
    const float4 be = *reinterpret_cast<const float4*>(a.beta + ch);
    float4 pe = make_float4(0.f, 0.f, 0.f, 0.f);
    if (a.y2) pe = *reinterpret_cast<const float4*>(a.pe + (long long)q.pe_row * a.C + ch);
    constexpr int CH = 8;
    for (int c = 0; c < GNC_R / CH; ++c) {
        const int tf = q.t0 + q.tl + c * CH * q.tpp;
        if (tf - q.tl >= q.ntok) break;
        float4 v[CH];
        gn_load_slots<CH>(a, v, q.row0, q.tok_stride, q.ntok, tf, q.tpp, ch);
#pragma unroll
        for (int r = 0; r < CH; ++r) {
            const int t = tf + r * q.tpp;
            const long long off = t < q.ntok ? (q.row0 + (long long)t * q.tok_stride) * a.C + ch : -1;
            gn_apply_store(a, off, v[r], mean, rstd, ga, be, pe, q.c4);
        }
    }
}

__global__ void pos_encoding_kernel(const float* __restrict__ gauss, int half, int t_len, float max_len, float* pe) {
    const int i = blockIdx.x * blockDim.x + threadIdx.x;
    if (i >= t_len * half) return;
    const int t = i / half, j = i - t * half;
    const float arg = ((float)t / max_len) * gauss[j] * 6.283185307179586f;
    pe[(long long)t * 2 * half + j] = sinf(arg);
    pe[(long long)t * 2 * half + half + j] = cosf(arg);
}

__global__ void lang_concat_kernel(const float* __restrict__ lang, const float* __restrict__ neg, float* __restrict__ out,
                                   float* __restrict__ lbar, int B, int L, int n_neg, int D) {
    const int d4 = D >> 2;
    const int i = blockIdx.x * blockDim.x + threadIdx.x;
    if (i >= B * d4) return;
    const int b = i / d4, c = (i - b * d4) * 4;
    const int W = L + n_neg;
    float4 acc = make_float4(0.f, 0.f, 0.f, 0.f);
    for (int w0 = 0; w0 < W; w0 += 8) {
        float4 v[8];
#pragma unroll
        for (int j = 0; j < 8; ++j) {
            const int w = min(w0 + j, W - 1);
            v[j] = w < L ? *reinterpret_cast<const float4*>(lang + ((long long)b * L + w) * D + c)
                         : *reinterpret_cast<const float4*>(neg + (long long)(w - L) * D + c);
        }
#pragma unroll
        for (int j = 0; j < 8; ++j) {
            if (w0 + j < W) {
                *reinterpret_cast<float4*>(out + ((long long)b * W + w0 + j) * D + c) = v[j];
                acc.x += v[j].x; acc.y += v[j].y; acc.z += v[j].z; acc.w += v[j].w;
            }
        }
    }
    const float inv = 1.f / (float)W;
    *reinterpret_cast<float4*>(lbar + (long long)b * D + c) = make_float4(acc.x * inv, acc.y * inv, acc.z * inv, acc.w * inv);
}

__global__ void lang_concat_shared_kernel(const float* __restrict__ lang, const float* __restrict__ neg, float* out, float* lbar, int B, int L,
                                          int n_neg, int D) {
    const int d4 = D >> 2;
    const int i = blockIdx.x * blockDim.x + threadIdx.x;
    if (i >= B * d4) return;
    const int b = i / d4, c = (i - b * d4) * 4;
    const int W = L + n_neg;
    float4 acc = make_float4(0.f, 0.f, 0.f, 0.f);
    for (int w = 0; w < W; ++w) {
        const float4 v = w < L ? *reinterpret_cast<const float4*>(lang + ((long long)b * L + w) * D + c)
                               : *reinterpret_cast<const float4*>(neg + (long long)(w - L) * D + c);
        if (w < L) *reinterpret_cast<float4*>(out + ((long long)b * L + w) * D + c) = v;
        else if (b == 0) *reinterpret_cast<float4*>(out + ((long long)B * L + (w - L)) * D + c) = v;
        acc.x += v.x; acc.y += v.y; acc.z += v.z; acc.w += v.w;
    }
    const float inv = 1.f / (float)W;
    *reinterpret_cast<float4*>(lbar + (long long)b * D + c) = make_float4(acc.x * inv, acc.y * inv, acc.z * inv, acc.w * inv);
}

__global__ void lang_concat_ragged_kernel(const float* __restrict__ lang, const float* __restrict__ neg, float* out, float* lbar,
                                          int B, const int4* __restrict__ units, int n_neg, int D) {
    const int d4 = D >> 2;
    const int i = blockIdx.x * blockDim.x + threadIdx.x;
    if (i >= B * d4) return;
    const int b = i / d4, c = (i - b * d4) * 4;
    const int4 u = units[b];
    const int L = u.y, W = L + n_neg;
    float4 acc = make_float4(0.f, 0.f, 0.f, 0.f);
    for (int w = 0; w < W; ++w) {
        const float4 v = w < L ? *reinterpret_cast<const float4*>(lang + ((long long)u.x + w) * D + c)
                               : *reinterpret_cast<const float4*>(neg + (long long)(w - L) * D + c);
        *reinterpret_cast<float4*>(out + ((long long)u.z + w) * D + c) = v;
        acc.x += v.x; acc.y += v.y; acc.z += v.z; acc.w += v.w;
    }
    const float inv = 1.f / (float)W;
    *reinterpret_cast<float4*>(lbar + (long long)b * D + c) = make_float4(acc.x * inv, acc.y * inv, acc.z * inv, acc.w * inv);
}

__global__ __launch_bounds__(256) void gather_rows_kernel(const float* __restrict__ src, float* __restrict__ dst,
                                                          const int4* __restrict__ list, int row_f4) {
    const int4 e = list[blockIdx.y];
    const long long n = (long long)e.z * row_f4;
    const float4* s4 = reinterpret_cast<const float4*>(src) + (long long)e.y * row_f4;
    float4* d4 = reinterpret_cast<float4*>(dst) + (long long)e.x * row_f4;
    for (long long i = (long long)blockIdx.x * 256 + threadIdx.x; i < n; i += (long long)gridDim.x * 256) d4[i] = s4[i];
}

}

int launch_lang_concat_shared(const float* lang, const float* neg, float* out, float* lbar, int B, int L, int n_neg, int D, hipStream_t s) {
    SOLA_ARG(D % 4 == 0 && B > 0 && L > 0 && n_neg >= 0, "lang_concat_shared: bad arguments");
    SolaProfScope prof(SOLA_PROF_MISC, s, 0, 4.0 * ((double)B * (2.0 * L + n_neg) + n_neg) * D);
    const int total = B * (D >> 2);
    hipLaunchKernelGGL(lang_concat_shared_kernel, dim3((total + 255) / 256), dim3(256), 0, s, lang, neg, out, lbar, B, L, n_neg, D);
    SOLA_LAUNCH_CHECK();
    return SOLA_OK;
}

int launch_lang_concat_ragged(const float* lang, const float* neg, float* out, float* lbar, int B, const int4* units, int n_neg,
                              int D, hipStream_t s) {
    SOLA_ARG(D % 4 == 0 && B > 0 && n_neg >= 0 && units, "lang_concat_ragged: bad arguments");
    const int n = B * (D / 4);
    SolaProfScope prof(SOLA_PROF_MISC, s, 0, 0);
    hipLaunchKernelGGL(lang_concat_ragged_kernel, dim3((n + 255) / 256), dim3(256), 0, s, lang, neg, out, lbar, B, units, n_neg, D);
    SOLA_LAUNCH_CHECK();
    return SOLA_OK;
}

int launch_gather_rows(const float* src, float* dst, const int4* list, int n, int row_floats, long long total_rows, hipStream_t s) {
    SOLA_ARG(src && dst && list && n > 0 && row_floats % 4 == 0, "gather_rows: bad arguments");
    SolaProfScope prof(SOLA_PROF_MISC, s, 0, 8.0 * total_rows * row_floats);
    const long long per = (total_rows / n + 1) * (row_floats / 4);
    const unsigned bx = (unsigned)std::max<long long>(1, std::min<long long>(64, (per + 1023) / 1024));
    hipLaunchKernelGGL(gather_rows_kernel, dim3(bx, n), dim3(256), 0, s, src, dst, list, row_floats / 4);
    SOLA_LAUNCH_CHECK();
    return SOLA_OK;
}

int launch_ws_standardize(const WsLayer* layers, int n_layers, hipStream_t s) {
    SOLA_ARG(n_layers >= 1 && n_layers <= WS_MAX_LAYERS, "ws: %d layers", n_layers);
    WsArgs a;
    a.n_layers = n_layers;
    int blocks = 0;
    double elems = 0;
    for (int i = 0; i < n_layers; ++i) {
        SOLA_ARG(layers[i].cin * layers[i].k <= 256 * WS_MAX_PER_THREAD && layers[i].cin * layers[i].k >= 2,
                 "ws: cin*k = %d unsupported (2..%d)", layers[i].cin * layers[i].k, 256 * WS_MAX_PER_THREAD);
        a.layer[i] = layers[i];
        a.first_block[i] = blocks;
        blocks += layers[i].cout;
        elems += (double)layers[i].cout * layers[i].cin * layers[i].k;
    }
    a.first_block[n_layers] = blocks;
    SolaProfScope prof(SOLA_PROF_WS, s, 6.0 * elems, 8.0 * elems);
    hipLaunchKernelGGL(ws_standardize_kernel, dim3(blocks), dim3(256), 0, s, a);
    SOLA_LAUNCH_CHECK();
    return SOLA_OK;
}

int g_gn_variant = 1;
int g_gn_wide = 1;
int g_gn_slices = 1;
static float2* gn_slice_scratch(size_t bytes, hipStream_t s) {
    struct Slot { float2* buf = nullptr; size_t cap = 0; };
    static std::mutex mu;
    static std::map<std::pair<int, hipStream_t>, Slot> table;
    int dev = 0;
    if (hipGetDevice(&dev) != hipSuccess) return nullptr;
    std::lock_guard<std::mutex> lock(mu);
    Slot& sl = table[std::make_pair(dev, s)];
    if (sl.cap >= bytes) return sl.buf;
    hipStreamCaptureStatus st = hipStreamCaptureStatusNone;
    if (hipStreamIsCapturing(s, &st) != hipSuccess || st != hipStreamCaptureStatusNone) return nullptr;
    if (sl.buf) { (void)hipStreamSynchronize(s); (void)hipFree(sl.buf); sl.buf = nullptr; sl.cap = 0; }
    const size_t want = std::max<size_t>(bytes * 2, (size_t)1 << 20);
    if (hipMalloc(&sl.buf, want) != hipSuccess) { sl.buf = nullptr; return nullptr; }
    sl.cap = want;
    return sl.buf;
}
int g_gn_h8 = 1;

int launch_group_norm(const GroupNormDesc& d, hipStream_t s) {
    SOLA_ARG(d.groups > 0 && d.C % d.groups == 0, "group_norm: C=%d groups=%d", d.C, d.groups);
    const int cg = d.C / d.groups;
    SOLA_ARG(cg % 4 == 0 && cg / 4 <= 256, "group_norm: channels per group %d must be a multiple of 4 and <= 1024", cg);
    SOLA_ARG(d.n_inst > 0 && d.ntok > 0 && d.inner > 0 && d.groups <= 65535, "group_norm: bad sizes");
    SOLA_ARG(d.y2 == nullptr || d.pe != nullptr, "group_norm: y2 needs pe");
    GnArgs a;
    a.x = d.x; a.y = d.y; a.y2 = d.y2; a.pe = d.pe; a.gamma = d.gamma; a.beta = d.beta;
    a.inner = d.inner; a.outer_stride = d.outer_stride; a.inner_stride = d.inner_stride; a.tok_stride = d.tok_stride;
    a.ntok = d.ntok; a.C = d.C; a.cg = cg; a.groups = d.groups; a.eps = d.eps; a.slope = d.slope; a.leaky = d.leaky; a.drop = d.drop; a.out_sp16 = d.out_sp16; a.guard = (d.out_sp16 || d.out_f16) ? d.guard : nullptr; a.units = d.units;
    a.in_f16 = d.in_f16; a.out_f16 = d.out_f16; a.in_scale_dev = d.in_scale_dev;
    a.y_cast = d.y_cast; a.y2_cast = d.y2_cast; a.cast_fmt = (d.y_cast || d.y2_cast) ? d.cast_fmt : 0;
    a.stats_out = static_cast<float2*>(d.stats_out);
    SOLA_ARG(a.cast_fmt == 0 || (!d.out_sp16 && !d.out_f16 && a.cast_fmt >= 2 && a.cast_fmt <= 3 && (!d.y2_cast || d.y2)),
             "group_norm: operand casts go with f32 outputs (format 2 = f16, 3 = bf16)");
    SOLA_ARG(!(d.out_f16 && d.out_sp16), "group_norm: one output format at a time");
    SOLA_ARG(!d.out_sp16 || cg % 8 == 0, "group_norm: split-f16 output needs channels per group %% 8 == 0");
    const double elems = (double)d.n_inst * d.ntok * d.C;
    SolaProfScope prof(SOLA_PROF_NORM, s, 8.0 * elems, (d.y2 ? 12.0 : 8.0) * elems);
    const int f4 = cg / 4;
    const long long n_units = (long long)d.n_inst * d.groups;
    SOLA_ARG(n_units < (1ll << 31), "group_norm: %lld (instance, group) units exceed the grid", n_units);
    const int rw = 64 % f4 == 0 ? (d.ntok + 64 / f4 - 1) / (64 / f4) : 1 << 30;
    const int rb = 256 % f4 == 0 ? (d.ntok + 256 / f4 - 1) / (256 / f4) : 1 << 30;
    const int f8 = cg / 8;
    const bool h8 = g_gn_variant != 0 && g_gn_h8 && d.in_f16 && d.out_f16 && !d.drop.enabled && cg % 8 == 0 && n_units < (1ll << 31);
    const int rw8 = (h8 && 64 % f8 == 0) ? (d.ntok + 64 / f8 - 1) / (64 / f8) : 1 << 30;
    const int rb8 = (h8 && 256 % f8 == 0) ? (d.ntok + 256 / f8 - 1) / (256 / f8) : 1 << 30;
    const int rk8 = (h8 && 1024 % f8 == 0) ? (d.ntok + 1024 / f8 - 1) / (1024 / f8) : 1 << 30;
    if (rw8 <= 2) {
        const dim3 grid((unsigned)((n_units + 3) / 4));
        if (rw8 == 1) hipLaunchKernelGGL((group_norm_reg_h8_kernel<1, true>), grid, dim3(256), 0, s, a, n_units);
        else hipLaunchKernelGGL((group_norm_reg_h8_kernel<2, true>), grid, dim3(256), 0, s, a, n_units);
    } else if (rb8 <= 4) {
        const dim3 grid((unsigned)n_units);
        if (rb8 <= 2) hipLaunchKernelGGL((group_norm_reg_h8_kernel<2, false>), grid, dim3(256), 0, s, a, n_units);
        else hipLaunchKernelGGL((group_norm_reg_h8_kernel<4, false>), grid, dim3(256), 0, s, a, n_units);
    } else if (rk8 <= 4) {
        hipLaunchKernelGGL((group_norm_reg_h8_kernel<4, false, 1024>), dim3((unsigned)n_units), dim3(1024), 0, s, a, n_units);
    } else if (g_gn_variant != 0 && rw <= 4 && n_units < (1ll << 31)) {
        const dim3 grid((unsigned)((n_units + 3) / 4));
        if (rw == 1) hipLaunchKernelGGL((group_norm_reg_kernel<1, true>), grid, dim3(256), 0, s, a, n_units);
        else if (rw == 2) hipLaunchKernelGGL((group_norm_reg_kernel<2, true>), grid, dim3(256), 0, s, a, n_units);
        else hipLaunchKernelGGL((group_norm_reg_kernel<4, true>), grid, dim3(256), 0, s, a, n_units);
    } else if (g_gn_variant != 0 && rb <= 32 && n_units < (1ll << 31)) {
        const dim3 grid((unsigned)n_units);
        if (rb <= 2) hipLaunchKernelGGL((group_norm_reg_kernel<2, false>), grid, dim3(256), 0, s, a, n_units);
        else if (rb <= 4) hipLaunchKernelGGL((group_norm_reg_kernel<4, false>), grid, dim3(256), 0, s, a, n_units);
        else if (rb <= 8) hipLaunchKernelGGL((group_norm_reg_kernel<8, false>), grid, dim3(256), 0, s, a, n_units);
        else if (rb <= 16 || !g_gn_wide || 1024 % f4 != 0) {
            if (rb <= 16) hipLaunchKernelGGL((group_norm_reg_kernel<16, false>), grid, dim3(256), 0, s, a, n_units);
            else hipLaunchKernelGGL((group_norm_reg_kernel<32, false>), grid, dim3(256), 0, s, a, n_units);
        } else {
            hipLaunchKernelGGL((group_norm_reg_kernel<8, false, 1024>), grid, dim3(1024), 0, s, a, n_units);
        }
    } else if (g_gn_variant != 0 && g_gn_slices && 256 % f4 == 0 && n_units < (1ll << 24)) {
        const int ts = (256 / f4) * GNC_R;
        const int S = (d.ntok + ts - 1) / ts;
        const long long blocks = n_units * S;
        float2* slots = (d.slice_ws && d.slice_ws_bytes >= (size_t)blocks * sizeof(float2)) ? static_cast<float2*>(d.slice_ws)
                                                                                         : gn_slice_scratch((size_t)blocks * sizeof(float2), s);
        if (slots && blocks < (1ll << 31)) {
            hipLaunchKernelGGL(group_norm_slice_stats_kernel, dim3((unsigned)blocks), dim3(256), 0, s, a, S, slots);
            SOLA_LAUNCH_CHECK();
            hipLaunchKernelGGL(group_norm_slice_apply_kernel, dim3((unsigned)blocks), dim3(256), 0, s, a, S, slots);
            if (d.stats_out && d.stats_written) *d.stats_written = 1;
        } else {
            hipLaunchKernelGGL(group_norm_kernel, dim3((unsigned)n_units), dim3(256), 0, s, a);
        }
    } else {
        hipLaunchKernelGGL(group_norm_kernel, dim3((unsigned)n_units), dim3(256), 0, s, a);
    }
    SOLA_LAUNCH_CHECK();
    return SOLA_OK;
}

int launch_pos_encoding(const float* gauss, int D, int t_len, int max_len, float* pe, hipStream_t s) {
    SOLA_ARG(D % 2 == 0 && t_len > 0, "pos_encoding: D=%d t_len=%d", D, t_len);
    const int half = D / 2, n = t_len * half;
    SolaProfScope prof(SOLA_PROF_MISC, s, 0, 4.0 * (n * 2 + half));
    hipLaunchKernelGGL(pos_encoding_kernel, dim3((n + 255) / 256), dim3(256), 0, s, gauss, half, t_len, (float)max_len, pe);
    SOLA_LAUNCH_CHECK();
    return SOLA_OK;
}

int launch_lang_concat(const float* lang, const float* neg, float* out, float* lbar, int B, int L, int n_neg, int D,
                       hipStream_t s) {
    SOLA_ARG(D % 4 == 0 && B > 0 && L >= 0 && n_neg >= 0 && L + n_neg > 0, "lang_concat: bad sizes");
    const int n = B * (D / 4);
    SolaProfScope prof(SOLA_PROF_MISC, s, 0, 8.0 * B * (L + n_neg) * D);
    hipLaunchKernelGGL(lang_concat_kernel, dim3((n + 255) / 256), dim3(256), 0, s, lang, neg, out, lbar, B, L, n_neg, D);
    SOLA_LAUNCH_CHECK();
    return SOLA_OK;
}
```

Before: 18880 samples/s.

## Fuse last-layer group norm into score head and weight casts into standardization

The inference forward now computes only the statistics of the final layer's group norm and applies the normalization inside the score head kernel, so the full normalized tensor is never written and re-read. The normalized buffer is rebuilt on demand only when a workspace tap asks for it. Weight standardization also writes the 16-bit operand copies (split-f16, f16 or bf16) directly, which removes six separate cast launches. Both paths are on by default. The score head takes on extra per-element arithmetic, and the deferred tap adds state that must stay consistent across calls.

Result: no change. 19040 samples/s (median of 6 runs) (+0.8%).

```diff
diff --git a/include/sola_hip.h b/include/sola_hip.h
--- a/include/sola_hip.h
+++ b/include/sola_hip.h
@@ -104,6 +104,8 @@
                      int32_t* dev_neg_argmax, void* dev_scratch, size_t scratch_bytes, void* stream);
 
 int sola_workspace_tap(const SolaCtx* ctx, const char* name, size_t* byte_offset, int64_t* rows, int64_t* cols);
+
+int sola_set_lean_ends(int mask);
 
 int sola_loss(const float* dev_score_map, const float* dev_score_tokens,
               const float* dev_labels,
diff --git a/sola_amd/_lib.py b/sola_amd/_lib.py
--- a/sola_amd/_lib.py
+++ b/sola_amd/_lib.py
@@ -78,6 +78,7 @@
     "sola_backward_ragged": (_i, [_vp, _vp, _vp, _vp, _vp, _sz, _vp]),
     "sola_loss_backward_ragged": (_i, [_vp, _vp, _vp, _vp, _vp, _i64, _i, _vp, _i, _i64, _i, _i, _f, _f, _f, _vp, _vp, _vp, _vp, _vp, _sz, _vp]),
     "sola_workspace_tap": (_i, [_vp, C.c_char_p, C.POINTER(_sz), C.POINTER(_i64), C.POINTER(_i64)]),
+    "sola_set_lean_ends": (_i, [_i]),
     "sola_loss": (_i, [_vp, _vp, _vp, _vp, _vp, _i64, _i, _i, _i, _i, _f, _f, _f, _vp, _vp, _vp, _sz, _vp]),
     "sola_select": (_i, [_vp, _i64, _f, _vp, _vp, _vp]),
     "sola_ws_standardize": (_i, [_vp, _i, _i, _i, _vp, _vp]),
diff --git a/sola_amd/csrc/api.hip b/sola_amd/csrc/api.hip
--- a/sola_amd/csrc/api.hip
+++ b/sola_amd/csrc/api.hip
@@ -379,10 +379,23 @@
     SOLA_ARG(c && name, "workspace_tap: null argument");
     auto it = c->last.bufs.find(name);
     SOLA_ARG(it != c->last.bufs.end(), "workspace_tap: no buffer named '%s' (run sola_forward first)", name);
+    if (c->tap_pending && c->tap_name == name) {
+        SolaCtx* m = const_cast<SolaCtx*>(c);
+        SOLA_HIP(hipSetDevice(c->device));
+        SOLA_TRY(launch_group_norm(c->tap_norm, c->tap_stream));
+        m->tap_pending = false;
+    }
     if (off) *off = it->second.off;
     if (rows) *rows = it->second.rows;
     if (cols) *cols = it->second.cols;
     return SOLA_OK;
+}
+
+extern int g_infer_lean_ends;
+extern "C" int sola_set_lean_ends(int mask) {
+    const int before = g_infer_lean_ends;
+    if (mask >= 0) g_infer_lean_ends = mask & 3;
+    return before;
 }
 
 extern "C" int sola_set_precision(SolaCtx* c, int precision) {
diff --git a/sola_amd/csrc/ctx.h b/sola_amd/csrc/ctx.h
--- a/sola_amd/csrc/ctx.h
+++ b/sola_amd/csrc/ctx.h
@@ -69,6 +69,10 @@
     const float* last_obj = nullptr;
     RagTables last_rag;
     const void* last_ws = nullptr;
+    bool tap_pending = false;
+    GroupNormDesc tap_norm{};
+    std::string tap_name;
+    hipStream_t tap_stream = nullptr;
     std::vector<char> qkv16;
     std::vector<char> res16;
     std::vector<char> attn_o16;
diff --git a/sola_amd/csrc/forward.hip b/sola_amd/csrc/forward.hip
--- a/sola_amd/csrc/forward.hip
+++ b/sola_amd/csrc/forward.hip
@@ -38,6 +38,7 @@
         p.add("obj_sp", z.rows0, c->cfg.object_token_dim);
         p.add("conv5_sp", z.M, D);
         p.add("lang_sp", z.BW, D);
+        p.add("gn2_stats", z.S * c->cfg.n_groups_module, 2);
     }
     if (train && c->precision >= 1 && z.M >= g_train_split_min_rows) {
         int64_t amax = std::max<int64_t>(z.rows0 * c->cfg.object_token_dim, std::max<int64_t>(z.M * D, z.BW * D));
@@ -456,6 +457,7 @@
     HeadDesc hd{xin, buf("lbar"), score_map, score_tokens, B, N, Tp, D};
     if (rs) { hd.B = 1; hd.N = rt.sumNS; hd.units = rt.u_strk; }
     SOLA_TRY(launch_score_head(hd, s));
+    c->tap_pending = false;
     c->last = p;
     c->last_rag = rt;
     c->last_ws = workspace;
diff --git a/sola_amd/csrc/forward_infer.hip b/sola_amd/csrc/forward_infer.hip
--- a/sola_amd/csrc/forward_infer.hip
+++ b/sola_amd/csrc/forward_infer.hip
@@ -3,6 +3,8 @@
 #include <algorithm>
 
 #include "ctx.h"
+
+extern int g_infer_lean_ends;
 
 int sola_refresh_lin16(SolaCtx* c, hipStream_t s) {
     if (!c->lin16_dirty) return SOLA_OK;
@@ -59,9 +61,15 @@
         const std::string nm = "short_motion_encoder." + std::to_string(kConvIdx[i]) + ".weight";
         layers[i] = WsLayer{ctx_weight(c, nm), c->ws_buf + c->ws_off[i], c->conv[i].cout, c->conv[i].cin, c->conv[i].k};
     }
+    const bool one_launch = (g_infer_lean_ends & 1) && fmt != 0;
+    for (int i = 0; i < 6 && one_launch; ++i) {
+        layers[i].fmt16 = fmt;
+        if (fmt == 1) layers[i].out16 = c->ws16_buf + c->ws_off[i];
+        else layers[i].out16 = reinterpret_cast<_Float16*>(c->ws16_buf) + c->ws_off[i];
+    }
     SOLA_TRY(launch_ws_standardize(layers, 6, s));
     c->ws16_fmt = 0;
-    for (int i = 0; i < 6 && fmt != 0; ++i) {
+    for (int i = 0; i < 6 && fmt != 0 && !one_launch; ++i) {
         const int kc = c->conv[i].k * c->conv[i].cin;
         const float* w = c->ws_buf + c->ws_off[i];
         if (fmt == 1) SOLA_TRY(launch_cast_sp16(w, kc, c->ws16_buf + c->ws_off[i], kc, c->conv[i].cout, kc, 1.f, s));
@@ -88,6 +96,8 @@
 }
 
 int g_attn_split_min_keys = 96;
+
+int g_infer_lean_ends = 3;
 
 int g_lang_shared_neg = 1;
 
@@ -108,6 +118,7 @@
                  "16-bit storage mode needs object_token_dim and lang_token_dim to be multiples of 64");
     Plan p = make_plan(c, B, N, T, L, false);
     SOLA_TRY(sola_check_forward_args(c, "forward", p.total, workspace, ws_bytes));
+    c->tap_pending = false;
     char* base = static_cast<char*>(workspace);
     auto buf = [&](const std::string& name) { return reinterpret_cast<float*>(base + p.bufs.at(name).off); };
     float* const splitk_ws = (!h16 && p.bufs.count("splitk")) ? buf("splitk") : nullptr;
@@ -275,6 +286,8 @@
     const float* xin = (sp || h16) ? buf("conv5_sp") : buf("conv5");
     const float* xres = conv5_16 ? buf("conv5_sp") : buf("conv5");
     int xres_sp = conv5_16 ? 1 : 0;
+    bool head_norm = false;
+    const float *head_gamma = nullptr, *head_beta = nullptr;
     for (int l = 0; l < c->cfg.n_layers; ++l) {
         const std::string lp = "object_lang_align_layers." + std::to_string(l) + ".";
         const std::string ls = "l" + std::to_string(l);
@@ -297,6 +310,26 @@
         if (shared_neg) SOLA_TRY(attention(q, buf("lk"), buf("lv"), B, N * Tp, Wn, 1, (long long)N * Tp, 0, 1, (long long)L, 0, 1, o2l_sp, L, (long long)B * L));
         else SOLA_TRY(attention(q, buf("lk"), buf("lv"), B, N * Tp, Wn, 1, (long long)N * Tp, 0, 1, (long long)Wn, 0, 1, o2l_sp));
         SOLA_TRY(out_proj(l, 2, x_mot, 1));
+        if (last && sp && (g_infer_lean_ends & 2)) {
+            GroupNormDesc nd{};
+            nd.x = buf("res"); nd.y = x_o2l;
+            nd.gamma = W(lp + "norm.2.weight"); nd.beta = W(lp + "norm.2.bias");
+            nd.n_inst = B; nd.inner = 1; nd.outer_stride = (long long)N * Tp; nd.inner_stride = 0; nd.tok_stride = 1; nd.ntok = N * Tp;
+            nd.C = D; nd.groups = c->cfg.n_groups_module; nd.eps = 1e-5f; nd.slope = 0.f; nd.leaky = 0;
+            nd.slice_ws = buf("gn_slots"); nd.slice_ws_bytes = (size_t)p.bufs.at("gn_slots").rows * p.bufs.at("gn_slots").cols * sizeof(float);
+            nd.stats_out = buf("gn2_stats");
+            if (group_norm_stats_only_supported(nd)) {
+                c->tap_norm = nd;
+                c->tap_norm.stats_out = nullptr;
+                c->tap_name = ls + "_o2l";
+                c->tap_stream = s;
+                nd.stats_only = 1;
+                SOLA_TRY(launch_group_norm(nd, s));
+                head_norm = true;
+                head_gamma = nd.gamma; head_beta = nd.beta;
+                break;
+            }
+        }
         SOLA_TRY(gn(lp, 2, x_o2l, nullptr, last ? 0 : 1, B, 1, (long long)N * Tp, 0, 1, N * Tp));
         xin = x_o2l;
         xres = x_o2l;
@@ -304,7 +337,12 @@
     }
 
     HeadDesc hd{xin, buf("lbar"), score_map, score_tokens, B, N, Tp, D};
+    if (head_norm) {
+        hd.x = buf("res");
+        hd.gn_stats = buf("gn2_stats"); hd.gn_gamma = head_gamma; hd.gn_beta = head_beta; hd.gn_groups = c->cfg.n_groups_module;
+    }
     SOLA_TRY(launch_score_head(hd, s));
+    c->tap_pending = head_norm;
     c->last = p;
     c->last_obj = nullptr;
     return SOLA_OK;
diff --git a/sola_amd/csrc/head.hip b/sola_amd/csrc/head.hip
--- a/sola_amd/csrc/head.hip
+++ b/sola_amd/csrc/head.hip
@@ -9,8 +9,21 @@
     float* score_tokens;
     int N, Tp, D;
     const int4* units;
+    const float2* gn_stats;
+    const float *gn_gamma, *gn_beta;
+    int gn_groups, gn_cg;
 };
 
+__device__ __forceinline__ float4 head_norm4(const float4 v, const float2 st, const float4 ga, const float4 be) {
+    float4 o;
+    o.x = (v.x - st.x) * st.y * ga.x + be.x;
+    o.y = (v.y - st.x) * st.y * ga.y + be.y;
+    o.z = (v.z - st.x) * st.y * ga.z + be.z;
+    o.w = (v.w - st.x) * st.y * ga.w + be.w;
+    return o;
+}
+
+template <bool NORM>
 __global__ __launch_bounds__(256) void score_head_kernel(const HeadArgs a) {
     extern __shared__ float sh[];
     float* logits = sh;
@@ -26,10 +39,15 @@
     const float4* xb = reinterpret_cast<const float4*>(a.x + row0 * a.D);
     const float4* lb = reinterpret_cast<const float4*>(a.lbar + (long long)b * a.D);
     const int lane = threadIdx.x & 63, wave = threadIdx.x >> 6;
+    const float4* ga4 = reinterpret_cast<const float4*>(a.gn_gamma);
+    const float4* be4 = reinterpret_cast<const float4*>(a.gn_beta);
+    const float2* st = NORM ? a.gn_stats + (long long)b * a.gn_groups : nullptr;
     for (int t = wave; t < Tp; t += 4) {
         float s = 0.f;
         for (int i = lane; i < d4n; i += 64) {
-            const float4 xv = xb[(long long)t * d4n + i], lv = lb[i];
+            float4 xv = xb[(long long)t * d4n + i];
+            const float4 lv = lb[i];
+            if (NORM) xv = head_norm4(xv, st[(i * 4) / a.gn_cg], ga4[i], be4[i]);
             s += (xv.x * lv.x + xv.y * lv.y) + (xv.z * lv.z + xv.w * lv.w);
         }
         s = wave_sum(s);
@@ -47,9 +65,13 @@
     float4* out = reinterpret_cast<float4*>(a.score_tokens + (long long)bn * a.D);
     for (int i = threadIdx.x; i < d4n; i += 256) {
         float4 acc = make_float4(0.f, 0.f, 0.f, 0.f);
+        float4 ga = make_float4(0.f, 0.f, 0.f, 0.f), be = ga;
+        float2 sg = make_float2(0.f, 0.f);
+        if (NORM) { ga = ga4[i]; be = be4[i]; sg = st[(i * 4) / a.gn_cg]; }
         for (int t = 0; t < Tp; ++t) {
             const float w = logits[t];
-            const float4 xv = xb[(long long)t * d4n + i];
+            float4 xv = xb[(long long)t * d4n + i];
+            if (NORM) xv = head_norm4(xv, sg, ga, be);
             acc.x += xv.x * w; acc.y += xv.y * w; acc.z += xv.z * w; acc.w += xv.w * w;
         }
         out[i] = acc;
@@ -314,12 +336,17 @@
 
 int launch_score_head(const HeadDesc& d, hipStream_t s) {
     SOLA_ARG(d.D % 4 == 0 && d.B > 0 && d.N > 0 && d.Tp > 0, "score_head: bad sizes");
-    HeadArgs a{d.x, d.lbar, d.score_map, d.score_tokens, d.N, d.Tp, d.D, d.units};
+    const bool norm = d.gn_stats != nullptr;
+    SOLA_ARG(!norm || (!d.units && d.gn_gamma && d.gn_beta && d.gn_groups > 0 && d.D % d.gn_groups == 0 && (d.D / d.gn_groups) % 4 == 0),
+             "score_head: the norm-applying form takes a uniform batch, gamma / beta and groups of a multiple of 4 channels");
+    HeadArgs a{d.x, d.lbar, d.score_map, d.score_tokens, d.N, d.Tp, d.D, d.units, static_cast<const float2*>(d.gn_stats), d.gn_gamma, d.gn_beta,
+               d.gn_groups, norm ? d.D / d.gn_groups : 4};
     const size_t lds = (((size_t)d.Tp + 3) & ~(size_t)3) * 4 + 16;
     SOLA_ARG(lds <= 60000, "score_head: T'=%d too long", d.Tp);
     const double elems = (double)d.B * d.N * d.Tp * d.D;
     SolaProfScope prof(SOLA_PROF_HEAD, s, 4.0 * elems, 4.0 * elems + 4.0 * d.B * d.N * d.D);
-    hipLaunchKernelGGL(score_head_kernel, dim3(d.B * d.N), dim3(256), lds, s, a);
+    if (norm) hipLaunchKernelGGL(score_head_kernel<true>, dim3(d.B * d.N), dim3(256), lds, s, a);
+    else hipLaunchKernelGGL(score_head_kernel<false>, dim3(d.B * d.N), dim3(256), lds, s, a);
     SOLA_LAUNCH_CHECK();
     return SOLA_OK;
 }
diff --git a/sola_amd/csrc/kernels.h b/sola_amd/csrc/kernels.h
--- a/sola_amd/csrc/kernels.h
+++ b/sola_amd/csrc/kernels.h
@@ -258,6 +258,8 @@
     const float* w;
     float* out;
     int cout, cin, k;
+    void* out16 = nullptr;
+    int fmt16 = 0;
 };
 int launch_ws_standardize(const WsLayer* layers, int n_layers, hipStream_t s);
 
@@ -285,8 +287,10 @@
     int cast_fmt = 0;
     void* stats_out = nullptr;
     int* stats_written = nullptr;
+    int stats_only = 0;
 };
 int launch_group_norm(const GroupNormDesc& d, hipStream_t s);
+bool group_norm_stats_only_supported(const GroupNormDesc& d);
 int launch_cast_sp16(const float* in, int ld_in, float* out, int ld_out, long long rows, int K, float scale, hipStream_t s, void* side16 = nullptr);
 int launch_amax_accumulate(const float* in, int ld_in, long long rows, int K, float* scal, hipStream_t s);
 int launch_amax_colsum(const float* in, int ld_in, long long rows, int K, float* scal, float* part, hipStream_t s);
@@ -317,6 +321,9 @@
     float* score_tokens;
     int B, N, Tp, D;
     const int4* units;
+    const void* gn_stats = nullptr;
+    const float *gn_gamma = nullptr, *gn_beta = nullptr;
+    int gn_groups = 0;
 };
 int launch_score_head(const HeadDesc& d, hipStream_t s);
 struct LossDesc {
diff --git a/sola_amd/csrc/norm.hip b/sola_amd/csrc/norm.hip
--- a/sola_amd/csrc/norm.hip
+++ b/sola_amd/csrc/norm.hip
@@ -16,8 +16,12 @@
     int n_layers;
 };
 
+typedef _Float16 ws_half8 __attribute__((ext_vector_type(8)));
+typedef __bf16 ws_bf16x8 __attribute__((ext_vector_type(8)));
+
 __global__ __launch_bounds__(256) void ws_standardize_kernel(const WsArgs a) {
     __shared__ float red[4];
+    __shared__ __attribute__((aligned(16))) float row[256 * WS_MAX_PER_THREAD];
     int li = 0;
     while (li + 1 < a.n_layers && (int)blockIdx.x >= a.first_block[li + 1]) ++li;
     const WsLayer L = a.layer[li];
@@ -49,7 +53,35 @@
         const int idx = threadIdx.x + 256 * i;
         if (idx < n) {
             const int ci = idx / L.k, kk = idx - ci * L.k;
-            out[kk * L.cin + ci] = v[i] / denom;
+            const float o = v[i] / denom;
+            out[kk * L.cin + ci] = o;
+            if (L.out16) row[kk * L.cin + ci] = o;
+        }
+    }
+    if (!L.out16) return;
+    __syncthreads();
+    for (int b = threadIdx.x; b * 8 < n; b += 256) {
+        const float4 v0 = *reinterpret_cast<const float4*>(row + b * 8), v1 = *reinterpret_cast<const float4*>(row + b * 8 + 4);
+        const float x[8] = {v0.x * 1.f, v0.y * 1.f, v0.z * 1.f, v0.w * 1.f, v1.x * 1.f, v1.y * 1.f, v1.z * 1.f, v1.w * 1.f};
+        if (L.fmt16 == 1) {
+            ws_half8 hi, lo;
+#pragma unroll
+            for (int j = 0; j < 8; ++j) { _Float16 h1, l1; split_f16(x[j], h1, l1); hi[j] = h1; lo[j] = l1; }
+            ws_half8* o = reinterpret_cast<ws_half8*>(static_cast<float*>(L.out16) + (long long)co * n + b * 8);
+            o[0] = hi;
+            o[1] = lo;
+        } else {
+            ws_half8 h;
+            if (L.fmt16 == 3) {
+                ws_bf16x8 q;
+#pragma unroll
+                for (int j = 0; j < 8; ++j) q[j] = (__bf16)x[j];
+                h = __builtin_bit_cast(ws_half8, q);
+            } else {
+#pragma unroll
+                for (int j = 0; j < 8; ++j) h[j] = (_Float16)x[j];
+            }
+            *reinterpret_cast<ws_half8*>(static_cast<_Float16*>(L.out16) + (long long)co * n + b * 8) = h;
         }
     }
 }
@@ -331,6 +363,40 @@
 }
 
 template <int R, bool WAVE, int NTHR = 256>
+__global__ __launch_bounds__(NTHR) void group_norm_reg_stats_kernel(const GnArgs a, long long n_units) {
+    __shared__ float red[NTHR / 64];
+    const int f4 = a.cg >> 2;
+    const int nthr = WAVE ? 64 : NTHR;
+    const int tid = WAVE ? (threadIdx.x & 63) : threadIdx.x;
+    const long long unit = WAVE ? (long long)blockIdx.x * 4 + (threadIdx.x >> 6) : (long long)blockIdx.x;
+    if (WAVE && unit >= n_units) return;
+    const int inst = (int)(unit / a.groups), g = (int)(unit - (long long)inst * a.groups);
+    const int tpp = nthr / f4;
+    const int tl = tid / f4, c4 = tid - tl * f4;
+    const GnUnit un = gn_unit(a, inst);
+    const int ntok = un.ntok;
+    const int ch = g * a.cg + c4 * 4;
+    const float cnt = (float)ntok * (float)a.cg;
+    float4 v[R];
+    gn_load_slots<R>(a, v, un.row0, un.tok_stride, ntok, tl, tpp, ch);
+    float s = 0.f;
+#pragma unroll
+    for (int r = 0; r < R; ++r) s += (v[r].x + v[r].y) + (v[r].z + v[r].w);
+    const float mean = (WAVE ? wave_sum(s) : block_sum_n<NTHR>(s, red)) / cnt;
+    float q = 0.f;
+#pragma unroll
+    for (int r = 0; r < R; ++r) {
+        if (tl + r * tpp < ntok) {
+            const float d0 = v[r].x - mean, d1 = v[r].y - mean, d2 = v[r].z - mean, d3 = v[r].w - mean;
+            q += (d0 * d0 + d1 * d1) + (d2 * d2 + d3 * d3);
+        }
+    }
+    const float var = (WAVE ? wave_sum(q) : block_sum_n<NTHR>(q, red)) / cnt;
+    const float rstd = 1.0f / sqrtf(var + a.eps);
+    if (tid == 0) a.stats_out[unit] = make_float2(mean, rstd);
+}
+
+template <int R, bool WAVE, int NTHR = 256>
 __global__ __launch_bounds__(NTHR) void group_norm_reg_h8_kernel(const GnArgs a, long long n_units) {
     __shared__ float red[NTHR / 64];
     const int f8 = a.cg >> 3;
@@ -622,6 +688,8 @@
     for (int i = 0; i < n_layers; ++i) {
         SOLA_ARG(layers[i].cin * layers[i].k <= 256 * WS_MAX_PER_THREAD && layers[i].cin * layers[i].k >= 2,
                  "ws: cin*k = %d unsupported (2..%d)", layers[i].cin * layers[i].k, 256 * WS_MAX_PER_THREAD);
+        SOLA_ARG(!layers[i].out16 || (layers[i].fmt16 >= 1 && layers[i].fmt16 <= 3 && (layers[i].cin * layers[i].k) % 8 == 0),
+                 "ws: the operand copy needs a format (1 split-f16, 2 f16, 3 bf16) and cin*k %% 8 == 0");
         a.layer[i] = layers[i];
         a.first_block[i] = blocks;
         blocks += layers[i].cout;
@@ -655,6 +723,25 @@
     return sl.buf;
 }
 int g_gn_h8 = 1;
+
+static int gn_stats_shape(const GroupNormDesc& d, bool* wave, bool* wide) {
+    if (g_gn_variant == 0 || d.groups <= 0 || d.C % d.groups != 0) return 0;
+    const int cg = d.C / d.groups;
+    if (cg % 4 != 0 || cg / 4 > 256 || (long long)d.n_inst * d.groups >= (1ll << 31)) return 0;
+    const int f4 = cg / 4;
+    const int rw = 64 % f4 == 0 ? (d.ntok + 64 / f4 - 1) / (64 / f4) : 1 << 30;
+    const int rb = 256 % f4 == 0 ? (d.ntok + 256 / f4 - 1) / (256 / f4) : 1 << 30;
+    *wave = rw <= 4;
+    *wide = false;
+    if (rw <= 4) return rw == 3 ? 4 : rw;
+    if (rb <= 16) return rb <= 2 ? 2 : rb <= 4 ? 4 : rb <= 8 ? 8 : 16;
+    if (rb <= 32 && g_gn_wide && 1024 % f4 == 0) { *wide = true; return 8; }
+    return 0;
+}
+bool group_norm_stats_only_supported(const GroupNormDesc& d) {
+    bool wave, wide;
+    return !d.in_f16 && !d.in_scale_dev && d.stats_out && gn_stats_shape(d, &wave, &wide) != 0;
+}
 
 int launch_group_norm(const GroupNormDesc& d, hipStream_t s) {
     SOLA_ARG(d.groups > 0 && d.C % d.groups == 0, "group_norm: C=%d groups=%d", d.C, d.groups);
@@ -678,6 +765,24 @@
     const int f4 = cg / 4;
     const long long n_units = (long long)d.n_inst * d.groups;
     SOLA_ARG(n_units < (1ll << 31), "group_norm: %lld (instance, group) units exceed the grid", n_units);
+    if (d.stats_only) {
+        SOLA_ARG(group_norm_stats_only_supported(d), "group_norm: no statistics-only kernel for this shape (ask group_norm_stats_only_supported)");
+        bool wave, wide;
+        const int r = gn_stats_shape(d, &wave, &wide);
+        const dim3 gw((unsigned)((n_units + 3) / 4)), gb((unsigned)n_units);
+        if (wave) {
+            if (r == 1) hipLaunchKernelGGL((group_norm_reg_stats_kernel<1, true>), gw, dim3(256), 0, s, a, n_units);
+            else if (r == 2) hipLaunchKernelGGL((group_norm_reg_stats_kernel<2, true>), gw, dim3(256), 0, s, a, n_units);
+            else hipLaunchKernelGGL((group_norm_reg_stats_kernel<4, true>), gw, dim3(256), 0, s, a, n_units);
+        } else if (wide) {
+            hipLaunchKernelGGL((group_norm_reg_stats_kernel<8, false, 1024>), gb, dim3(1024), 0, s, a, n_units);
+        } else if (r == 2) hipLaunchKernelGGL((group_norm_reg_stats_kernel<2, false>), gb, dim3(256), 0, s, a, n_units);
+        else if (r == 4) hipLaunchKernelGGL((group_norm_reg_stats_kernel<4, false>), gb, dim3(256), 0, s, a, n_units);
+        else if (r == 8) hipLaunchKernelGGL((group_norm_reg_stats_kernel<8, false>), gb, dim3(256), 0, s, a, n_units);
+        else hipLaunchKernelGGL((group_norm_reg_stats_kernel<16, false>), gb, dim3(256), 0, s, a, n_units);
+        SOLA_LAUNCH_CHECK();
+        return SOLA_OK;
+    }
     const int rw = 64 % f4 == 0 ? (d.ntok + 64 / f4 - 1) / (64 / f4) : 1 << 30;
     const int rb = 256 % f4 == 0 ? (d.ntok + 256 / f4 - 1) / (256 / f4) : 1 << 30;
     const int f8 = cg / 8;
```
